# Yotsuei/ClearConverse

Measured on AMD Instinct MI355X. Metric: xRT (audio-sec/wall-sec) end-to-end, 30 s 16 kHz clips, higher is better.
Workload: dtype bf16

## Files before the change

clearconverse_amd/_lib.py:

```python
from __future__ import annotations

import ctypes as C
import os
from pathlib import Path
from typing import Optional

_PKG = Path(__file__).resolve().parent
LIB_PATH = _PKG / "libccx.so"


class CcxError(RuntimeError):
    pass


class WhisperDims(C.Structure):
    _fields_ = [(n, C.c_int) for n in (
        "n_mels", "n_audio_ctx", "n_audio_state", "n_audio_head", "n_audio_layer",
        "n_vocab", "n_text_ctx", "n_text_state", "n_text_head", "n_text_layer")]


class SepformerDims(C.Structure):
    _fields_ = [(n, C.c_int) for n in (
        "n_filters", "kernel", "stride", "d_model", "n_head", "d_ffn", "n_layers", "n_blocks", "segment", "n_spk")]


class DecodeRules(C.Structure):
    _fields_ = [(n, C.c_int) for n in (
        "eot", "sot", "sot_prev", "no_speech", "no_timestamps", "timestamp_begin", "blank",
        "max_initial_timestamp_index", "n_suppress")] + [("suppress", C.POINTER(C.c_int))]


class GemmDesc(C.Structure):
    _fields_ = [
        ("A", C.c_void_p), ("W", C.c_void_p), ("lda", C.c_int64), ("ldw", C.c_int64),
        ("M", C.c_int), ("N", C.c_int), ("K", C.c_int), ("ntaps", C.c_int), ("a_tap_stride", C.c_int64),
        ("bias", C.c_void_p), ("out", C.c_void_p), ("ldo", C.c_int64), ("resid", C.c_void_p), ("ldr", C.c_int64),
        ("resid_mod", C.c_int), ("scale", C.c_void_p), ("shift", C.c_void_p), ("slope", C.c_float),
        ("rpb_in", C.c_int), ("rpb_out", C.c_int), ("roff", C.c_int), ("rpb_valid", C.c_int),
        ("img_rows_in", C.c_int), ("img_rows_valid", C.c_int), ("img_rows_out", C.c_int),
        ("resid_bf16", C.c_void_p), ("ldrb", C.c_int64),
        ("hq", C.c_void_p), ("hk", C.c_void_p), ("hv", C.c_void_p),
        ("d_model", C.c_int), ("n_head", C.c_int), ("S", C.c_int), ("Spad", C.c_int),
        ("v_transposed", C.c_int), ("first_block", C.c_int),
        ("a_elems", C.c_int64), ("w_elems", C.c_int64), ("out_elems", C.c_int64), ("resid_elems", C.c_int64),
        ("resid_bf16_elems", C.c_int64), ("heads_elems", C.c_int64)]


class DecAttnDesc(C.Structure):
    _fields_ = [
        ("q", C.c_void_p), ("k", C.c_void_p), ("v", C.c_void_p),
        ("rows", C.c_int), ("n_seq", C.c_int), ("H", C.c_int), ("kv_T", C.c_int), ("T", C.c_int),
        ("pos", C.POINTER(C.c_int)), ("row_seq", C.POINTER(C.c_int)), ("rows_per_seq", C.c_int),
        ("nsplit", C.c_int), ("combine", C.c_int), ("lds_pad", C.c_int),
        ("x", C.c_void_p), ("pend", C.c_void_p), ("pend_n", C.c_int), ("pend_stride", C.c_int64),
        ("ln_g", C.c_void_p), ("ln_b", C.c_void_p), ("eps", C.c_float),
        ("wq_host", C.c_void_p), ("bq", C.c_void_p),
        ("out", C.c_void_p), ("part_o", C.c_void_p), ("part_ml", C.c_void_p), ("q_x_out", C.c_void_p),
        ("q_elems", C.c_int64), ("kv_elems", C.c_int64), ("out_elems", C.c_int64), ("part_o_elems", C.c_int64),
        ("part_ml_elems", C.c_int64), ("x_elems", C.c_int64), ("pend_elems", C.c_int64), ("q_x_out_elems", C.c_int64)]


DEC_ATTN_SELF, DEC_ATTN_SPLIT, DEC_ATTN_STREAM, DEC_ATTN_PREFILL, DEC_ATTN_FUSED_Q, DEC_ATTN_TWO_LAUNCH_Q = range(6)


class DecSeqState(C.Structure):
    _fields_ = [(n, C.c_int) for n in ("pos", "prompt_len", "n_gen", "done", "last_tok", "pen_tok", "last_ts_tok", "n_tokens")] + [
        ("sum_logprob", C.c_float), ("no_speech_prob", C.c_float)]


class DecSelectDesc(C.Structure):
    _fields_ = [
        ("logits", C.c_void_p), ("ld", C.c_int64), ("n_vocab", C.c_int), ("B", C.c_int),
        ("rules", C.POINTER(DecodeRules)), ("state", C.POINTER(DecSeqState)),
        ("prompt", C.POINTER(C.c_int)), ("max_prompt", C.c_int), ("sample_len", C.c_int),
        ("gen", C.POINTER(C.c_int)), ("cur_tok", C.POINTER(C.c_int)), ("pos", C.POINTER(C.c_int)), ("n_done", C.POINTER(C.c_int)),
        ("tok_emb", C.c_void_p), ("pos_emb", C.c_void_p), ("x", C.c_void_p), ("D", C.c_int),
        ("sample", C.c_int), ("temperature", C.c_float), ("seed", C.c_uint64), ("row0", C.c_int),
        ("logits_elems", C.c_int64), ("tok_emb_elems", C.c_int64), ("pos_emb_elems", C.c_int64), ("x_elems", C.c_int64)]


class SepDesc(C.Structure):
    _fields_ = (
        [(n, C.c_void_p) for n in ("h", "xin", "y", "qkv", "att", "feats", "fc")]
        + [(n, C.c_int64) for n in ("h_elems", "xin_elems", "y_elems", "qkv_elems", "att_elems", "feats_elems", "fc_elems")]
        + [("rows", C.c_int), ("seq_start", C.POINTER(C.c_int)), ("seq_len", C.POINTER(C.c_int)), ("n_seq", C.c_int),
           ("n_tok", C.c_int), ("d_ffn", C.c_int)]
        + [(n, C.c_void_p) for n in ("ln_g", "ln_b", "gln_g", "gln_b", "wqkv", "bqkv", "wo", "bo", "w1", "b1", "w2", "b2", "wdec")]
        + [(n, C.c_int64) for n in ("ln_elems", "gln_elems", "wqkv_elems", "bqkv_elems", "wo_elems", "bo_elems", "w1_elems",
                                    "b1_elems", "w2_elems", "b2_elems", "wdec_elems")]
        + [("utt_tok0", C.POINTER(C.c_int)), ("utt_L", C.POINTER(C.c_int)), ("utt_T", C.POINTER(C.c_int)), ("n_utt", C.c_int),
           ("segment", C.c_int), ("out", C.c_void_p), ("out_stride", C.c_int64), ("out_elems", C.c_int64)])


SEP_ATTN_BLOCK, SEP_ATTENTION, SEP_FFN, SEP_FINAL_NORM, SEP_DECODER = range(5)


class AlignDesc(C.Structure):
    _fields_ = [
        ("q", C.c_void_p), ("k", C.c_void_p), ("q_elems", C.c_int64), ("k_elems", C.c_int64),
        ("n_seq", C.c_int), ("H", C.c_int), ("Spad", C.c_int),
        ("heads", C.POINTER(C.c_int)), ("n_heads", C.c_int), ("head0", C.c_int), ("t", C.c_int),
        ("Hsel", C.c_int), ("T", C.c_int), ("Mmax", C.c_int),
        ("n_keys", C.POINTER(C.c_int)), ("n_rows", C.POINTER(C.c_int)), ("r0", C.c_int),
        ("P", C.c_void_p), ("A", C.c_void_p), ("P_elems", C.c_int64), ("A_elems", C.c_int64),
        ("text_idx", C.c_void_p), ("time_idx", C.c_void_p), ("path_len", C.c_void_p), ("jump_frame", C.c_void_p),
        ("text_idx_elems", C.c_int64), ("time_idx_elems", C.c_int64), ("path_len_elems", C.c_int64), ("jump_frame_elems", C.c_int64)]


ALIGN_SCORES, ALIGN_MATRIX, ALIGN_DTW = range(3)


_vp, _i, _i64, _f = C.c_void_p, C.c_int, C.c_int64, C.c_float
_ip = C.POINTER(C.c_int)
_i32p = C.POINTER(C.c_int32)
_i64p = C.POINTER(C.c_int64)
_fp = C.POINTER(C.c_float)

PROTOTYPES = {
    "ccx_version": (C.c_char_p, []),
    "ccx_ctx_create": (_i, [_i, C.POINTER(_vp)]),
    "ccx_ctx_destroy": (None, [_vp]),
    "ccx_last_error": (C.c_char_p, [_vp]),
    "ccx_prof_enable": (_i, [_vp, _i]),
    "ccx_prof_count": (_i, [_vp]),
    "ccx_prof_get": (_i, [_vp, _i, C.c_char_p, _i, C.POINTER(C.c_double), C.POINTER(C.c_double), _fp]),
    "ccx_gemm_bf16": (_i, [_vp, _i, _vp, _i64, _vp, _i64, _vp, _vp, _i64, _vp, _i64, _i, _i, _i, _vp]),
    "ccx_gemm_bf16_desc": (_i, [_vp, _i, C.POINTER(GemmDesc), _vp]),
    "ccx_layernorm": (_i, [_vp, _vp, _vp, _vp, _vp, _vp, _i, _i, _f, _vp]),
    "ccx_gather_rows": (_i, [_vp, _vp, _vp, _i, _i, _vp, _i64, _vp]),
    "ccx_peak_normalize": (_i, [_vp, _vp, _vp, _i64, _vp, _i, _f, _vp]),
    "ccx_row_variance": (_i, [_vp, _vp, _i64, _vp, _i, _vp, _vp]),
    "ccx_cross_attention_xa": (_i, [_vp, _vp, _vp, _vp, _vp, _vp, _vp, _i, _i, _i, _i, _i, _vp, _vp]),
    "ccx_cosine_rows": (_i, [_vp, _vp, _vp, _i, _i, _i, _vp, _vp]),
    "ccx_speaker_profiles": (_i, [_vp, _vp, _vp, _vp, _i, _i, _i, _i, _vp, _vp]),
    "ccx_resample_sinc": (_i, [_vp, _vp, _i64, _vp, _i, _i, _i, _i, _vp, _vp, _i64, _vp, _i, _vp]),
    "ccx_enc_attention": (_i, [_vp, _vp, _vp, _vp, _vp, _i, _i, _i, _i, _vp]),
    "ccx_whisper_create": (_i, [_vp, C.POINTER(WhisperDims), _i, C.POINTER(_vp)]),
    "ccx_whisper_destroy": (None, [_vp]),
    "ccx_whisper_set_tensor": (_i, [_vp, C.c_char_p, _vp, _i, _i, _i64p]),
    "ccx_whisper_set_max_audio": (_i, [_vp, C.c_double]),
    "ccx_whisper_share_encoder_scratch": (_i, [_vp, _vp]),
    "ccx_whisper_finalize": (_i, [_vp]),
    "ccx_whisper_set_rules": (_i, [_vp, C.POINTER(DecodeRules)]),
    "ccx_whisper_logmel": (_i, [_vp, _vp, _i64, _ip, _ip, _i, _vp, _vp]),
    "ccx_whisper_set_mel": (_i, [_vp, _vp, _i, _vp]),
    "ccx_whisper_encode": (_i, [_vp, _i, _vp, _vp]),
    "ccx_whisper_decoder_logits": (_i, [_vp, _i32p, _i, _i, _vp, _vp]),
    "ccx_whisper_decode_greedy": (_i, [_vp, _i32p, _i32p, _i, _i, _i, _i32p, _i32p, _fp, _fp, _vp]),
    "ccx_dec_attention_desc": (_i, [_vp, _i, C.POINTER(DecAttnDesc), _vp]),
    "ccx_dec_select_step": (_i, [_vp, C.POINTER(DecSelectDesc), _vp]),
    "ccx_align_op": (_i, [_vp, _i, C.POINTER(AlignDesc), _vp]),
    "ccx_whisper_align": (_i, [_vp, _i32p, _i32p, _i, _i, _i32p, _i32p, _i, _i, _vp, _vp, _i32p, _vp]),
    "ccx_whisper_last_cross_path": (_i, [_vp]),
    "ccx_whisper_prepare_lanes": (_i, [_vp, _vp]),
    "ccx_whisper_trace_lanes": (_i, [_vp, C.c_char_p, _i]),
    "ccx_whisper_decode": (_i, [_vp, _i32p, _i32p, _i, _i, _i, _f, C.c_uint64, _i32p, _i32p, _fp, _fp, _vp]),
    "ccx_sepformer_create": (_i, [_vp, C.POINTER(SepformerDims), _i, _i, C.POINTER(_vp)]),
    "ccx_sepformer_destroy": (None, [_vp]),
    "ccx_sepformer_set_tensor": (_i, [_vp, C.c_char_p, _vp, _i64]),
    "ccx_sepformer_finalize": (_i, [_vp]),
    "ccx_sepformer_separate": (_i, [_vp, _vp, _i64, _ip, _i, _vp, _vp]),
    "ccx_sep_op": (_i, [_vp, _i, C.POINTER(SepDesc), _vp]),
    "ccx_speaker_create": (_i, [_vp, _i, _i, _i, _i, _i64, C.POINTER(_vp)]),
    "ccx_speaker_destroy": (None, [_vp]),
    "ccx_speaker_set_tensor": (_i, [_vp, C.c_char_p, _vp, _i64]),
    "ccx_speaker_finalize": (_i, [_vp]),
    "ccx_speaker_embed": (_i, [_vp, _vp, _i64p, _ip, _i, _vp, _i64p, _ip, _vp, _vp]),
    "ccx_speaker_segment": (_i, [_vp, _vp, _i64p, _ip, _i, _vp, _i64, _ip, _vp]),
    "ccx_resnet_create": (_i, [_vp, _i, _i64, _i, C.POINTER(_vp)]),
    "ccx_resnet_destroy": (None, [_vp]),
    "ccx_resnet_set_tensor": (_i, [_vp, C.c_char_p, _vp, _i64]),
    "ccx_resnet_finalize": (_i, [_vp]),
    "ccx_resnet_embed": (_i, [_vp, _vp, _i64, _i, _i, _vp, _i, _ip, _i, _vp, _vp]),
    "ccx_specgate_create": (_i, [_vp, _i64, _i, _i, C.POINTER(_vp)]),
    "ccx_specgate_destroy": (None, [_vp]),
    "ccx_specgate_reduce": (_i, [_vp, _vp, _i64, _ip, _i, _f, _vp, _vp]),
    "ccx_specgate_reduce_long": (_i, [_vp, _vp, _i64, _f, _vp, _vp]),
    "ccx_specgate_set_clip_noise": (_i, [_vp, _i]),
}

_lib: Optional[C.CDLL] = None


def load() -> C.CDLL:
    global _lib
    if _lib is not None:
        return _lib
    if not LIB_PATH.exists():
        raise CcxError(f"{LIB_PATH} is missing: run `python -m clearconverse_amd.build` "
                       "(there is no CPU fallback for the HIP path)")
    import torch
    try:
        lib = C.CDLL(str(LIB_PATH))
    except OSError as e:
        raise CcxError(f"cannot load {LIB_PATH}: {e}") from e
    for name, (res, args) in PROTOTYPES.items():
        try:
            fn = getattr(lib, name)
        except AttributeError as e:
            raise CcxError(f"libccx.so does not export {name}") from e
        fn.restype = res
        fn.argtypes = args
    _lib = lib
    return lib


class Context:

    def __init__(self, device: int = 0):
        self.lib = load()
        h = _vp()
        rc = self.lib.ccx_ctx_create(device, C.byref(h))
        if rc != 0:
            raise CcxError(f"ccx_ctx_create({device}) failed: {self.lib.ccx_last_error(None).decode()}")
        self.handle = h
        self.device = device

    def check(self, rc: int, what: str = ""):
        if rc != 0:
            raise CcxError(f"{what or 'ccx call'} failed ({rc}): {self.lib.ccx_last_error(self.handle).decode()}")

    prof_on = False

    def prof_enable(self, on: bool = True):
        self.check(self.lib.ccx_prof_enable(self.handle, 1 if on else 0), "ccx_prof_enable")
        self.prof_on = bool(on)

    def prof_records(self):
        out = []
        buf = C.create_string_buffer(64)
        fl, by, ms = C.c_double(), C.c_double(), C.c_float()
        for i in range(self.lib.ccx_prof_count(self.handle)):
            self.check(self.lib.ccx_prof_get(self.handle, i, buf, 64, C.byref(fl), C.byref(by), C.byref(ms)), "ccx_prof_get")
            out.append((buf.value.decode(), fl.value, by.value, ms.value))
        return out

    def close(self):
        if getattr(self, "handle", None):
            self.lib.ccx_ctx_destroy(self.handle)
            self.handle = None

    def __del__(self):
        try:
            self.close()
        except Exception:
            pass


def current_stream_ptr() -> int:
    import torch
    return int(torch.cuda.current_stream().cuda_stream)


def ptr(t) -> int:
    if t is None:
        return 0
    if not t.is_contiguous():
        raise CcxError("tensor passed to libccx must be contiguous")
    return int(t.data_ptr())
```

clearconverse_amd/csrc/dec_ops.hip:

```cpp
#include "../../include/ccx.h"
#include "ccx_common.h"
#include "decoder.h"
#include "op_scratch.h"

static_assert(sizeof(ccx_dec_seq_state) == sizeof(DecSeqState), "ccx_dec_seq_state mirrors DecSeqState field for field");

namespace {

__global__ void dec_ops_bf16_to_f32_kernel(const bf16_t* __restrict__ in, float* __restrict__ out, long n) {
  const long i = (long)blockIdx.x * 256 + threadIdx.x;
  if (i < n) out[i] = bf16_to_f32(in[i]);
}

}

extern "C" int ccx_dec_attention_desc(ccx_ctx* ctx, int form, const ccx_dec_attn_desc* d, void* stream_) {
  if (!ctx) return CCX_ERR_ARG;
  hipStream_t stream = (hipStream_t)stream_;
  CCX_REQUIRE(ctx, d != nullptr, "ccx_dec_attention_desc: desc is NULL");
  CCX_REQUIRE(ctx, form >= CCX_DEC_ATTN_SELF && form <= CCX_DEC_ATTN_TWO_LAUNCH_Q, "ccx_dec_attention_desc: unknown form %d", form);
  const bool is_self = form == CCX_DEC_ATTN_SELF, is_split = form == CCX_DEC_ATTN_SPLIT, is_stream = form == CCX_DEC_ATTN_STREAM;
  const bool is_prefill = form == CCX_DEC_ATTN_PREFILL, with_q = form == CCX_DEC_ATTN_FUSED_Q || form == CCX_DEC_ATTN_TWO_LAUNCH_Q;
  const bool partials = is_split || with_q;
  const bool final_out = is_self || is_stream || is_prefill || (is_split && d->combine);
  const int rows = d->rows, H = d->H, n_seq = d->n_seq, kv_T = d->kv_T;
  CCX_REQUIRE(ctx, rows >= 1 && rows <= 65536 && n_seq >= 1 && n_seq <= 65536 && H >= 1 && H <= 64 && kv_T >= 1 && kv_T <= (1 << 20),
              "ccx_dec_attention_desc: rows=%d, n_seq=%d, H=%d or kv_T=%d out of range", rows, n_seq, H, kv_T);
  CCX_REQUIRE(ctx, d->k && d->v && ccx_aligned16(d->k) && ccx_aligned16(d->v), "ccx_dec_attention_desc: k / v null or not 16-byte aligned");
  const int64_t kv_need = (int64_t)n_seq * H * kv_T * 64;
  CCX_REQUIRE(ctx, kv_need <= d->kv_elems, "ccx_dec_attention_desc: k / v are read up to element %ld, kv_elems=%ld", (long)kv_need, (long)d->kv_elems);
  if (is_self || is_split || is_prefill) {
    if (d->row_seq)
      for (int i = 0; i < rows; i++)
        CCX_REQUIRE(ctx, d->row_seq[i] >= 0 && d->row_seq[i] < n_seq, "ccx_dec_attention_desc: row_seq[%d] = %d out of range [0, %d)", i, d->row_seq[i], n_seq);
    else CCX_REQUIRE(ctx, rows <= n_seq, "ccx_dec_attention_desc: row_seq is NULL with more rows (%d) than sequences (%d)", rows, n_seq);
  } else {
    CCX_REQUIRE(ctx, d->row_seq == nullptr, "ccx_dec_attention_desc: row_seq is not taken by form %d (row r reads sequence r)", form);
    CCX_REQUIRE(ctx, rows <= n_seq, "ccx_dec_attention_desc: more rows (%d) than sequences (%d)", rows, n_seq);
  }
  if (is_prefill) {
    const int P = d->rows_per_seq;
    CCX_REQUIRE(ctx, P >= 2 && P <= 4096, "ccx_dec_attention_desc: rows_per_seq = %d, the prefill form needs >= 2", P);
    CCX_REQUIRE(ctx, d->row_seq && rows % P == 0, "ccx_dec_attention_desc: rows_per_seq needs row_seq and a multiple of it in rows");
    for (int i = 0; i < rows; i++) {
      CCX_REQUIRE(ctx, d->row_seq[i] == d->row_seq[i - i % P], "ccx_dec_attention_desc: row %d is not in its group's sequence (row_seq)", i);
      CCX_REQUIRE(ctx, d->row_seq[i] == i / P, "ccx_dec_attention_desc: row_seq[%d] = %d, the prefill form needs group g on sequence g", i, d->row_seq[i]);
    }
  } else CCX_REQUIRE(ctx, d->rows_per_seq <= 1, "ccx_dec_attention_desc: rows_per_seq = %d is taken by the prefill form only", d->rows_per_seq);
  if (is_self) {
    CCX_REQUIRE(ctx, d->pos != nullptr, "ccx_dec_attention_desc: pos is NULL");
    for (int i = 0; i < rows; i++)
      CCX_REQUIRE(ctx, d->pos[i] >= 0 && d->pos[i] < kv_T, "ccx_dec_attention_desc: pos[%d] = %d out of range [0, kv_T = %d)", i, d->pos[i], kv_T);
  } else {
    CCX_REQUIRE(ctx, d->pos == nullptr, "ccx_dec_attention_desc: pos is taken by the self form only");
    CCX_REQUIRE(ctx, d->T >= 1 && d->T <= kv_T, "ccx_dec_attention_desc: T = %d out of range [1, kv_T = %d]", d->T, kv_T);
  }
  if (is_prefill) CCX_REQUIRE(ctx, d->T <= 1536, "ccx_dec_attention_desc: T = %d, the prefill form streams at most 1536 keys per block", d->T);
  const int nsplit = partials ? d->nsplit : 1;
  CCX_REQUIRE(ctx, nsplit >= 1 && nsplit <= 8, "ccx_dec_attention_desc: nsplit = %d out of range [1, 8]", d->nsplit);
  CCX_REQUIRE(ctx, d->lds_pad >= 0 && d->lds_pad <= 128 * 1024 && ((is_split || is_stream) || d->lds_pad == 0),
              "ccx_dec_attention_desc: lds_pad = %d out of range [0, 131072] or given to a form that has none", d->lds_pad);
  if (!with_q) {
    CCX_REQUIRE(ctx, d->q && ccx_aligned16(d->q), "ccx_dec_attention_desc: q null or not 16-byte aligned");
    CCX_REQUIRE(ctx, (int64_t)rows * H * 64 <= d->q_elems, "ccx_dec_attention_desc: q is read up to element %ld, q_elems=%ld", (long)rows * H * 64, (long)d->q_elems);
  }
  if (final_out) {
    CCX_REQUIRE(ctx, d->out != nullptr, "ccx_dec_attention_desc: out is NULL");
    CCX_REQUIRE(ctx, (int64_t)rows * H * 64 <= d->out_elems, "ccx_dec_attention_desc: out is written up to element %ld, out_elems=%ld", (long)rows * H * 64, (long)d->out_elems);
  }
  if (partials) {
    CCX_REQUIRE(ctx, d->part_o && d->part_ml && ccx_aligned16(d->part_o) && ccx_aligned16(d->part_ml), "ccx_dec_attention_desc: part_o / part_ml null or not 16-byte aligned");
    const int64_t po = (int64_t)rows * H * nsplit * 64, pml = (int64_t)rows * H * nsplit * 2;
    CCX_REQUIRE(ctx, po <= d->part_o_elems, "ccx_dec_attention_desc: part_o is written up to element %ld, part_o_elems=%ld", (long)po, (long)d->part_o_elems);
    CCX_REQUIRE(ctx, pml <= d->part_ml_elems, "ccx_dec_attention_desc: part_ml is written up to element %ld, part_ml_elems=%ld", (long)pml, (long)d->part_ml_elems);
  }
  if (with_q) {
    CCX_REQUIRE(ctx, rows <= 16 && H == 12, "ccx_dec_attention_desc: the fused query needs rows <= 16 (got %d) and H == 12 (got %d)", rows, H);
    CCX_REQUIRE(ctx, d->x && d->pend && d->ln_g && d->ln_b && d->bq && d->wq_host, "ccx_dec_attention_desc: x, pend, ln_g, ln_b, bq or wq_host is NULL");
    CCX_REQUIRE(ctx, ccx_aligned16(d->x) && ccx_aligned16(d->pend) && ccx_aligned16(d->ln_g) && ccx_aligned16(d->ln_b) && ccx_aligned16(d->bq),
                "ccx_dec_attention_desc: x, pend, ln_g, ln_b or bq not 16-byte aligned");
    CCX_REQUIRE(ctx, d->pend_n >= 0 && d->pend_n <= 4, "ccx_dec_attention_desc: pend_n = %d out of range [0, 4]", d->pend_n);
    CCX_REQUIRE(ctx, d->pend_stride >= (int64_t)rows * 768 && d->pend_stride % 4 == 0, "ccx_dec_attention_desc: pend_stride = %ld smaller than a slab or not a multiple of 4", (long)d->pend_stride);
    CCX_REQUIRE(ctx, (int64_t)rows * 768 <= d->x_elems, "ccx_dec_attention_desc: x is read up to element %ld, x_elems=%ld", (long)rows * 768, (long)d->x_elems);
    const int64_t pn = (int64_t)((d->pend_n > 1 ? d->pend_n : 1) - 1) * d->pend_stride + (int64_t)rows * 768;
    CCX_REQUIRE(ctx, pn <= d->pend_elems, "ccx_dec_attention_desc: pend is read up to element %ld, pend_elems=%ld", (long)pn, (long)d->pend_elems);
    if (d->q_x_out) {
      CCX_REQUIRE(ctx, ccx_aligned16(d->q_x_out) && d->q_x_out != d->x, "ccx_dec_attention_desc: q_x_out not 16-byte aligned or aliasing x");
      CCX_REQUIRE(ctx, (int64_t)rows * 768 <= d->q_x_out_elems, "ccx_dec_attention_desc: q_x_out is written up to element %ld, q_x_out_elems=%ld", (long)rows * 768, (long)d->q_x_out_elems);
    }
  }

  ccx_op_scratch sc;
#define DO_HIP(expr) do { hipError_t e_ = (expr); if (e_ != hipSuccess) return ccx_fail(ctx, CCX_ERR_HIP, "%s failed: %s", #expr, hipGetErrorString(e_)); } while (0)
  DecAttnParams ap;
  memset(&ap, 0, sizeof(ap));
  ap.q = (const float*)d->q; ap.k = (const bf16_t*)d->k; ap.v = (const bf16_t*)d->v; ap.H = H; ap.kv_T = kv_T; ap.T = is_self ? 0 : d->T;
  ap.scale_log2e = 0.125f * 1.4426950408889634f;
  ap.part_o = (float*)d->part_o; ap.part_ml = (float*)d->part_ml; ap.lds_pad = d->lds_pad;
  const long n_out = (long)rows * H * 64;
  bf16_t* d_out16 = nullptr;
  if (final_out) {
    DO_HIP(sc.alloc(&d_out16, (size_t)n_out));
    DO_HIP(hipMemsetAsync(d_out16, 0xFF, (size_t)n_out * 2, stream));
    ap.out_bf16 = d_out16;
  }
  int* d_pos = nullptr; int* d_rs = nullptr;
  if (is_self) { DO_HIP(sc.upload(&d_pos, d->pos, (size_t)rows)); ap.pos = d_pos; }
  if (d->row_seq) { DO_HIP(sc.upload(&d_rs, d->row_seq, (size_t)rows)); ap.row_seq = d_rs; }
  bf16_t* d_wq = nullptr; float* d_q = nullptr;
  if (with_q) {
    const std::vector<bf16_t> packed = pack_mfma_rows(d->wq_host, 768, 768, 16);
    DO_HIP(sc.upload(&d_wq, packed.data(), packed.size()));
  }
  int rc = CCX_OK;
  if (is_self) rc = ccx_launch_dec_attention(ctx, ap, rows, 1, true, stream);
  else if (is_split) {
    rc = ccx_launch_dec_attention(ctx, ap, rows, nsplit, false, stream);
    if (rc == CCX_OK && d->combine) rc = ccx_launch_dec_combine(ctx, ap.part_o, ap.part_ml, nsplit, d_out16, rows, H, stream);
  } else if (is_stream) {
    ap.stream_mode = 1;
    rc = ccx_launch_dec_attention(ctx, ap, rows, 1, true, stream);
  } else if (is_prefill) {
    ap.stream_mode = 1; ap.rows_per_seq = d->rows_per_seq;
    rc = ccx_launch_dec_attention(ctx, ap, rows / d->rows_per_seq, 1, true, stream);
  } else if (form == CCX_DEC_ATTN_FUSED_Q) {
    ap.qx = (const float*)d->x; ap.q_pend = (const float*)d->pend; ap.q_pend_n = d->pend_n; ap.q_pend_stride = (long)d->pend_stride;
    ap.q_x_out = (float*)d->q_x_out; ap.q_ln_g = (const float*)d->ln_g; ap.q_ln_b = (const float*)d->ln_b; ap.q_eps = d->eps;
    ap.q_W = d_wq; ap.q_bias = (const float*)d->bq; ap.q_K = 768;
    rc = ccx_launch_dec_cross_fused_q(ctx, ap, rows, nsplit, stream);
  } else {
    DO_HIP(sc.alloc(&d_q, (size_t)rows * 768));
    DecLinearParams lp;
    memset(&lp, 0, sizeof(lp));
    lp.M = rows; lp.N = 768; lp.K = 768; lp.W = d_wq; lp.ldw = 768; lp.bias = (const float*)d->bq; lp.out = d_q; lp.ldo = 768;
    lp.x = (const float*)d->x; lp.pend = (const float*)d->pend; lp.pend_n = d->pend_n; lp.pend_stride = (long)d->pend_stride;
    lp.x_out = (float*)d->q_x_out; lp.ln_g = (const float*)d->ln_g; lp.ln_b = (const float*)d->ln_b; lp.eps = d->eps;
    rc = ccx_launch_dec_linear(ctx, ACT_LN, DEPI_F32, lp, stream);
    ap.q = d_q;
    if (rc == CCX_OK) rc = ccx_launch_dec_attention(ctx, ap, rows, nsplit, false, stream);
  }
  if (rc == CCX_OK && final_out) {
    hipLaunchKernelGGL(dec_ops_bf16_to_f32_kernel, dim3((unsigned)((n_out + 255) / 256)), dim3(256), 0, stream, d_out16, (float*)d->out, n_out);
    DO_HIP(hipGetLastError());
  }
  DO_HIP(hipStreamSynchronize(stream));
  return rc;
}

extern "C" int ccx_dec_select_step(ccx_ctx* ctx, const ccx_dec_select_desc* d, void* stream_) {
  if (!ctx) return CCX_ERR_ARG;
  hipStream_t stream = (hipStream_t)stream_;
  CCX_REQUIRE(ctx, d != nullptr, "ccx_dec_select_step: desc is NULL");
  const int V = d->n_vocab, B = d->B, D = d->D;
  CCX_REQUIRE(ctx, B >= 1 && B <= 65536, "ccx_dec_select_step: B = %d out of range", B);
  CCX_REQUIRE(ctx, V >= 4 && V % 4 == 0 && V <= 13 * 4096, "ccx_dec_select_step: n_vocab = %d must be a multiple of 4 and <= 53248", V);
  CCX_REQUIRE(ctx, d->ld >= V && d->ld % 4 == 0, "ccx_dec_select_step: ld = %ld must be >= n_vocab and a multiple of 4", (long)d->ld);
  CCX_REQUIRE(ctx, d->logits && ccx_aligned16(d->logits), "ccx_dec_select_step: logits null or not 16-byte aligned");
  CCX_REQUIRE(ctx, (int64_t)(B - 1) * d->ld + V <= d->logits_elems, "ccx_dec_select_step: logits are read up to element %ld, logits_elems=%ld",
              (long)((int64_t)(B - 1) * d->ld + V), (long)d->logits_elems);
  CCX_REQUIRE(ctx, d->rules && d->state && d->gen && d->cur_tok && d->pos && d->n_done, "ccx_dec_select_step: rules, state, gen, cur_tok, pos or n_done is NULL");
  const ccx_decode_rules& r = *d->rules;
  std::vector<unsigned char> mask;
  CCX_TRY(ccx_build_suppress_mask(ctx, "ccx_dec_select_step", &r, V, mask));
  CCX_REQUIRE(ctx, r.no_speech >= 0 && r.timestamp_begin >= 0 && r.blank >= 0, "ccx_dec_select_step: rules.no_speech, timestamp_begin or blank negative");
  CCX_REQUIRE(ctx, d->sample_len >= 1 && d->sample_len <= (1 << 20), "ccx_dec_select_step: sample_len = %d out of range", d->sample_len);
  CCX_REQUIRE(ctx, d->max_prompt >= 0 && (d->max_prompt == 0 || d->prompt), "ccx_dec_select_step: prompt is NULL with max_prompt = %d", d->max_prompt);
  CCX_REQUIRE(ctx, D >= 4 && D % 4 == 0 && D <= 4096, "ccx_dec_select_step: D = %d must be a multiple of 4 in [4, 4096]", D);
  CCX_REQUIRE(ctx, d->tok_emb && d->pos_emb && d->x && ccx_aligned16(d->tok_emb) && ccx_aligned16(d->pos_emb) && ccx_aligned16(d->x),
              "ccx_dec_select_step: tok_emb, pos_emb or x null or not 16-byte aligned");
  CCX_REQUIRE(ctx, (int64_t)V * D <= d->tok_emb_elems, "ccx_dec_select_step: tok_emb is read up to element %ld, tok_emb_elems=%ld", (long)V * D, (long)d->tok_emb_elems);
  CCX_REQUIRE(ctx, (int64_t)B * D <= d->x_elems, "ccx_dec_select_step: x is written up to element %ld, x_elems=%ld", (long)B * D, (long)d->x_elems);
  const int64_t pos_rows = d->pos_emb_elems / D;
  CCX_REQUIRE(ctx, d->sample == 0 || d->sample == 1, "ccx_dec_select_step: sample = %d must be 0 or 1", d->sample);
  CCX_REQUIRE(ctx, d->sample || d->temperature == 0.f, "ccx_dec_select_step: temperature %g needs sample = 1", (double)d->temperature);
  CCX_REQUIRE(ctx, d->temperature >= 0.f && d->row0 >= 0, "ccx_dec_select_step: temperature or row0 negative");
  for (int b = 0; b < B; b++) {
    const ccx_dec_seq_state& s = d->state[b];
    CCX_REQUIRE(ctx, s.n_gen >= 0 && s.n_gen <= d->sample_len, "ccx_dec_select_step: state[%d].n_gen = %d out of range [0, sample_len = %d]", b, s.n_gen, d->sample_len);
    CCX_REQUIRE(ctx, s.pos >= 0 && s.pos + 1 < pos_rows, "ccx_dec_select_step: state[%d].pos = %d, pos + 1 must be a row of pos_emb (%ld rows)", b, s.pos, (long)pos_rows);
    CCX_REQUIRE(ctx, s.prompt_len >= 0 && s.prompt_len <= d->max_prompt, "ccx_dec_select_step: state[%d].prompt_len = %d out of range [0, max_prompt = %d]", b, s.prompt_len, d->max_prompt);
    CCX_REQUIRE(ctx, s.done == 0 || s.done == 1, "ccx_dec_select_step: state[%d].done = %d must be 0 or 1", b, s.done);
    const bool prompt_phase = s.pos < s.prompt_len - 1;
    if (prompt_phase) {
      const int tok = d->prompt[(size_t)b * d->max_prompt + s.pos + 1];
      CCX_REQUIRE(ctx, tok >= 0 && tok < V, "ccx_dec_select_step: prompt[%d][%d] = %d out of range", b, s.pos + 1, tok);
    } else if (!s.done) {
      CCX_REQUIRE(ctx, s.n_gen < d->sample_len, "ccx_dec_select_step: state[%d].n_gen = %d leaves no room in gen (sample_len = %d)", b, s.n_gen, d->sample_len);
      CCX_REQUIRE(ctx, s.last_tok < V && s.pen_tok < V && s.last_ts_tok < V, "ccx_dec_select_step: state[%d] holds a token id >= n_vocab", b);
    }
  }

  ccx_op_scratch sc;
  unsigned char* d_mask = nullptr; DecSeqState* d_state = nullptr;
  int *d_prompt = nullptr, *d_cur = nullptr, *d_pos = nullptr, *d_gen = nullptr, *d_ndone = nullptr;
  unsigned* d_cfg = nullptr;
  const size_t n_gen_tab = (size_t)B * d->sample_len;
  constexpr int kGuard = 16;
  std::vector<int> gen_h(n_gen_tab + kGuard, 0x5a5a5a5a);
  memcpy(gen_h.data(), d->gen, n_gen_tab * 4);
  DO_HIP(sc.upload(&d_mask, mask.data(), mask.size()));
  DO_HIP(sc.upload(&d_state, (const DecSeqState*)d->state, (size_t)B));
  if (d->max_prompt > 0) DO_HIP(sc.upload(&d_prompt, d->prompt, (size_t)B * d->max_prompt));
  DO_HIP(sc.upload(&d_cur, d->cur_tok, (size_t)B));
  DO_HIP(sc.upload(&d_pos, d->pos, (size_t)B));
  DO_HIP(sc.upload(&d_gen, gen_h.data(), gen_h.size()));
  DO_HIP(sc.upload(&d_ndone, d->n_done, (size_t)1));
  unsigned cfg[4] = {0u, (unsigned)(d->seed & 0xffffffffu), (unsigned)(d->seed >> 32), 0u};
  memcpy(&cfg[0], &d->temperature, 4);
  DO_HIP(sc.upload(&d_cfg, cfg, (size_t)4));

  DecSelectParams sp;
  memset(&sp, 0, sizeof(sp));
  sp.logits = (const float*)d->logits; sp.ld_logits = (long)d->ld; sp.n_vocab = V; sp.state = d_state; sp.prompt = d_prompt;
  sp.max_prompt = d->max_prompt; sp.cur_tok = d_cur; sp.pos = d_pos; sp.gen = d_gen; sp.sample_len = d->sample_len;
  sp.n_done = d_ndone; sp.suppress_mask = d_mask; sp.eot = r.eot; sp.blank = r.blank;
  sp.no_speech = r.no_speech; sp.timestamp_begin = r.timestamp_begin;
  sp.max_initial_ts = r.max_initial_timestamp_index;
  sp.tok_emb = (const float*)d->tok_emb; sp.pos_emb = (const float*)d->pos_emb; sp.x = (float*)d->x; sp.D = D;
  sp.sample_cfg = d_cfg; sp.row0 = d->row0; sp.sample = d->sample;
  CCX_TRY(ccx_launch_dec_select(ctx, sp, B, stream));
  DO_HIP(hipStreamSynchronize(stream));
  DO_HIP(hipMemcpy(gen_h.data(), d_gen, gen_h.size() * 4, hipMemcpyDeviceToHost));
  for (int i = 0; i < kGuard; i++)
    if (gen_h[n_gen_tab + i] != 0x5a5a5a5a) return ccx_fail(ctx, CCX_ERR_STATE, "ccx_dec_select_step: the kernel wrote behind the gen table (word %d)", i);
  memcpy(d->gen, gen_h.data(), n_gen_tab * 4);
  DO_HIP(hipMemcpy(d->state, d_state, (size_t)B * sizeof(DecSeqState), hipMemcpyDeviceToHost));
  DO_HIP(hipMemcpy(d->cur_tok, d_cur, (size_t)B * 4, hipMemcpyDeviceToHost));
  DO_HIP(hipMemcpy(d->pos, d_pos, (size_t)B * 4, hipMemcpyDeviceToHost));
  DO_HIP(hipMemcpy(d->n_done, d_ndone, 4, hipMemcpyDeviceToHost));
#undef DO_HIP
  return CCX_OK;
}
```

clearconverse_amd/csrc/decoder.h:

```cpp
#pragma once
#include <vector>
#include "../../include/ccx.h"
#include "ccx_common.h"

enum { ACT_LN = 0, ACT_BF16 = 1, ACT_COMBINE = 2 };
enum { DEPI_BF16_GELU = 1, DEPI_PARTIAL = 2, DEPI_F32 = 3, DEPI_SELF_QKV = 4, DEPI_RESOLVE = 5 };

struct DecLinearParams {
  int M, N, K;
  const bf16_t* W; long ldw;
  const float* bias;
  const float* x;
  const float* pend; int pend_n; long pend_stride;
  float* x_out;
  const float* ln_g; const float* ln_b; float eps;
  float* ln_mean_out;
  const bf16_t* act; long lda;
  const float* part_o; const float* part_ml; int nsplit;
  float* xres; bf16_t* xb; float2* st_out; const float* shift; float shift_c;
  void* out; long ldo;
  bf16_t* cache_k; bf16_t* cache_v; int cache_T; const int* pos; const int* row_seq;
};
int ccx_launch_dec_linear(ccx_ctx* ctx, int act, int epi, const DecLinearParams& p, hipStream_t stream);
int ccx_dec_linear_ksplit(int K, int epi);
int ccx_launch_dec_resolve_ln(ccx_ctx* ctx, const float* x, const float* pend, int pend_n, long pend_stride, const float* g,
                              const float* b, bf16_t* out, float* x_out, int M, int K, float eps, hipStream_t stream,
                              float* mean_out = nullptr);

struct DecAttnParams {
  const float* q;
  const bf16_t* k;
  const bf16_t* v;
  int H, kv_T;
  const int* pos;
  int T;
  float scale_log2e;
  bf16_t* out_bf16;
  float* part_o;
  float* part_ml;
  int lds_pad;
  int stream_mode;
  const int* row_seq; int rows_per_seq;
  const float* qx; const float* q_pend; int q_pend_n; long q_pend_stride; float* q_x_out;
  const float* q_ln_g; const float* q_ln_b; float q_eps;
  const bf16_t* q_W; const float* q_bias; int q_K;
};
int ccx_launch_dec_attention(ccx_ctx* ctx, const DecAttnParams& p, int B, int nsplit, bool final_out, hipStream_t stream);
int ccx_launch_dec_cross_fused_q(ccx_ctx* ctx, const DecAttnParams& p, int B, int nsplit, hipStream_t stream);

struct DecSeqState {
  int pos, prompt_len, n_gen, done;
  int last_tok, pen_tok, last_ts_tok, n_tokens;
  float sum_logprob, no_speech_prob;
};

struct DecSelectParams {
  const float* logits; long ld_logits; int n_vocab;
  DecSeqState* state;
  const int* prompt; int max_prompt;
  int* cur_tok; int* pos;
  int* gen; int sample_len;
  int* n_done;
  const unsigned char* suppress_mask;
  int eot, blank, no_speech, timestamp_begin, max_initial_ts;
  const float* tok_emb; const float* pos_emb; float* x; int D;
  const unsigned* sample_cfg; int row0;
  int sample;
};
int ccx_launch_dec_select(ccx_ctx* ctx, const DecSelectParams& p, int B, hipStream_t stream);
int ccx_launch_dec_embed(ccx_ctx* ctx, const float* tok_emb, const float* pos_emb, const int* cur_tok, const int* pos,
                         float* x, int B, int D, hipStream_t stream);
int ccx_launch_dec_gather_rows(ccx_ctx* ctx, const bf16_t* src, const int* idx, bf16_t* dst, int n, int D, hipStream_t stream);
int ccx_launch_dec_combine(ccx_ctx* ctx, const float* part_o, const float* part_ml, int nsplit, bf16_t* out, int M, int H,
                           hipStream_t stream);

static inline std::vector<bf16_t> pack_mfma_rows(const float* src, int N, int K, int row_pad) {
  const int Np = (N + row_pad - 1) / row_pad * row_pad;
  const int kst = K / 32;
  std::vector<bf16_t> tmp((size_t)Np * K, 0);
  for (int nt = 0; nt < Np / 16; nt++)
    for (int ks = 0; ks < kst; ks++)
      for (int l = 0; l < 64; l++) {
        const int n = nt * 16 + (l & 15), k0 = ks * 32 + 8 * (l >> 4);
        bf16_t* dst = &tmp[(((size_t)nt * kst + ks) * 64 + l) * 8];
        if (n < N)
          for (int j = 0; j < 8; j++) dst[j] = ccx_host_f32_to_bf16(src[(size_t)n * K + k0 + j]);
      }
  return tmp;
}

static inline int ccx_build_suppress_mask(ccx_ctx* ctx, const char* who, const ccx_decode_rules* r, int V, std::vector<unsigned char>& mask) {
  CCX_REQUIRE(ctx, r->eot >= 0 && r->eot < V, "%s: rules.eot = %d out of range [0, n_vocab = %d)", who, r->eot, V);
  CCX_REQUIRE(ctx, r->sot < V, "%s: rules.sot = %d out of range (n_vocab = %d)", who, r->sot, V);
  CCX_REQUIRE(ctx, r->no_speech < V, "%s: rules.no_speech = %d out of range (n_vocab = %d)", who, r->no_speech, V);
  CCX_REQUIRE(ctx, r->timestamp_begin <= V, "%s: rules.timestamp_begin = %d behind n_vocab = %d", who, r->timestamp_begin, V);
  CCX_REQUIRE(ctx, r->blank < V, "%s: rules.blank = %d out of range (n_vocab = %d)", who, r->blank, V);
  CCX_REQUIRE(ctx, r->no_timestamps < V, "%s: rules.no_timestamps = %d out of range (n_vocab = %d)", who, r->no_timestamps, V);
  mask.assign((size_t)V + 4, 0);
  for (int i = 0; i < r->n_suppress; i++) {
    CCX_REQUIRE(ctx, r->suppress[i] >= 0 && r->suppress[i] < V, "%s: rules.suppress[%d] = %d out of range [0, n_vocab = %d)", who, i, r->suppress[i], V);
    mask[r->suppress[i]] = 1;
  }
  if (r->no_timestamps >= 0) mask[r->no_timestamps] = 1;
  return CCX_OK;
}
```

clearconverse_amd/csrc/decoder.hip:

```cpp
#include <string>
#include "decoder.h"

__global__ void dec_embed_kernel(const float* __restrict__ tok_emb, const float* __restrict__ pos_emb,
                                 const int* __restrict__ cur_tok, const int* __restrict__ pos, float* __restrict__ x,
                                 int D) {
  const int b = blockIdx.x;
  const float4* te = (const float4*)(tok_emb + (long)cur_tok[b] * D);
  const float4* pe = (const float4*)(pos_emb + (long)pos[b] * D);
  float4* xo = (float4*)(x + (long)b * D);
  for (int i = threadIdx.x; i < D / 4; i += blockDim.x) {
    const float4 a = te[i], c = pe[i];
    xo[i] = make_float4(a.x + c.x, a.y + c.y, a.z + c.z, a.w + c.w);
  }
}

#include "dec_ln.h"

__device__ __forceinline__ float centre_shift(float mean, float rstd) { return fabsf(mean) * rstd > 1.f ? mean : 0.f; }

__device__ __forceinline__ uint4 combine_partials(const float* part_o, const float* part_ml, int nsplit, int mh, int c) {
  const float2* ml = (const float2*)(part_ml + ((long)mh * nsplit) * 2);
  const float* ob = part_o + ((long)mh * nsplit) * 64 + 8 * c;
  float2 mlv[8];
  float4 oa[8], oc[8];
// ... 1043 lines not shown
#pragma unroll
  for (int i = 0; i < SEL_V4; i++) {
    const int v0 = tid * 4 + i * 4096;
    if (v0 + 3 < V) {
      const float4 f = *(const float4*)(lg + v0);
      const uchar4 m = *(const uchar4*)(p.suppress_mask + v0);
      val[4 * i] = f.x; val[4 * i + 1] = f.y; val[4 * i + 2] = f.z; val[4 * i + 3] = f.w;
      sup |= ((unsigned long long)((m.x ? 1 : 0) | (m.y ? 2 : 0) | (m.z ? 4 : 0) | (m.w ? 8 : 0))) << (4 * i);
    } else {
      val[4 * i] = val[4 * i + 1] = val[4 * i + 2] = val[4 * i + 3] = -INFINITY;
      sup |= 0xFull << (4 * i);
    }
  }
  const int i_gen = s.n_gen;
  const int tsb = p.timestamp_begin;

  if (i_gen == 0) {
    float mx = -INFINITY;
#pragma unroll
    for (int i = 0; i < SEL_V4 * 4; i++) mx = fmaxf(mx, val[i]);
    mx = block_reduce_max(mx, sh);
    float sum = 0.f;
#pragma unroll
    for (int i = 0; i < SEL_V4 * 4; i++) sum += __builtin_amdgcn_exp2f((val[i] - mx) * 1.4426950408889634f);
    sum = block_reduce_sum(sum, sh);
    if (tid == 0) s.no_speech_prob = expf(lg[p.no_speech] - mx) / sum;
  }

  const bool last_ts = i_gen >= 1 && s.last_tok >= tsb;
  const bool pen_ts = i_gen < 2 || s.pen_tok >= tsb;
  int s_lo = tsb;
  if (s.last_ts_tok >= 0) s_lo = (last_ts && !pen_ts) ? s.last_ts_tok : s.last_ts_tok + 1;
  int s_hi = V;
  if (i_gen == 0 && p.max_initial_ts >= 0) s_hi = tsb + p.max_initial_ts + 1;
  if (last_ts && pen_ts) s_hi = s_lo;
  const int t_lo = (i_gen == 0) ? tsb : ((last_ts && !pen_ts) ? p.eot : 0);

  float mx_text = -INFINITY, mx_ts = -INFINITY;
  int am_text = 0x7fffffff, am_ts = 0x7fffffff;
#pragma unroll
  for (int i = 0; i < SEL_V4 * 4; i++) {
    const int v = tid * 4 + (i >> 2) * 4096 + (i & 3);
    const bool is_text = v < tsb;
    const bool allowed = !((sup >> i) & 1) && (is_text ? (v >= t_lo) : (v >= s_lo && v < s_hi));
    const float x = allowed ? val[i] : -INFINITY;
    val[i] = x;
    const bool bt_ = is_text && x > mx_text, bs_ = !is_text && x > mx_ts;
    mx_text = bt_ ? x : mx_text; am_text = bt_ ? v : am_text;
    mx_ts = bs_ ? x : mx_ts; am_ts = bs_ ? v : am_ts;
  }
  auto block_argmax = [&](float v_, int idx, float& oval, int& oidx) {
#pragma unroll
    for (int o = 32; o > 0; o >>= 1) {
      const float ov = __shfl_xor(v_, o, 64);
      const int oi = __shfl_xor(idx, o, 64);
      if (ov > v_ || (ov == v_ && oi < idx)) { v_ = ov; idx = oi; }
    }
    __syncthreads();
    if ((tid & 63) == 0) { sh_v[tid >> 6] = v_; sh_i[tid >> 6] = idx; }
    __syncthreads();
    oval = sh_v[0]; oidx = sh_i[0];
    for (int w = 1; w < (int)(blockDim.x >> 6); w++)
      if (sh_v[w] > oval || (sh_v[w] == oval && sh_i[w] < oidx)) { oval = sh_v[w]; oidx = sh_i[w]; }
  };
  float bt, bs; int it, is;
  block_argmax(mx_text, am_text, bt, it);
  block_argmax(mx_ts, am_ts, bs, is);
  const float mx_all = fmaxf(bt, bs);

  float se_text = 0.f, se_ts = 0.f;
#pragma unroll
  for (int i = 0; i < SEL_V4 * 4; i++) {
    const int v = tid * 4 + (i >> 2) * 4096 + (i & 3);
    const float e = __builtin_amdgcn_exp2f((val[i] - mx_all) * 1.4426950408889634f);
    se_text += (v < tsb) ? e : 0.f;
    se_ts += (v < tsb) ? 0.f : e;
  }
  se_text = block_reduce_sum(se_text, sh);
  se_ts = block_reduce_sum(se_ts, sh);

  const float lse_ts = (se_ts > 0.f) ? mx_all + logf(se_ts) : -INFINITY;
  const bool force_ts = lse_ts > bt;
  const float lnorm = logf(force_ts ? se_ts : se_text + se_ts);

  const float temperature = SAMPLE ? __uint_as_float(p.sample_cfg[0]) : 0.f;
  int samp = -1; float samp_logit = 0.f;
  if (SAMPLE && temperature > 0.f) {
    const uint2 key = make_uint2(p.sample_cfg[1], p.sample_cfg[2]);
    const float inv_t = 1.0f / temperature;
    float best = -INFINITY, best_logit = -INFINITY; int best_i = 0x7fffffff;
#pragma unroll
    for (int i = 0; i < SEL_V4; i++) {
      const int v0 = tid * 4 + i * 4096;
      const uint4 r = philox4x32_10(make_uint4((unsigned)(v0 >> 2), (unsigned)(p.row0 + b), (unsigned)i_gen, 0u), key);
      const unsigned rr[4] = {r.x, r.y, r.z, r.w};
#pragma unroll
      for (int j = 0; j < 4; j++) {
        const int v = v0 + j;
        const float x = (force_ts && v < tsb) ? -INFINITY : val[4 * i + j];
        const float sc = x * inv_t + gumbel_from_u32(rr[j]);
        if (sc > best) { best = sc; best_i = v; best_logit = x; }
      }
    }
    float ov; int oi;
    block_argmax(best, best_i, ov, oi);
    samp = oi;
    __syncthreads();
    if (best_i == samp && best == ov) sh[0] = best_logit;
    __syncthreads();
    samp_logit = sh[0];
  }

  if (tid == 0) {
    int next; float logprob;
    if (samp >= 0) {
      next = samp;
      logprob = (samp_logit - mx_all) - lnorm;
    } else if (force_ts) {
      next = is;
      logprob = (bs - mx_all) - lnorm;
    } else {
      if (bt > bs || (bt == bs && it < is)) next = it; else next = is;
      logprob = -lnorm;
    }
    s.sum_logprob += logprob;
    p.gen[(long)b * p.sample_len + i_gen] = next;
    s.n_gen = i_gen + 1;
    s.pen_tok = s.last_tok;
    s.last_tok = next;
    if (next >= tsb) s.last_ts_tok = next;
    int cont = 0;
    if (next == p.eot) {
      s.done = 1;
      s.n_tokens = i_gen;
      atomicAdd(p.n_done, 1);
    } else if (s.n_gen >= p.sample_len) {
      s.done = 1;
      s.n_tokens = s.n_gen;
      atomicAdd(p.n_done, 1);
    } else {
      s.pos += 1;
      p.cur_tok[b] = next;
      p.pos[b] = s.pos;
      cont = 1;
    }
    p.state[b] = s;
    sh_next[0] = cont ? next : -1;
    sh_next[1] = s.pos;
  }
  __syncthreads();
  if (sh_next[0] >= 0) embed_next(sh_next[0], sh_next[1]);
}

int ccx_launch_dec_embed(ccx_ctx* ctx, const float* tok_emb, const float* pos_emb, const int* cur_tok, const int* pos,
                         float* x, int B, int D, hipStream_t stream) {
  hipLaunchKernelGGL(dec_embed_kernel, dim3(B), dim3(192), 0, stream, tok_emb, pos_emb, cur_tok, pos, x, D);
  CCX_CHECK_LAUNCH(ctx);
  return CCX_OK;
}

int ccx_launch_dec_select(ccx_ctx* ctx, const DecSelectParams& p, int B, hipStream_t stream) {
  ccx_prof_scope ps(ctx, stream, "dec_select_kernel", 0.0, (double)B * p.n_vocab * 5.0);
  if (p.sample) hipLaunchKernelGGL(dec_select_kernel<true>, dim3(B), dim3(1024), 0, stream, p);
  else hipLaunchKernelGGL(dec_select_kernel<false>, dim3(B), dim3(1024), 0, stream, p);
  CCX_CHECK_LAUNCH(ctx);
  return CCX_OK;
}
```

clearconverse_amd/csrc/gemm_bf16.h:

```cpp
#pragma once
#include "ccx_common.h"

enum GemmEpi {
  EPI_BF16 = 0,
  EPI_BF16_GELU = 1,
  EPI_F32_RESID = 2,
  EPI_F32 = 3,
  EPI_HEADS = 4,
  EPI_BF16_RELU = 5,
  EPI_F32_GELU_POS = 6,
  EPI_BF16_LRELU_AFFINE = 7,
  EPI_BF16_ADD_RELU = 8
};

struct GemmParams {
  const bf16_t* A;
  const bf16_t* W;
  long lda, ldw;
  int M, N, K;
  int ntaps; long a_tap_stride;
  const float* bias;
  void* out;
  long ldo;
  const float* resid;
  long ldr;
  int resid_mod;
  const float* scale; const float* shift;
  float slope;
  int rpb_in, rpb_out, roff, rpb_valid;
  int img_rows_in, img_rows_valid, img_rows_out;
  const bf16_t* resid_bf16; long ldrb;
  bf16_t* hq; bf16_t* hk; bf16_t* hv;
  int d_model, n_head;
  int S, Spad;
  int v_transposed;
  int first_block;
};

__host__ __device__ inline long ccx_gemm_remap_row(const GemmParams& p, int m, bool& valid) {
  if (p.rpb_in <= 0) { valid = true; return m; }
  int g = m / p.rpb_in;
  const int i = m - g * p.rpb_in;
  valid = i < p.rpb_valid;
  if (p.img_rows_in > 0) {
    const int img = g / p.img_rows_in, r = g - img * p.img_rows_in;
    valid = valid && r < p.img_rows_valid;
    g = img * p.img_rows_out + r;
  }
  return (long)g * p.rpb_out + i + p.roff;
}

int ccx_launch_gemm(ccx_ctx* ctx, int epi, const GemmParams& p, hipStream_t stream);
```

clearconverse_amd/csrc/gemm_bf16.hip:

```cpp
#include <map>
#include <string>
#include "gemm_bf16.h"

#ifndef CCX_ABL_NO_MFMA
#define CCX_ABL_NO_MFMA 0
#endif
#ifndef CCX_ABL_NO_DMA
#define CCX_ABL_NO_DMA 0
#endif
#ifndef CCX_ABL_NO_EPI
#define CCX_ABL_NO_EPI 0
#endif
#ifndef CCX_ABL_STORE_LOCAL
#define CCX_ABL_STORE_LOCAL 0
#endif
#define BM 128
#define BN 128
#define BK 64
#define STAGE_BYTES 32768

typedef const __attribute__((address_space(1))) void* gptr_t;
typedef __attribute__((address_space(3))) void* lptr_t;

__device__ __forceinline__ int keyA(int r) { return (r >> 1) & 7; }
template <int CM> __device__ __forceinline__ int w_row(int j, int i) {
  return CM == 1 ? 16 * j + i : 32 * (j >> 1) + 8 * (i >> 2) + 4 * (j & 1) + (i & 3);
}
template <int CM> __device__ __forceinline__ int keyW(int r) {
  return CM == 1 ? (r >> 1) & 7 : ((r >> 1) & 1) | (((r >> 3) & 1) << 1) | (((r >> 4) & 1) << 2);
}
template <int CM> __device__ __forceinline__ int col4(int j, int h) {
  return CM == 1 ? 16 * j + 4 * h : 32 * (j >> 1) + 8 * h + 4 * (j & 1);
}
__device__ __forceinline__ void epi_store16(void* dst, uint4 v) { *(uint4*)dst = v; }
__device__ __forceinline__ void epi_store16f(void* dst, float4 v) { *(float4*)dst = v; }
__device__ __forceinline__ float4 epi_load16f(const float* src) { return *(const float4*)src; }

constexpr int colmap_of(int epi) { return (epi == EPI_F32 || epi == EPI_F32_RESID || epi == EPI_F32_GELU_POS) ? 1 : 2; }

template <bool SWAP, int CM, int WM, int WN, int MT>
__device__ __forceinline__ void gemm_mainloop(const GemmParams& p, char* smem, int m0, int n0, f32x4 (&acc)[MT][4]) {
  constexpr int NW = WM * WN;
  constexpr int A_ROWS = WM * MT * 16, B_ROWS = WN * 64;
  constexpr int A_BYTES = A_ROWS * 128, B_BYTES = B_ROWS * 128;
  constexpr int STAGE = A_BYTES + B_BYTES;
  constexpr int NA = A_ROWS / 8 / NW, NB = B_ROWS / 8 / NW;
  const int tid = threadIdx.x, lane = tid & 63, wave = tid >> 6;
  const int wr = wave / WN, wc = wave % WN;

  const bf16_t* srcA[NA];
  const bf16_t* srcB[NB];
#pragma unroll
  for (int i = 0; i < NA; i++) {
    const int r = (wave * NA + i) * 8 + (lane >> 3);
    int gm = m0 + r; gm = gm < p.M ? gm : p.M - 1;
    srcA[i] = p.A + (long)gm * p.lda + (((lane & 7) ^ keyA(r)) << 3);
  }
#pragma unroll
  for (int i = 0; i < NB; i++) {
    const int r = (wave * NB + i) * 8 + (lane >> 3);
    int gn = n0 + r; gn = gn < p.N ? gn : p.N - 1;
    srcB[i] = p.W + (long)gn * p.ldw + (((lane & 7) ^ keyW<CM>(r)) << 3);
  }
  const int kt_per_tap = p.K / BK;
  auto stage = [&](int t, int buf) {
    char* sA = smem + buf * STAGE;
    char* sB = sA + A_BYTES;
    const int tap = t / kt_per_tap;
    const long ka = (long)(t - tap * kt_per_tap) * BK + (long)tap * p.a_tap_stride;
    const int kw = t * BK;
#pragma unroll
    for (int i = 0; i < NA; i++)
      __builtin_amdgcn_global_load_lds((gptr_t)(srcA[i] + ka), (lptr_t)(sA + (wave * NA + i) * 1024), 16, 0, 0);
#pragma unroll
    for (int i = 0; i < NB; i++)
      __builtin_amdgcn_global_load_lds((gptr_t)(srcB[i] + kw), (lptr_t)(sB + (wave * NB + i) * 1024), 16, 0, 0);
  };

  const int l15 = lane & 15, h = lane >> 4;
  const int ka = keyA(l15);
  const int kb = keyW<CM>(w_row<CM>(0, l15));
  int offA[2], offB[2];
#pragma unroll
  for (int ks = 0; ks < 2; ks++) {
    offA[ks] = (wr * MT * 16 + l15) * 128 + (((4 * ks + h) ^ ka) << 4);
    offB[ks] = (wc * 64 + w_row<CM>(0, l15)) * 128 + (((4 * ks + h) ^ kb) << 4);
  }

  const int nt = kt_per_tap * (p.ntaps > 1 ? p.ntaps : 1);
  stage(0, 0);
  __syncthreads();
  for (int t = 0; t < nt; t++) {
    const int buf = t & 1;
    if (t + 1 < nt) stage(t + 1, buf ^ 1);
    const char* sA = smem + buf * STAGE;
    const char* sB = sA + A_BYTES;
#pragma unroll
    for (int ks = 0; ks < 2; ks++) {
      bf16x8 b[4];
#pragma unroll
      for (int j = 0; j < 4; j++) b[j] = *(const bf16x8*)(sB + offB[ks] + w_row<CM>(j, 0) * 128);
#pragma unroll
      for (int mt = 0; mt < MT; mt++) {
        const bf16x8 a = *(const bf16x8*)(sA + offA[ks] + mt * 16 * 128);
#pragma unroll
        for (int j = 0; j < 4; j++) {
          if (SWAP)
            acc[mt][j] = __builtin_amdgcn_mfma_f32_16x16x32_bf16(b[j], a, acc[mt][j], 0, 0, 0);
          else
            acc[mt][j] = __builtin_amdgcn_mfma_f32_16x16x32_bf16(a, b[j], acc[mt][j], 0, 0, 0);
        }
      }
    }
    __syncthreads();
  }
}

__device__ __forceinline__ long remap_row(const GemmParams& p, int m, bool& valid) { return ccx_gemm_remap_row(p, m, valid); }

template <int EPI, int WM, int WN, int MT, typename MainLoop>
__device__ __forceinline__ void gemm_tile(const GemmParams& p, char* smem, int m0, int n0, MainLoop mainloop) {
  constexpr int CM = colmap_of(EPI);
  const int lane = threadIdx.x & 63;
  const int wave = __builtin_amdgcn_readfirstlane(threadIdx.x >> 6);
  const int wr = wave / WN, wc = wave % WN;
  const int l15 = lane & 15, h = lane >> 4;
  const int cb = n0 + wc * 64;

  f32x4 acc[MT][4];
#pragma unroll
  for (int i = 0; i < MT; i++)
#pragma unroll
    for (int j = 0; j < 4; j++) acc[i][j] = (f32x4){0.f, 0.f, 0.f, 0.f};

  if (EPI == EPI_HEADS) {
    const int blk = n0 / p.d_model + p.first_block;
    if (blk == 2 && p.v_transposed) {
      mainloop(p, smem, m0, n0, acc, std::false_type{});
      float bvj[4];
#pragma unroll
      for (int j = 0; j < 4; j++) bvj[j] = p.bias ? p.bias[cb + w_row<CM>(j, l15)] : 0.f;
#pragma unroll
      for (int j = 0; j < 4; j++) asm volatile("" ::"v"(bvj[j]));
#pragma unroll
      for (int j = 0; j < 4; j++) {
        const int n = cb + w_row<CM>(j, l15);
        const int nn = n % p.d_model, hh = nn >> 6, d = nn & 63;
        const float bv = bvj[j];
#pragma unroll
        for (int mt = 0; mt < MT; mt++) {
          const int m = m0 + wr * MT * 16 + mt * 16 + 4 * h;
          if (m < p.M) {
            const int b = m / p.S, s = m - b * p.S;
            bf16_t* dst = p.hv + ((long)(b * p.n_head + hh) * 64 + d) * p.Spad + s;
            uint2 v;
            v.x = pack_bf16x2(acc[mt][j][0] + bv, acc[mt][j][1] + bv);
            v.y = pack_bf16x2(acc[mt][j][2] + bv, acc[mt][j][3] + bv);
            *(uint2*)dst = v;
          }
        }
      }
      return;
    }
  }

  mainloop(p, smem, m0, n0, acc, std::true_type{});

  const int Nw = (p.N + 15) & ~15;
  if (EPI != EPI_HEADS && cb >= Nw) return;
  int c4[4];
#pragma unroll
  for (int j = 0; j < 4; j++) c4[j] = cb + col4<CM>(j, h);
  float bias[16];
#pragma unroll
  for (int i = 0; i < 16; i++) bias[i] = 0.f;
  if (p.bias) {
    const bool al = ((uintptr_t)p.bias & 15) == 0;
#pragma unroll
    for (int j = 0; j < 4; j++) {
      if (al && c4[j] + 4 <= p.N) {
        const float4 b4 = *(const float4*)(p.bias + c4[j]);
        bias[4 * j] = b4.x; bias[4 * j + 1] = b4.y; bias[4 * j + 2] = b4.z; bias[4 * j + 3] = b4.w;
      } else {
#pragma unroll
        for (int r = 0; r < 4; r++) bias[4 * j + r] = (c4[j] + r < p.N) ? p.bias[c4[j] + r] : 0.f;
      }
    }
  }
#pragma unroll
  for (int i = 0; i < 16; i++) asm volatile("" ::"v"(bias[i]));

  constexpr bool RES_F32 = (EPI == EPI_F32_RESID || EPI == EPI_F32_GELU_POS || EPI == EPI_BF16_LRELU_AFFINE);
  constexpr bool RES_BF16 = (EPI == EPI_BF16_ADD_RELU);
  constexpr bool OUT_BF16 = CM == 2;
  constexpr int GM = EPI == EPI_BF16_LRELU_AFFINE ? 1 : (RES_F32 || RES_BF16) ? 2 : 4;
  constexpr int NG = MT / GM;
  struct Group {
    long orow[GM];
    bool ok[GM];
    float4 rf[RES_F32 ? GM : 1][4];
    uint4 rb[RES_BF16 ? GM : 1][2];
  };
  auto rows = [&](auto full_tag) {
    constexpr bool FULL = decltype(full_tag)::value;
    auto request = [&](int mt0, Group& G) {
      if (EPI == EPI_HEADS) return;
#pragma unroll
      for (int g = 0; g < GM; g++) {
        const int m = m0 + wr * MT * 16 + (mt0 + g) * 16 + l15;
        bool valid = FULL;
        long orow = m;
        if (!FULL) { orow = 0; if (m < p.M) orow = remap_row(p, m, valid); }
        G.ok[g] = valid; G.orow[g] = orow;
        if constexpr (RES_F32) {
          const bool have = EPI != EPI_BF16_LRELU_AFFINE || p.resid != nullptr;
          const long rrow = !valid ? 0 : (EPI != EPI_BF16_LRELU_AFFINE && p.resid_mod > 0) ? (orow % p.resid_mod) : orow;
#pragma unroll
          for (int j = 0; j < 4; j++) {
            const int cj = (FULL || c4[j] < Nw) ? c4[j] : 0;
            if (have) G.rf[g][j] = epi_load16f(p.resid + rrow * p.ldr + cj);
            else G.rf[g][j] = make_float4(0.f, 0.f, 0.f, 0.f);
          }
        }
        if constexpr (RES_BF16) {
          const long rrow = valid ? orow : 0;
#pragma unroll
          for (int i = 0; i < 2; i++) {
            const int ci = (FULL || c4[2 * i] < Nw) ? c4[2 * i] : 0;
            if (p.resid_bf16) G.rb[g][i] = *(const uint4*)(p.resid_bf16 + rrow * p.ldrb + ci);
            else G.rb[g][i] = make_uint4(0, 0, 0, 0);
          }
        }
      }
    };
    auto finish = [&](int mt0, const Group& G) {
#pragma unroll
      for (int g = 0; g < GM; g++) {
        if constexpr (RES_F32) {
#pragma unroll
          for (int j = 0; j < 4; j++) asm volatile("" ::"v"(G.rf[g][j].x), "v"(G.rf[g][j].y), "v"(G.rf[g][j].z), "v"(G.rf[g][j].w));
        }
        if constexpr (RES_BF16) {
#pragma unroll
          for (int i = 0; i < 2; i++) asm volatile("" ::"v"(G.rb[g][i].x), "v"(G.rb[g][i].y), "v"(G.rb[g][i].z), "v"(G.rb[g][i].w));
        }
      }
#pragma unroll
      for (int g = 0; g < GM; g++) {
        const int mt = mt0 + g;
        const int m = m0 + wr * MT * 16 + mt * 16 + l15;
        if (!FULL && m >= p.M) continue;
        float v[16];
#pragma unroll
        for (int j = 0; j < 4; j++)
#pragma unroll
          for (int r = 0; r < 4; r++) v[4 * j + r] = acc[mt][j][r] + bias[4 * j + r];

        if (EPI == EPI_HEADS) {
          const int blk = cb / p.d_model + p.first_block;
          const int hh = (cb % p.d_model) >> 6;
          const int b = m / p.S, s = m - b * p.S;
          bf16_t* base = blk == 0 ? p.hq : (blk == 1 ? p.hk : p.hv);
          bf16_t* dst = base + ((long)(b * p.n_head + hh) * p.Spad + s) * 64;
#pragma unroll
          for (int i = 0; i < 2; i++) {
            uint4 o;
            o.x = pack_bf16x2(v[8 * i], v[8 * i + 1]);     o.y = pack_bf16x2(v[8 * i + 2], v[8 * i + 3]);
            o.z = pack_bf16x2(v[8 * i + 4], v[8 * i + 5]); o.w = pack_bf16x2(v[8 * i + 6], v[8 * i + 7]);
            epi_store16(dst + (c4[2 * i] - cb), o);
          }
          continue;
        }

        if (!FULL && !G.ok[g]) continue;
        const long orow = CCX_ABL_STORE_LOCAL ? (G.orow[g] & 255) : G.orow[g];

        if constexpr (EPI == EPI_BF16_LRELU_AFFINE) {
#pragma unroll
          for (int j = 0; j < 4; j++) {
            v[4 * j + 0] += G.rf[g][j].x; v[4 * j + 1] += G.rf[g][j].y; v[4 * j + 2] += G.rf[g][j].z; v[4 * j + 3] += G.rf[g][j].w;
          }
#pragma unroll
          for (int j = 0; j < 4; j++)
#pragma unroll
            for (int r = 0; r < 4; r++) {
              const int c = c4[j] + r;
              float t = v[4 * j + r] >= 0.f ? v[4 * j + r] : p.slope * v[4 * j + r];
              const float sc = (p.scale && c < p.N) ? p.scale[c] : 1.f;
              const float sh = (p.shift && c < p.N) ? p.shift[c] : 0.f;
              v[4 * j + r] = t * sc + sh;
            }
        }
        if constexpr (EPI == EPI_BF16_ADD_RELU) {
          const uint32_t rw[8] = {G.rb[g][0].x, G.rb[g][0].y, G.rb[g][0].z, G.rb[g][0].w, G.rb[g][1].x, G.rb[g][1].y, G.rb[g][1].z, G.rb[g][1].w};
#pragma unroll
          for (int i = 0; i < 8; i++) {
            v[2 * i] += __uint_as_float(rw[i] << 16);
            v[2 * i + 1] += __uint_as_float(rw[i] & 0xffff0000u);
          }
#pragma unroll
          for (int i = 0; i < 16; i++) v[i] = fmaxf(v[i], 0.f);
        }
        if constexpr (OUT_BF16) {
          if (EPI == EPI_BF16_GELU) {
#pragma unroll
            for (int i = 0; i < 16; i++) v[i] = gelu_erf(v[i]);
          }
          if (EPI == EPI_BF16_RELU) {
#pragma unroll
            for (int i = 0; i < 16; i++) v[i] = fmaxf(v[i], 0.f);
          }
          bf16_t* dst = (bf16_t*)p.out + orow * p.ldo;
#pragma unroll
          for (int i = 0; i < 2; i++) {
            if (!FULL && c4[2 * i] >= Nw) continue;
            uint4 o;
            o.x = pack_bf16x2(v[8 * i], v[8 * i + 1]);     o.y = pack_bf16x2(v[8 * i + 2], v[8 * i + 3]);
            o.z = pack_bf16x2(v[8 * i + 4], v[8 * i + 5]); o.w = pack_bf16x2(v[8 * i + 6], v[8 * i + 7]);
            epi_store16(dst + c4[2 * i], o);
          }
        } else {
          if (EPI == EPI_F32_GELU_POS) {
#pragma unroll
            for (int i = 0; i < 16; i++) v[i] = gelu_erf(v[i]);
          }
          if constexpr (EPI == EPI_F32_RESID || EPI == EPI_F32_GELU_POS) {
#pragma unroll
            for (int j = 0; j < 4; j++) {
              v[4 * j + 0] += G.rf[g][j].x; v[4 * j + 1] += G.rf[g][j].y; v[4 * j + 2] += G.rf[g][j].z; v[4 * j + 3] += G.rf[g][j].w;
            }
          }
          float* dst = (float*)p.out + orow * p.ldo;
#pragma unroll
          for (int j = 0; j < 4; j++) {
            if (!FULL && c4[j] >= Nw) continue;
            epi_store16f(dst + c4[j], make_float4(v[4 * j], v[4 * j + 1], v[4 * j + 2], v[4 * j + 3]));
          }
        }
      }
    };
    Group G[2];
    request(0, G[0]);
#pragma unroll
// ... 71 lines not shown
  if (full) rows(std::true_type{});
  else rows(std::false_type{});
}

template <int EPI, int WM, int WN, int MT>
__global__ __launch_bounds__(WM * WN * 64, (WM * WN) >= 4 ? (WM * WN) / 4 * (MT == 4 ? 2 : 1) : 4) void gemm_bf16_nt_kernel(GemmParams p) {
  constexpr int TBM = WM * MT * 16, TBN = WN * 64;
  extern __shared__ __attribute__((aligned(16))) char smem[];
  const int tiles_n = (p.N + TBN - 1) / TBN;
  const int wg = xcd_remap(blockIdx.x, gridDim.x);
  const int tm = wg / tiles_n, tn = wg - tm * tiles_n;
  gemm_tile<EPI, WM, WN, MT>(p, smem, tm * TBM, tn * TBN, [](const GemmParams& pp, char* sm, int m0, int n0, f32x4 (&acc)[MT][4], auto swap) {
    gemm_mainloop<decltype(swap)::value, colmap_of(EPI), WM, WN, MT>(pp, sm, m0, n0, acc);
  });
}

template <bool SWAP, int CM>
__device__ __forceinline__ void gemm_mainloop_phased(const GemmParams& p, char* smem, int m0, int n0, f32x4 (&acc)[8][4]) {
  const int tid = threadIdx.x, lane = tid & 63;
  const int wave = __builtin_amdgcn_readfirstlane(tid >> 6);
  const int wr = wave >> 2, wc = wave & 3;

  const bf16_t* srcA[2][2];
  const bf16_t* srcB[2][2];
  int dstA[2][2], dstB[2][2];
#pragma unroll
  for (int a = 0; a < 2; a++)
#pragma unroll
    for (int i = 0; i < 2; i++) {
      const int r0 = wr * 128 + a * 64 + wc * 16 + i * 8;
      const int r = r0 + (lane >> 3);
      int gm = m0 + r; gm = gm < p.M ? gm : p.M - 1;
      srcA[a][i] = p.A + (long)gm * p.lda + (((lane & 7) ^ keyA(r)) << 3);
      dstA[a][i] = r0 * 128;
      const int x = 2 * wave + i;
      const int g8 = 8 * (x >> 2) + 4 * a + (x & 3);
      const int rb = g8 * 8 + (lane >> 3);
      int gn = n0 + rb; gn = gn < p.N ? gn : p.N - 1;
      srcB[a][i] = p.W + (long)gn * p.ldw + (((lane & 7) ^ keyW<CM>(rb)) << 3);
      dstB[a][i] = 32768 + g8 * 1024;
    }
  const int kt_per_tap = p.K / BK;
  const int nt = kt_per_tap * (p.ntaps > 1 ? p.ntaps : 1);
  auto a_koff = [&](int t) -> long {
    const int tap = t / kt_per_tap;
    return (long)(t - tap * kt_per_tap) * BK + (long)tap * p.a_tap_stride;
  };
  auto stage_a = [&](int t, long ka, int a) {
    char* buf = smem + (t & 1) * 65536;
    __builtin_amdgcn_global_load_lds((gptr_t)(srcA[a][0] + ka), (lptr_t)(buf + dstA[a][0]), 16, 0, 0);
    __builtin_amdgcn_global_load_lds((gptr_t)(srcA[a][1] + ka), (lptr_t)(buf + dstA[a][1]), 16, 0, 0);
  };
  auto stage_b = [&](int t, int b) {
    char* buf = smem + (t & 1) * 65536;
    const int kw = t * BK;
    __builtin_amdgcn_global_load_lds((gptr_t)(srcB[b][0] + kw), (lptr_t)(buf + dstB[b][0]), 16, 0, 0);
    __builtin_amdgcn_global_load_lds((gptr_t)(srcB[b][1] + kw), (lptr_t)(buf + dstB[b][1]), 16, 0, 0);
  };

  const int l15 = lane & 15, h = lane >> 4;
  const int ka_ = keyA(l15);
  const int kb_ = keyW<CM>(w_row<CM>(0, l15));
  int offA[2], offB[2];
#pragma unroll
  for (int ks = 0; ks < 2; ks++) {
    offA[ks] = (wr * 128 + l15) * 128 + (((4 * ks + h) ^ ka_) << 4);
    offB[ks] = 32768 + (wc * 64 + w_row<CM>(0, l15)) * 128 + (((4 * ks + h) ^ kb_) << 4);
  }

  long ka1 = nt > 1 ? a_koff(1) : 0;
  long ka2 = nt > 2 ? a_koff(2) : 0;
  int kk2 = nt > 2 ? 2 % kt_per_tap : 0;
  stage_a(0, 0, 0); stage_b(0, 0); stage_b(0, 1); stage_a(0, 0, 1);
  if (nt > 1) {
    stage_a(1, ka1, 0); stage_b(1, 0); stage_b(1, 1);
    asm volatile("s_waitcnt vmcnt(6)" ::: "memory");
  } else {
    asm volatile("s_waitcnt vmcnt(0)" ::: "memory");
  }
  __builtin_amdgcn_s_barrier();
  if (wr == 1) __builtin_amdgcn_s_barrier();

  bf16x8 fa[4][2], fb0[2][2], fb1[2][2];
#define CCX_PHASE_MFMA(MT0, J0, FB)                                                                         \
  __builtin_amdgcn_sched_barrier(0);                                                                        \
  __builtin_amdgcn_s_barrier();                                                                             \
  asm volatile("s_waitcnt lgkmcnt(0)" ::: "memory");                                                        \
  __builtin_amdgcn_sched_barrier(0);                                                                        \
  __builtin_amdgcn_s_setprio(1);                                                                            \
  _Pragma("unroll") for (int ks = 0; ks < 2; ks++)                                                          \
  _Pragma("unroll") for (int m = 0; m < 4; m++)                                                             \
  _Pragma("unroll") for (int jj = 0; jj < 2; jj++) {                                                        \
    if (CCX_ABL_NO_MFMA) { asm volatile("" ::"v"(FB[jj][ks]), "v"(fa[m][ks])); }                           \
    else if (SWAP) acc[MT0 + m][J0 + jj] = __builtin_amdgcn_mfma_f32_16x16x32_bf16(FB[jj][ks], fa[m][ks], acc[MT0 + m][J0 + jj], 0, 0, 0); \
    else      acc[MT0 + m][J0 + jj] = __builtin_amdgcn_mfma_f32_16x16x32_bf16(fa[m][ks], FB[jj][ks], acc[MT0 + m][J0 + jj], 0, 0, 0); \
  }                                                                                                         \
  __builtin_amdgcn_s_setprio(0);                                                                            \
  __builtin_amdgcn_sched_barrier(0);                                                                        \
  __builtin_amdgcn_s_barrier();

  for (int t = 0; t < nt; t++) {
    const char* buf = smem + (t & 1) * 65536;
#pragma unroll
    for (int ks = 0; ks < 2; ks++)
#pragma unroll
      for (int jj = 0; jj < 2; jj++) fb0[jj][ks] = *(const bf16x8*)(buf + offB[ks] + w_row<CM>(jj, 0) * 128);
    __builtin_amdgcn_sched_barrier(0);
#pragma unroll
    for (int ks = 0; ks < 2; ks++)
#pragma unroll
      for (int m = 0; m < 4; m++) fa[m][ks] = *(const bf16x8*)(buf + offA[ks] + m * 16 * 128);
    if (!CCX_ABL_NO_DMA && t + 1 < nt) stage_a(t + 1, ka1, 1);
    CCX_PHASE_MFMA(0, 0, fb0)
#pragma unroll
    for (int ks = 0; ks < 2; ks++)
#pragma unroll
      for (int jj = 0; jj < 2; jj++) fb1[jj][ks] = *(const bf16x8*)(buf + offB[ks] + w_row<CM>(2 + jj, 0) * 128);
    if (!CCX_ABL_NO_DMA && t + 2 < nt) stage_a(t + 2, ka2, 0);
    CCX_PHASE_MFMA(0, 2, fb1)
#pragma unroll
    for (int ks = 0; ks < 2; ks++)
#pragma unroll
      for (int m = 0; m < 4; m++) fa[m][ks] = *(const bf16x8*)(buf + offA[ks] + (4 + m) * 16 * 128);
    if (!CCX_ABL_NO_DMA && t + 2 < nt) stage_b(t + 2, 0);
    CCX_PHASE_MFMA(4, 2, fb1)
    if (!CCX_ABL_NO_DMA && t + 2 < nt) {
      stage_b(t + 2, 1);
      asm volatile("s_waitcnt vmcnt(6)" ::: "memory");
    } else {
      asm volatile("s_waitcnt vmcnt(0)" ::: "memory");
    }
    CCX_PHASE_MFMA(4, 0, fb0)
    ka1 = ka2;
    kk2++;
    if (kk2 == kt_per_tap) { kk2 = 0; ka2 += BK + p.a_tap_stride - (long)kt_per_tap * BK; }
    else ka2 += BK;
  }
#undef CCX_PHASE_MFMA
  if (wr == 0) __builtin_amdgcn_s_barrier();
}

template <int EPI>
__global__ __launch_bounds__(512, 1) void gemm_bf16_phased_kernel(GemmParams p) {
  extern __shared__ __attribute__((aligned(16))) char smem[];
  const int tiles_n = (p.N + 255) / 256;
  const int wg = xcd_remap(blockIdx.x, gridDim.x);
  const int tm = wg / tiles_n, tn = wg - tm * tiles_n;
  gemm_tile<EPI, 2, 4, 8>(p, smem, tm * 256, tn * 256, [](const GemmParams& pp, char* sm, int m0, int n0, f32x4 (&acc)[8][4], auto swap) {
    gemm_mainloop_phased<decltype(swap)::value, colmap_of(EPI)>(pp, sm, m0, n0, acc);
  });
}

template <int EPI, int WM, int WN, int MT>
static int launch_epi_geo(ccx_ctx* ctx, const GemmParams& p, hipStream_t stream) {
  constexpr int TBM = WM * MT * 16, TBN = WN * 64;
  constexpr int LDS = 2 * (TBM + TBN) * 128;
  const int tiles = ccx_cdiv(p.M, TBM) * ccx_cdiv(p.N, TBN);
  static ccx_lds_optin optin;
  CCX_HIP(ctx, optin.ensure(ctx->device, (const void*)gemm_bf16_nt_kernel<EPI, WM, WN, MT>, LDS));
  {
    const double obytes = (EPI == EPI_F32 || EPI == EPI_F32_RESID || EPI == EPI_F32_GELU_POS) ? 4.0 : 2.0;
    const double kt = (double)p.K * (p.ntaps > 1 ? p.ntaps : 1);
    const bool by_shape = ctx->prof_on && getenv("CCX_PROF_SHAPES") != nullptr;
    const char* label = "gemm_bf16_nt_kernel";
    if (by_shape) {
      static std::mutex mu;
      static std::map<std::string, std::string> names;
      char buf[160];
      snprintf(buf, sizeof(buf), "gemm<epi%d,%dx%d> M=%d N=%d K=%d taps=%d", EPI, TBM, TBN, p.M, p.N, p.K, p.ntaps > 1 ? p.ntaps : 1);
      std::lock_guard<std::mutex> lk(mu);
      label = names.emplace(buf, buf).first->second.c_str();
    }
    ccx_prof_scope ps(ctx, stream, label, 2.0 * p.M * (double)p.N * kt,
                      2.0 * ((double)p.M * p.K + (double)p.N * kt) + obytes * p.M * (double)p.N);
    hipLaunchKernelGGL((gemm_bf16_nt_kernel<EPI, WM, WN, MT>), dim3(tiles), dim3(WM * WN * 64), LDS, stream, p);
  }
  CCX_CHECK_LAUNCH(ctx);
  return CCX_OK;
}

template <int EPI>
static int launch_phased(ccx_ctx* ctx, const GemmParams& p, hipStream_t stream) {
  constexpr int LDS = 131072;
  const int tiles = ccx_cdiv(p.M, 256) * ccx_cdiv(p.N, 256);
  static ccx_lds_optin optin;
  CCX_HIP(ctx, optin.ensure(ctx->device, (const void*)gemm_bf16_phased_kernel<EPI>, LDS));
  {
    const double obytes = (EPI == EPI_F32 || EPI == EPI_F32_RESID || EPI == EPI_F32_GELU_POS) ? 4.0 : 2.0;
    const double kt = (double)p.K * (p.ntaps > 1 ? p.ntaps : 1);
    const bool by_shape = ctx->prof_on && getenv("CCX_PROF_SHAPES") != nullptr;
    const char* label = "gemm_bf16_nt_kernel";
    if (by_shape) {
      static std::mutex mu;
      static std::map<std::string, std::string> names;
      char buf[160];
      snprintf(buf, sizeof(buf), "gemm<epi%d,256x256> M=%d N=%d K=%d taps=%d", EPI, p.M, p.N, p.K, p.ntaps > 1 ? p.ntaps : 1);
      std::lock_guard<std::mutex> lk(mu);
      label = names.emplace(buf, buf).first->second.c_str();
    }
    ccx_prof_scope ps(ctx, stream, label, 2.0 * p.M * (double)p.N * kt,
                      2.0 * ((double)p.M * p.K + (double)p.N * kt) + obytes * p.M * (double)p.N);
    hipLaunchKernelGGL((gemm_bf16_phased_kernel<EPI>), dim3(tiles), dim3(512), LDS, stream, p);
  }
  CCX_CHECK_LAUNCH(ctx);
  return CCX_OK;
}

template <int EPI>
static int launch_epi(ccx_ctx* ctx, const GemmParams& p, hipStream_t stream) {
  const long big_tiles = (long)ccx_cdiv(p.M, 256) * ccx_cdiv(p.N, 256);
  bool fits = p.N >= 256 && (p.N % 256 == 0 || p.N >= 1024);
  if (EPI == EPI_HEADS) fits = fits && p.N % 256 == 0 && p.d_model % 256 == 0;
  if (fits && big_tiles >= 224) return launch_phased<EPI>(ctx, p, stream);
  if (EPI != EPI_HEADS && p.N <= 64) return launch_epi_geo<EPI, 4, 1, 4>(ctx, p, stream);
  return launch_epi_geo<EPI, 2, 2, 4>(ctx, p, stream);
}

int ccx_launch_gemm(ccx_ctx* ctx, int epi, const GemmParams& p, hipStream_t stream) {
  CCX_REQUIRE(ctx, p.M > 0 && p.N > 0 && p.K > 0, "gemm: empty problem M=%d N=%d K=%d", p.M, p.N, p.K);
  CCX_REQUIRE(ctx, p.K % BK == 0, "gemm: K=%d must be a multiple of %d", p.K, BK);
  CCX_REQUIRE(ctx, p.lda % 8 == 0 && p.ldw % 8 == 0, "gemm: lda/ldw must be multiples of 8 elements");
  CCX_REQUIRE(ctx, p.ntaps <= 1 || (p.a_tap_stride % 8 == 0 && p.ldw >= (long)p.ntaps * p.K), "gemm: bad tap layout");
  CCX_REQUIRE(ctx, ((uintptr_t)p.A & 15) == 0 && ((uintptr_t)p.W & 15) == 0, "gemm: A/W must be 16-byte aligned");
  if (epi == EPI_HEADS) {
    CCX_REQUIRE(ctx, p.d_model % 128 == 0 && p.S > 0 && p.S % 4 == 0 && p.Spad >= p.S && p.Spad % 8 == 0,
                "gemm heads: bad d_model/S/Spad");
    CCX_REQUIRE(ctx, p.N % 128 == 0, "gemm heads: N must be a multiple of 128");
    CCX_REQUIRE(ctx, p.n_head > 0 && p.d_model == 64 * p.n_head && p.M % p.S == 0, "gemm heads: d_model must be 64 * n_head and M a multiple of S");
    const int nblk = p.N / p.d_model;
    CCX_REQUIRE(ctx, p.N % p.d_model == 0 && p.first_block >= 0 && p.first_block + nblk <= 3,
                "gemm heads: N=%d from block %d does not fit q/k/v of d_model=%d", p.N, p.first_block, p.d_model);
    for (int b = p.first_block; b < p.first_block + nblk; b++) {
      const bf16_t* dst = b == 0 ? p.hq : (b == 1 ? p.hk : p.hv);
      CCX_REQUIRE(ctx, dst != nullptr && ((uintptr_t)dst & 15) == 0, "gemm heads: hq/hk/hv null or not 16-byte aligned (block %d)", b);
    }
  } else {
    CCX_REQUIRE(ctx, p.out != nullptr && p.ldo % 8 == 0, "gemm: out null or ldo not a multiple of 8");
    CCX_REQUIRE(ctx, p.ldo >= (long)ccx_cdiv(p.N, 16) * 16, "gemm: ldo=%ld must cover N rounded up to 16", p.ldo);
    CCX_REQUIRE(ctx, ((uintptr_t)p.out & 15) == 0, "gemm: out must be 16-byte aligned");
  }
  const long Nw = (long)ccx_cdiv(p.N, 16) * 16;
  const bool res_f32 = epi == EPI_F32_RESID || epi == EPI_F32_GELU_POS || epi == EPI_BF16_LRELU_AFFINE;
  CCX_REQUIRE(ctx, (epi != EPI_F32_RESID && epi != EPI_F32_GELU_POS) || p.resid != nullptr, "gemm: epilogue %d needs resid", epi);
  if (res_f32 && p.resid) {
    CCX_REQUIRE(ctx, ((uintptr_t)p.resid & 15) == 0, "gemm: resid must be 16-byte aligned");
    CCX_REQUIRE(ctx, p.ldr % 4 == 0 && p.ldr >= Nw, "gemm: ldr=%ld must be a multiple of 4 and cover N rounded up to 16", p.ldr);
  }
  if (epi == EPI_BF16_ADD_RELU && p.resid_bf16) {
    CCX_REQUIRE(ctx, ((uintptr_t)p.resid_bf16 & 15) == 0, "gemm: resid_bf16 must be 16-byte aligned");
    CCX_REQUIRE(ctx, p.ldrb % 8 == 0 && p.ldrb >= Nw, "gemm: ldrb=%ld must be a multiple of 8 and cover N rounded up to 16", p.ldrb);
  }
  CCX_REQUIRE(ctx, p.resid_mod >= 0, "gemm: resid_mod=%d must not be negative", p.resid_mod);
  CCX_REQUIRE(ctx, p.resid_mod == 0 || epi == EPI_F32_RESID || epi == EPI_F32_GELU_POS,
              "gemm: resid_mod is honoured by epilogues 2 and 6 only (epilogue %d)", epi);
  CCX_REQUIRE(ctx, p.rpb_in <= 0 || (p.rpb_valid > 0 && p.rpb_valid <= p.rpb_in),
              "gemm: row remap needs 0 < rpb_valid <= rpb_in (rpb_valid=%d rpb_in=%d)", p.rpb_valid, p.rpb_in);
  CCX_REQUIRE(ctx, p.img_rows_in <= 0 || (p.img_rows_valid > 0 && p.img_rows_valid <= p.img_rows_in),
              "gemm: row remap needs 0 < img_rows_valid <= img_rows_in (img_rows_valid=%d img_rows_in=%d)", p.img_rows_valid, p.img_rows_in);
  switch (epi) {
    case EPI_BF16: return launch_epi<EPI_BF16>(ctx, p, stream);
    case EPI_BF16_GELU: return launch_epi<EPI_BF16_GELU>(ctx, p, stream);
    case EPI_BF16_RELU: return launch_epi<EPI_BF16_RELU>(ctx, p, stream);
    case EPI_F32_RESID: return launch_epi<EPI_F32_RESID>(ctx, p, stream);
    case EPI_F32: return launch_epi<EPI_F32>(ctx, p, stream);
    case EPI_HEADS: return launch_epi<EPI_HEADS>(ctx, p, stream);
    case EPI_F32_GELU_POS: return launch_epi<EPI_F32_GELU_POS>(ctx, p, stream);
    case EPI_BF16_LRELU_AFFINE: return launch_epi<EPI_BF16_LRELU_AFFINE>(ctx, p, stream);
    case EPI_BF16_ADD_RELU: return launch_epi<EPI_BF16_ADD_RELU>(ctx, p, stream);
  }
  return ccx_fail(ctx, CCX_ERR_ARG, "gemm: unknown epilogue %d", epi);
}
```

clearconverse_amd/csrc/whisper.hip:

```cpp
#include <array>
#include <atomic>
#include <map>
#include <chrono>
#include <math.h>
#include "../../include/ccx.h"
#include "align.h"
#include "attention.h"
#include "ccx_common.h"
#include "cross_x.h"
#include "decoder.h"
#include "elementwise.h"
#include "gemm_bf16.h"
#include "logmel.h"
#include "model_store.h"

namespace {

struct EncLayer {
  float *ln1_g, *ln1_b, *ln2_g, *ln2_b;
  bf16_t *Wqkv, *Wo, *W1, *W2;
  float *bqkv, *bo, *b1, *b2;
};
struct DecLayer {
  float *ln1_g, *ln1_b, *lnc_g, *lnc_b, *ln2_g, *ln2_b;
  bf16_t *Wqkv, *Wo, *Wcq, *Wckv, *Wco, *W1, *W2;
  bf16_t* WckT = nullptr;
  bf16_t* Wcq_plain = nullptr;
  bf16_t* Wcq_g = nullptr;
  float *scq = nullptr, *ccq = nullptr;
  float bo_mean = 0.f;
  float *bqkv, *bo, *bcq, *bckv, *bco, *b1, *b2;
  bf16_t *crossK, *crossV, *selfK, *selfV;
};

}

struct ccx_whisper {
  ccx_ctx* ctx = nullptr;
  ccx_whisper_dims d{};
  int max_batch = 0;
  bool finalized = false;
  ccx_whisper* scratch_donor = nullptr;
  int scratch_takers = 0;
  bool destroy_pending = false;
  std::atomic<ccx_whisper*> scratch_owner{nullptr};
  hipEvent_t scratch_free = nullptr;
  ccx_dev_store store{"whisper"};

  int Spad = 0;
  int Vpad = 0;
  int Fraw = 3008;
  static constexpr int kCrossSplitMax = 8;

  LogmelTables lm{};
  bf16_t *Wc1 = nullptr, *Wc2 = nullptr;
  float *bc1 = nullptr, *bc2 = nullptr, *enc_pos = nullptr, *lnp_g = nullptr, *lnp_b = nullptr;
  std::vector<EncLayer> enc;
  float *tok_emb_f32 = nullptr, *dec_pos = nullptr, *lnd_g = nullptr, *lnd_b = nullptr;
  bf16_t* tok_emb_rm = nullptr;
  std::vector<DecLayer> dec;
  ccx_decode_rules rules{};
  unsigned char* suppress_mask = nullptr;
  bool rules_set = false;

  float* lm_raw = nullptr; unsigned int* lm_max = nullptr; int *lm_n = nullptr, *lm_seek = nullptr, *lm_seg = nullptr;
  bf16_t *im2col = nullptr, *h1 = nullptr, *xn = nullptr, *qb = nullptr, *kb = nullptr, *vtb = nullptr, *attn = nullptr,
         *ffn = nullptr, *xa = nullptr;
  float* x = nullptr;
  float *dx = nullptr, *dx2 = nullptr, *pend = nullptr, *dq = nullptr, *dlogits = nullptr, *part_o = nullptr, *part_ml = nullptr;
  bf16_t *dattn = nullptr, *dffn = nullptr, *dxn = nullptr;
  int *cur_tok = nullptr, *pos = nullptr, *prompt = nullptr, *gen = nullptr, *n_done = nullptr;
  bool sampling = false;
  unsigned* sample_cfg = nullptr;
  DecSeqState* state = nullptr;
  int max_prompt_cap = 0, sample_cap = 0;
  static constexpr int kPrefillMax = 16;
  float *pf_x = nullptr, *pf_x2 = nullptr, *pf_pend = nullptr, *pf_q = nullptr;
  bf16_t *pf_xn = nullptr, *pf_attn = nullptr, *pf_ffn = nullptr;
  int *pf_tok = nullptr, *pf_pos = nullptr, *pf_seq = nullptr, *pf_last = nullptr;
  std::map<std::array<int, 9>, hipGraphExec_t> graphs;
  hipStream_t own_stream = nullptr;
  hipEvent_t own_event = nullptr;
  static constexpr int kMaxLanes = 4;
  int cross_lds_pad = 0;
  int cross_stream = 0;
  int fuse_cross_q = 1;
  static constexpr int kKvSeqs = 80;
  bool xs_on = false, xs_active = false, xs_fuse_q = true;
  int last_cross_path = -1;
  int kv_cap = 0, kv_ready = 0;
  bf16_t *xq = nullptr, *pf_xq = nullptr;
  bf16_t *dxb = nullptr, *pf_xb = nullptr;
  float2 *dst2 = nullptr, *pf_st2 = nullptr;
  float *dshift = nullptr, *pf_shift = nullptr;
  bool lnfree = true;
  float *xs_po = nullptr, *xs_pml = nullptr, *pf_xs_po = nullptr, *pf_xs_pml = nullptr;
  static constexpr int kLanePool = 8;
  hipStream_t lane_pool[kLanePool] = {};
  std::map<hipStream_t, std::vector<hipStream_t>> lane_sets;
  int* probe_sink = nullptr;
  unsigned long long* stamps = nullptr;
  int* stamp_count = nullptr;
  bool stamps_on = false;
  int stamp_level = 1;
  std::string stamp_path;
  static constexpr int kStampCap = 1 << 16;
  hipEvent_t lane_start[kMaxLanes] = {}, lane_poll[2][kMaxLanes] = {};
  int* poll_host = nullptr;
  float *al_P = nullptr, *al_A = nullptr;
  unsigned char* al_trace = nullptr;
  int* al_ints = nullptr;
  size_t al_P_elems = 0, al_A_elems = 0, al_trace_bytes = 0, al_ints_elems = 0;
  const struct AlignPass* align_pass = nullptr;
};

struct AlignPass {
  std::vector<int> first, count;
  const int *heads = nullptr, *hsel = nullptr, *n_keys = nullptr;
  int Hsel = 0, T = 0, Mmax = 0, t = 0;
};

namespace {

int up_bf16_packed(ccx_whisper* w, bf16_t** out, const float* src, int N, int K, int row_pad) {
  return w->store.upload(out, pack_mfma_rows(src, N, K, row_pad));
}

std::vector<float> conv_to_gemm(const ccx_host_tensor& t, int Kpad) {
  const int64_t O = t.shape[0], I = t.shape[1], T = t.shape[2];
  std::vector<float> r((size_t)O * Kpad, 0.f);
  for (int64_t o = 0; o < O; o++)
    for (int64_t c = 0; c < I; c++)
      for (int64_t k = 0; k < T; k++) r[(size_t)o * Kpad + k * I + c] = t.data[(o * I + c) * T + k];
  return r;
}

int build_logmel_tables(ccx_whisper* w) {
  CCX_NEED(w->store, mf, "mel_filters", w->d.n_mels, 201);
  CCX_REQUIRE(w->ctx, w->d.n_mels == 80, "whisper: only n_mels == 80 is supported (got %d)", w->d.n_mels);
  std::vector<float> c(400 * 208, 0.f), s(400 * 208, 0.f), fb(80 * 208, 0.f);
  std::vector<int> rg(160);
  const double two_pi = 6.283185307179586476925286766559;
  for (int n = 0; n < 400; n++) {
    const double win = 0.5 - 0.5 * cos(two_pi * n / 400.0);
    for (int k = 0; k < 201; k++) {
      const int ph = (int)(((long)n * k) % 400);
      const double a = two_pi * ph / 400.0;
      c[n * 208 + k] = (float)(cos(a) * win);
      s[n * 208 + k] = (float)(sin(a) * win);
    }
  }
  for (int m = 0; m < 80; m++) {
    int k0 = 201, k1 = 0;
    for (int k = 0; k < 201; k++) {
      const float v = mf->data[m * 201 + k];
      fb[m * 208 + k] = v;
      if (v != 0.f) { if (k < k0) k0 = k; k1 = k + 1; }
    }
    if (k1 == 0) { k0 = 0; k1 = 0; }
    rg[2 * m] = k0; rg[2 * m + 1] = k1;
  }
  float *dc, *ds, *dfb; int* drg;
  CCX_TRY(w->store.upload(&dc, c));
  CCX_TRY(w->store.upload(&ds, s));
  CCX_TRY(w->store.upload(&dfb, fb));
  CCX_TRY(w->store.upload(&drg, rg));
  w->lm.dft_cos = dc; w->lm.dft_sin = ds; w->lm.mel_fb = dfb; w->lm.mel_range = drg;
  return CCX_OK;
}

std::vector<float> cat_rows(std::initializer_list<const std::vector<float>*> parts) {
  std::vector<float> r;
  for (auto p : parts) r.insert(r.end(), p->begin(), p->end());
  return r;
}

}

extern "C" {

int ccx_whisper_create(ccx_ctx* ctx, const ccx_whisper_dims* dims, int max_batch, ccx_whisper** out) {
  if (!ctx) return CCX_ERR_ARG;
  CCX_REQUIRE(ctx, dims && out, "ccx_whisper_create: null argument");
  CCX_REQUIRE(ctx, max_batch >= 1 && max_batch <= 1536, "ccx_whisper_create: max_batch %d out of range", max_batch);
  const ccx_whisper_dims& d = *dims;
  CCX_REQUIRE(ctx, d.n_audio_state % 128 == 0 && d.n_text_state == d.n_audio_state, "whisper: n_state must be a multiple of 128 and equal for encoder/decoder");
  CCX_REQUIRE(ctx, d.n_audio_state / d.n_audio_head == 64 && d.n_text_state / d.n_text_head == 64, "whisper: head_dim must be 64");
  CCX_REQUIRE(ctx, d.n_audio_state <= 1024, "whisper: n_state > 1024 not supported yet");
  CCX_REQUIRE(ctx, d.n_audio_ctx == 1500 && d.n_mels == 80, "whisper: n_audio_ctx must be 1500 and n_mels 80");
  CCX_REQUIRE(ctx, d.n_audio_ctx % 4 == 0, "whisper: n_audio_ctx must be a multiple of 4");
  CCX_REQUIRE(ctx, d.n_vocab % 4 == 0 && d.n_vocab <= 13 * 4096, "whisper: n_vocab must be a multiple of 4 and <= 53248");
  ccx_whisper* w = new ccx_whisper();
  w->ctx = ctx;
  w->store.ctx = ctx;
  w->store.zero_uploads = false;
  w->d = d;
  w->max_batch = max_batch;
  w->Spad = ccx_cdiv(d.n_audio_ctx, 128) * 128;
  w->Vpad = ccx_cdiv(d.n_vocab, 128) * 128;
  *out = w;
  return CCX_OK;
}

void ccx_whisper_destroy(ccx_whisper* w) {
  if (!w) return;
  if (w->scratch_takers > 0) {
    w->destroy_pending = true;
    return;
  }
  if (ccx_whisper* dn = w->scratch_donor) {
    w->scratch_donor = nullptr;
    ccx_whisper* me = w;
    dn->scratch_owner.compare_exchange_strong(me, nullptr);
    if (--dn->scratch_takers == 0 && dn->destroy_pending) ccx_whisper_destroy(dn);
  }
  if (w->scratch_free) hipEventDestroy(w->scratch_free);
  for (auto& g : w->graphs) hipGraphExecDestroy(g.second);
  if (w->own_stream) hipStreamDestroy(w->own_stream);
  if (w->own_event) hipEventDestroy(w->own_event);
  for (int i = 0; i < ccx_whisper::kMaxLanes; i++) {
    if (w->lane_start[i]) hipEventDestroy(w->lane_start[i]);
    if (w->lane_poll[0][i]) hipEventDestroy(w->lane_poll[0][i]);
    if (w->lane_poll[1][i]) hipEventDestroy(w->lane_poll[1][i]);
  }
  for (int i = 0; i < ccx_whisper::kLanePool; i++)
    if (w->lane_pool[i]) hipStreamDestroy(w->lane_pool[i]);
  if (w->poll_host) hipHostFree(w->poll_host);
  for (void* p : {(void*)w->al_P, (void*)w->al_A, (void*)w->al_trace, (void*)w->al_ints})
    if (p) hipFree(p);
  w->store.free_all();
  delete w;
}

int ccx_whisper_set_tensor(ccx_whisper* w, const char* name, const void* data, int dtype, int ndim, const int64_t* shape) {
  if (!w) return CCX_ERR_ARG;
  CCX_REQUIRE(w->ctx, !w->finalized, "whisper: set_tensor after finalize");
  CCX_REQUIRE(w->ctx, name && data && ndim >= 1 && ndim <= 4 && shape, "whisper: set_tensor bad arguments");
  const std::string nm(name);
  const bool known = nm == "mel_filters" || nm.rfind("encoder.", 0) == 0 || nm.rfind("decoder.", 0) == 0;
  CCX_REQUIRE(w->ctx, known, "whisper: unknown tensor name '%s'", name);
  return w->store.stage(name, data, dtype, ndim, shape);
}

int ccx_whisper_set_max_audio(ccx_whisper* w, double seconds) {
  if (!w) return CCX_ERR_ARG;
  CCX_REQUIRE(w->ctx, !w->finalized, "whisper: set_max_audio after finalize");
  CCX_REQUIRE(w->ctx, seconds >= 1.0 && seconds <= 7200.0, "whisper: max audio %.1f s out of range [1, 7200]", seconds);
  const long frames = (long)(seconds * 100.0) + 8;
  w->Fraw = (int)((frames + 31) / 32 * 32);
// ... 61 lines not shown
    CCX_TRY(w->store.upload_bf16(&w->Wc2, g2));
    CCX_TRY(w->store.upload(&w->bc1, c1b->data.data(), D));
    CCX_TRY(w->store.upload(&w->bc2, c2b->data.data(), D));
    CCX_TRY(w->store.upload(&w->enc_pos, pe->data.data(), (size_t)S * D));
    CCX_TRY(w->store.upload(&w->lnp_g, lg->data.data(), D));
    CCX_TRY(w->store.upload(&w->lnp_b, lb->data.data(), D));
  }
  w->enc.resize(d.n_audio_layer);
  const std::vector<float> zerosD(D, 0.f);
  for (int l = 0; l < d.n_audio_layer; l++) {
    const std::string p = "encoder.blocks." + std::to_string(l) + ".";
    EncLayer& L = w->enc[l];
    CCX_NEED(w->store, qw, p + "attn.query.weight", D, D); CCX_NEED(w->store, qbias, p + "attn.query.bias", D);
    CCX_NEED(w->store, kw, p + "attn.key.weight", D, D);
    CCX_NEED(w->store, vw, p + "attn.value.weight", D, D); CCX_NEED(w->store, vbias, p + "attn.value.bias", D);
    CCX_NEED(w->store, ow, p + "attn.out.weight", D, D); CCX_NEED(w->store, obias, p + "attn.out.bias", D);
    CCX_NEED(w->store, l1g, p + "attn_ln.weight", D); CCX_NEED(w->store, l1b, p + "attn_ln.bias", D);
    CCX_NEED(w->store, m0w, p + "mlp.0.weight", F, D); CCX_NEED(w->store, m0b, p + "mlp.0.bias", F);
    CCX_NEED(w->store, m2w, p + "mlp.2.weight", D, F); CCX_NEED(w->store, m2b, p + "mlp.2.bias", D);
    CCX_NEED(w->store, l2g, p + "mlp_ln.weight", D); CCX_NEED(w->store, l2b, p + "mlp_ln.bias", D);
    std::vector<float> wqkv = cat_rows({&qw->data, &kw->data, &vw->data});
    std::vector<float> bqkv = cat_rows({&qbias->data, &zerosD, &vbias->data});
    CCX_TRY(w->store.upload_bf16(&L.Wqkv, wqkv)); CCX_TRY(w->store.upload(&L.bqkv, bqkv));
    CCX_TRY(w->store.upload_bf16(&L.Wo, ow->data)); CCX_TRY(w->store.upload(&L.bo, obias->data.data(), D));
    CCX_TRY(w->store.upload_bf16(&L.W1, m0w->data)); CCX_TRY(w->store.upload(&L.b1, m0b->data.data(), F));
    CCX_TRY(w->store.upload_bf16(&L.W2, m2w->data)); CCX_TRY(w->store.upload(&L.b2, m2b->data.data(), D));
    CCX_TRY(w->store.upload(&L.ln1_g, l1g->data.data(), D)); CCX_TRY(w->store.upload(&L.ln1_b, l1b->data.data(), D));
    CCX_TRY(w->store.upload(&L.ln2_g, l2g->data.data(), D)); CCX_TRY(w->store.upload(&L.ln2_b, l2b->data.data(), D));
  }

  {
    CCX_NEED(w->store, te, "decoder.token_embedding.weight", d.n_vocab, D);
    CCX_NEED(w->store, pe, "decoder.positional_embedding", d.n_text_ctx, D);
    CCX_NEED(w->store, lg, "decoder.ln.weight", D);
    CCX_NEED(w->store, lb, "decoder.ln.bias", D);
    CCX_TRY(w->store.upload(&w->tok_emb_f32, te->data));
    CCX_TRY(w->store.upload_bf16(&w->tok_emb_rm, te->data.data(), (size_t)d.n_vocab * D));
    CCX_TRY(w->store.upload(&w->dec_pos, pe->data));
    CCX_TRY(w->store.upload(&w->lnd_g, lg->data.data(), D));
    CCX_TRY(w->store.upload(&w->lnd_b, lb->data.data(), D));
  }
  w->dec.resize(d.n_text_layer);
  const int Tc = d.n_text_ctx;
  {
    const char* e = getenv("CCX_CROSS_X");
    w->xs_on = (!e || atoi(e) != 0) && d.n_text_state == D && d.n_text_head == H && ccx_xs_supported(D, H);
    w->kv_cap = w->xs_on ? (B < ccx_whisper::kKvSeqs ? B : ccx_whisper::kKvSeqs) : B;
  }
  for (int l = 0; l < d.n_text_layer; l++) {
    const std::string p = "decoder.blocks." + std::to_string(l) + ".";
    DecLayer& L = w->dec[l];
    CCX_NEED(w->store, qw, p + "attn.query.weight", D, D); CCX_NEED(w->store, qbias, p + "attn.query.bias", D);
    CCX_NEED(w->store, kw, p + "attn.key.weight", D, D);
    CCX_NEED(w->store, vw, p + "attn.value.weight", D, D); CCX_NEED(w->store, vbias, p + "attn.value.bias", D);
    CCX_NEED(w->store, ow, p + "attn.out.weight", D, D); CCX_NEED(w->store, obias, p + "attn.out.bias", D);
    CCX_NEED(w->store, l1g, p + "attn_ln.weight", D); CCX_NEED(w->store, l1b, p + "attn_ln.bias", D);
    CCX_NEED(w->store, cqw, p + "cross_attn.query.weight", D, D); CCX_NEED(w->store, cqb, p + "cross_attn.query.bias", D);
    CCX_NEED(w->store, ckw, p + "cross_attn.key.weight", D, D);
    CCX_NEED(w->store, cvw, p + "cross_attn.value.weight", D, D); CCX_NEED(w->store, cvb, p + "cross_attn.value.bias", D);
    CCX_NEED(w->store, cow, p + "cross_attn.out.weight", D, D); CCX_NEED(w->store, cob, p + "cross_attn.out.bias", D);
    CCX_NEED(w->store, lcg, p + "cross_attn_ln.weight", D); CCX_NEED(w->store, lcb, p + "cross_attn_ln.bias", D);
    CCX_NEED(w->store, m0w, p + "mlp.0.weight", F, D); CCX_NEED(w->store, m0b, p + "mlp.0.bias", F);
    CCX_NEED(w->store, m2w, p + "mlp.2.weight", D, F); CCX_NEED(w->store, m2b, p + "mlp.2.bias", D);
    CCX_NEED(w->store, l2g, p + "mlp_ln.weight", D); CCX_NEED(w->store, l2b, p + "mlp_ln.bias", D);
    std::vector<float> wqkv = cat_rows({&qw->data, &kw->data, &vw->data});
    std::vector<float> bqkv = cat_rows({&qbias->data, &zerosD, &vbias->data});
    std::vector<float> wckv = cat_rows({&ckw->data, &cvw->data});
    std::vector<float> bckv = cat_rows({&zerosD, &cvb->data});
    CCX_TRY(up_bf16_packed(w, &L.Wqkv, wqkv.data(), 3 * D, D, 16)); CCX_TRY(w->store.upload(&L.bqkv, bqkv));
    CCX_TRY(up_bf16_packed(w, &L.Wo, ow->data.data(), D, D, 16)); CCX_TRY(w->store.upload(&L.bo, obias->data.data(), D));
    { double sb = 0.0; for (int k = 0; k < D; k++) sb += obias->data[k]; L.bo_mean = (float)(sb / D); }
    CCX_TRY(up_bf16_packed(w, &L.Wcq, cqw->data.data(), D, D, 16)); CCX_TRY(w->store.upload(&L.bcq, cqb->data.data(), D));
    CCX_TRY(w->store.upload_bf16(&L.Wckv, wckv)); CCX_TRY(w->store.upload(&L.bckv, bckv));
    CCX_TRY(up_bf16_packed(w, &L.Wco, cow->data.data(), D, D, 16)); CCX_TRY(w->store.upload(&L.bco, cob->data.data(), D));
    CCX_TRY(up_bf16_packed(w, &L.W1, m0w->data.data(), F, D, 16)); CCX_TRY(w->store.upload(&L.b1, m0b->data.data(), F));
    CCX_TRY(up_bf16_packed(w, &L.W2, m2w->data.data(), D, F, 16)); CCX_TRY(w->store.upload(&L.b2, m2b->data.data(), D));
    CCX_TRY(w->store.upload(&L.ln1_g, l1g->data.data(), D)); CCX_TRY(w->store.upload(&L.ln1_b, l1b->data.data(), D));
    CCX_TRY(w->store.upload(&L.lnc_g, lcg->data.data(), D)); CCX_TRY(w->store.upload(&L.lnc_b, lcb->data.data(), D));
    CCX_TRY(w->store.upload(&L.ln2_g, l2g->data.data(), D)); CCX_TRY(w->store.upload(&L.ln2_b, l2b->data.data(), D));
    if (w->xs_on) {
      std::vector<float> wkt((size_t)D * D);
      for (int hh = 0; hh < H; hh++)
        for (int f = 0; f < D; f++)
          for (int dd = 0; dd < 64; dd++) wkt[((size_t)hh * D + f) * 64 + dd] = ckw->data[(size_t)(hh * 64 + dd) * D + f];
      CCX_TRY(w->store.upload_bf16(&L.WckT, wkt));
      CCX_TRY(w->store.upload_bf16(&L.Wcq_plain, cqw->data));
      std::vector<float> Wg((size_t)D * D), sv(D), cv(D);
      for (int n = 0; n < D; n++) {
        double ss = 0.0, cc = 0.0;
        for (int k = 0; k < D; k++) {
          const float v = lcg->data[k] * cqw->data[(size_t)n * D + k];
          Wg[(size_t)n * D + k] = v;
          const uint32_t bits = (uint32_t)ccx_host_f32_to_bf16(v) << 16;
          float r;
          memcpy(&r, &bits, 4);
          ss += (double)r;
          cc += (double)lcb->data[k] * (double)cqw->data[(size_t)n * D + k];
        }
        sv[n] = (float)ss;
        cv[n] = (float)(cc + (double)cqb->data[n]);
      }
      CCX_TRY(w->store.upload_bf16(&L.Wcq_g, Wg)); CCX_TRY(w->store.upload(&L.scq, sv)); CCX_TRY(w->store.upload(&L.ccq, cv));
    }
    const size_t ck = (size_t)w->kv_cap * H * w->Spad * 64, sk = (size_t)B * H * Tc * 64;
    CCX_TRY(w->store.alloc(&L.crossK, ck, true)); CCX_TRY(w->store.alloc(&L.crossV, ck, true));
    CCX_TRY(w->store.alloc(&L.selfK, sk, true)); CCX_TRY(w->store.alloc(&L.selfV, sk, true));
  }
  w->store.staged.clear();

  if (ccx_whisper* dn = w->scratch_donor) {
    w->lm_raw = dn->lm_raw; w->lm_max = dn->lm_max; w->lm_n = dn->lm_n; w->lm_seek = dn->lm_seek; w->lm_seg = dn->lm_seg;
    w->im2col = dn->im2col; w->h1 = dn->h1; w->x = dn->x; w->xn = dn->xn;
    w->qb = dn->qb; w->kb = dn->kb; w->vtb = dn->vtb; w->attn = dn->attn; w->ffn = dn->ffn;
  } else {
    CCX_TRY(w->store.alloc(&w->lm_raw, (size_t)B * 80 * w->Fraw, true));
    CCX_TRY(w->store.alloc(&w->lm_max, (size_t)B, true));
    CCX_TRY(w->store.alloc(&w->lm_n, (size_t)B, true));
    CCX_TRY(w->store.alloc(&w->lm_seek, (size_t)B, true));
    CCX_TRY(w->store.alloc(&w->lm_seg, (size_t)B, true));
    CCX_TRY(w->store.alloc(&w->im2col, (size_t)B * 3000 * 256, true));
    CCX_TRY(w->store.alloc(&w->h1, ((size_t)B * 3002 + 2) * D, true));
    CCX_TRY(w->store.alloc(&w->x, (size_t)B * S * D, true));
    CCX_TRY(w->store.alloc(&w->xn, (size_t)B * S * D, true));
    CCX_TRY(w->store.alloc(&w->qb, (size_t)B * H * w->Spad * 64, true));
    CCX_TRY(w->store.alloc(&w->kb, (size_t)B * H * w->Spad * 64, true));
    CCX_TRY(w->store.alloc(&w->vtb, (size_t)B * H * 64 * w->Spad, true));
    CCX_TRY(w->store.alloc(&w->attn, (size_t)B * S * D, true));
    CCX_TRY(w->store.alloc(&w->ffn, (size_t)B * S * F, true));
  }

  CCX_TRY(w->store.alloc(&w->xa, ((size_t)B * S + 16) * D, true));
  if (w->xs_on) {
    CCX_TRY(w->store.alloc(&w->xq, (size_t)B * H * D, true));
    CCX_TRY(w->store.alloc(&w->pf_xq, (size_t)B * ccx_whisper::kPrefillMax * H * D, true));
    CCX_TRY(w->store.alloc(&w->xs_po, ccx_xs_part_o_elems(B, H, D), true));
    CCX_TRY(w->store.alloc(&w->xs_pml, ccx_xs_part_ml_elems(B), true));
    CCX_TRY(w->store.alloc(&w->pf_xs_po, ccx_xs_part_o_elems((size_t)B * ccx_whisper::kPrefillMax, H, D), true));
    CCX_TRY(w->store.alloc(&w->pf_xs_pml, ccx_xs_part_ml_elems((size_t)B * ccx_whisper::kPrefillMax), true));
    CCX_TRY(w->store.alloc(&w->dxb, (size_t)B * D, true));
    CCX_TRY(w->store.alloc(&w->pf_xb, (size_t)B * ccx_whisper::kPrefillMax * D, true));
    CCX_TRY(w->store.alloc(&w->dst2, (size_t)B * (D / 16), true));
    CCX_TRY(w->store.alloc(&w->pf_st2, (size_t)B * ccx_whisper::kPrefillMax * (D / 16), true));
    CCX_TRY(w->store.alloc(&w->dshift, (size_t)B, true));
    CCX_TRY(w->store.alloc(&w->pf_shift, (size_t)B * ccx_whisper::kPrefillMax, true));
  }
  CCX_TRY(w->store.alloc(&w->dx, (size_t)B * D, true));
  CCX_TRY(w->store.alloc(&w->dx2, (size_t)B * D, true));
  CCX_TRY(w->store.alloc(&w->pend, (size_t)4 * B * D, true));
  CCX_TRY(w->store.alloc(&w->dxn, (size_t)B * D, true));
  CCX_TRY(w->store.alloc(&w->dq, (size_t)B * D, true));
  CCX_TRY(w->store.alloc(&w->dattn, (size_t)B * D, true));
  CCX_TRY(w->store.alloc(&w->dffn, (size_t)B * F, true));
  CCX_TRY(w->store.alloc(&w->dlogits, (size_t)B * w->Vpad, true));
  CCX_TRY(w->store.alloc(&w->part_o, (size_t)B * H * ccx_whisper::kCrossSplitMax * 64, true));
  CCX_TRY(w->store.alloc(&w->part_ml, (size_t)B * H * ccx_whisper::kCrossSplitMax * 2, true));
  CCX_TRY(w->store.alloc(&w->cur_tok, (size_t)B, true));
  CCX_TRY(w->store.alloc(&w->pos, (size_t)B, true));
  CCX_TRY(w->store.alloc(&w->n_done, (size_t)ccx_whisper::kMaxLanes, true));
  CCX_TRY(w->store.alloc(&w->sample_cfg, (size_t)4, true));
  CCX_TRY(w->store.alloc(&w->state, (size_t)B, true));
  {
    const size_t R = (size_t)B * ccx_whisper::kPrefillMax;
    CCX_TRY(w->store.alloc(&w->pf_x, R * D, true)); CCX_TRY(w->store.alloc(&w->pf_x2, R * D, true)); CCX_TRY(w->store.alloc(&w->pf_pend, 4 * R * D, true));
    CCX_TRY(w->store.alloc(&w->pf_q, R * D, true)); CCX_TRY(w->store.alloc(&w->pf_xn, R * D, true)); CCX_TRY(w->store.alloc(&w->pf_attn, R * D, true));
    CCX_TRY(w->store.alloc(&w->pf_ffn, R * F, true));
    CCX_TRY(w->store.alloc(&w->pf_tok, R, true)); CCX_TRY(w->store.alloc(&w->pf_pos, R, true)); CCX_TRY(w->store.alloc(&w->pf_seq, R, true));
    CCX_TRY(w->store.alloc(&w->pf_last, (size_t)B, true));
  }
  w->max_prompt_cap = d.n_text_ctx;
  w->sample_cap = d.n_text_ctx;
  CCX_TRY(w->store.alloc(&w->prompt, (size_t)B * w->max_prompt_cap, true));
  CCX_TRY(w->store.alloc(&w->gen, (size_t)B * w->sample_cap, true));
  int prio_least = 0, prio_greatest = 0;
  CCX_HIP(w->ctx, hipDeviceGetStreamPriorityRange(&prio_least, &prio_greatest));
  CCX_HIP(w->ctx, hipStreamCreateWithPriority(&w->own_stream, hipStreamNonBlocking, prio_greatest));
  CCX_HIP(w->ctx, hipEventCreateWithFlags(&w->own_event, hipEventDisableTiming));
  for (int i = 0; i < ccx_whisper::kMaxLanes; i++) {
    CCX_HIP(w->ctx, hipEventCreateWithFlags(&w->lane_start[i], hipEventDisableTiming));
    CCX_HIP(w->ctx, hipEventCreateWithFlags(&w->lane_poll[0][i], hipEventDisableTiming));
    CCX_HIP(w->ctx, hipEventCreateWithFlags(&w->lane_poll[1][i], hipEventDisableTiming));
  }
  for (int i = 0; i < ccx_whisper::kLanePool; i++) CCX_HIP(w->ctx, hipStreamCreateWithPriority(&w->lane_pool[i], hipStreamNonBlocking, prio_greatest));
  CCX_TRY(w->store.alloc(&w->probe_sink, (size_t)64, true));
  CCX_TRY(w->store.alloc(&w->stamps, (size_t)ccx_whisper::kMaxLanes * ccx_whisper::kStampCap, true));
  CCX_TRY(w->store.alloc(&w->stamp_count, (size_t)ccx_whisper::kMaxLanes, true));
  if (const char* e = getenv("CCX_DEC_STAMPS")) {
    w->stamps_on = true;
    w->stamp_path = e;
    if (const char* l = getenv("CCX_DEC_STAMP_LEVEL")) w->stamp_level = atoi(l);
  }
  CCX_HIP(w->ctx, hipHostMalloc((void**)&w->poll_host, 2 * ccx_whisper::kMaxLanes * sizeof(int), 0));
  w->finalized = true;
  return CCX_OK;
}

static int scratch_acquire(ccx_whisper* w, hipStream_t stream) {
  ccx_whisper* root = w->scratch_donor ? w->scratch_donor : w;
  if (root->scratch_free) {
    ccx_whisper* owner = root->scratch_owner.load(std::memory_order_acquire);
    CCX_REQUIRE(w->ctx, owner == nullptr || owner == w,
                "whisper: the shared encoder workspaces hold another instance's staged windows -- issue its ccx_whisper_encode before this logmel / set_mel");
    root->scratch_owner.store(w, std::memory_order_release);
    CCX_HIP(w->ctx, hipStreamWaitEvent(stream, root->scratch_free, 0));
  }
  return CCX_OK;
}
static int scratch_release(ccx_whisper* w, hipStream_t stream) {
  ccx_whisper* root = w->scratch_donor ? w->scratch_donor : w;
  if (root->scratch_free) {
    CCX_HIP(w->ctx, hipEventRecord(root->scratch_free, stream));
    ccx_whisper* me = w;
    root->scratch_owner.compare_exchange_strong(me, nullptr, std::memory_order_acq_rel);
  }
  return CCX_OK;
}

int ccx_whisper_logmel(ccx_whisper* w, const float* audio, int64_t stride, const int* n_samples, const int* seek, int B,
                       float* mel_out, void* stream_) {
  if (!w) return CCX_ERR_ARG;
  hipStream_t stream = (hipStream_t)stream_;
  CCX_REQUIRE(w->ctx, w->finalized, "whisper: not finalized");
  CCX_REQUIRE(w->ctx, audio && n_samples && B >= 1 && B <= w->max_batch, "whisper_logmel: bad arguments (B=%d, max %d)", B, w->max_batch);
  CCX_TRY(scratch_acquire(w, stream));
  long fcomp = 32;
  for (int b = 0; b < B; b++) {
    CCX_REQUIRE(w->ctx, n_samples[b] >= 0 && n_samples[b] <= stride, "whisper_logmel: n_samples[%d]=%d exceeds stride", b, n_samples[b]);
    const int s = seek ? seek[b] : 0;
    const long need_frames = ((long)n_samples[b] + 200 + 159) / 160 + 1;
    CCX_REQUIRE(w->ctx, need_frames <= w->Fraw, "whisper_logmel: clip %d (%d samples) exceeds the configured maximum of %d frames (ccx_whisper_set_max_audio)", b, n_samples[b], w->Fraw);
    if (need_frames > fcomp) fcomp = need_frames;
    CCX_REQUIRE(w->ctx, s >= 0, "whisper_logmel: negative seek");
  }
  std::vector<int> seg(B), sk(B);
  for (int b = 0; b < B; b++) {
    sk[b] = seek ? seek[b] : 0;
    int sl = n_samples[b] / 160 - sk[b];
    seg[b] = sl < 0 ? 0 : (sl > 3000 ? 3000 : sl);
  }
  CCX_HIP(w->ctx, hipMemcpyAsync(w->lm_n, n_samples, B * 4, hipMemcpyHostToDevice, stream));
  CCX_HIP(w->ctx, hipMemcpyAsync(w->lm_seek, sk.data(), B * 4, hipMemcpyHostToDevice, stream));
  CCX_HIP(w->ctx, hipMemcpyAsync(w->lm_seg, seg.data(), B * 4, hipMemcpyHostToDevice, stream));
  CCX_HIP(w->ctx, hipStreamSynchronize(stream));
  fcomp = (fcomp + 31) / 32 * 32;
  return ccx_launch_logmel(w->ctx, w->lm, audio, stride, w->lm_n, w->lm_seek, w->lm_seg, B, w->Fraw, (int)fcomp, w->lm_raw,
                           w->lm_max, mel_out, w->im2col, stream);
}

__global__ void mel_to_im2col_kernel(const float* __restrict__ mel, bf16_t* __restrict__ im2col) {
  const int b = blockIdx.y, t = blockIdx.x * 4 + (threadIdx.x >> 8), k = threadIdx.x & 255;
  if (t >= 3000) return;
  float v = 0.f;
  if (k < 240) {
    const int tap = k / 80, c = k - tap * 80, fr = t - 1 + tap;
    if (fr >= 0 && fr < 3000) v = mel[((long)b * 80 + c) * 3000 + fr];
  }
  im2col[((long)b * 3000 + t) * 256 + k] = f32_to_bf16(v);
}

int ccx_whisper_set_mel(ccx_whisper* w, const float* mel, int B, void* stream_) {
  if (!w) return CCX_ERR_ARG;
  CCX_REQUIRE(w->ctx, w->finalized && mel && B >= 1 && B <= w->max_batch, "whisper_set_mel: bad arguments");
  CCX_TRY(scratch_acquire(w, (hipStream_t)stream_));
  hipLaunchKernelGGL(mel_to_im2col_kernel, dim3(750, B), dim3(1024), 0, (hipStream_t)stream_, mel, w->im2col);
  CCX_CHECK_LAUNCH(w->ctx);
  return CCX_OK;
}

static int project_cross_kv(ccx_whisper* w, int n, hipStream_t stream) {
  const ccx_whisper_dims& d = w->d;
  const int D = d.n_audio_state, S = d.n_audio_ctx, H = d.n_audio_head;
  CCX_REQUIRE(w->ctx, n <= w->kv_cap, "whisper: cross K/V caches hold %d sequences, %d asked for", w->kv_cap, n);
  GemmParams p;
  for (int l = 0; l < d.n_text_layer; l++) {
    const DecLayer& L = w->dec[l];
    memset(&p, 0, sizeof(p));
    p.A = w->xa; p.lda = D; p.W = L.Wckv; p.ldw = D; p.M = n * S; p.N = 2 * D; p.K = D; p.bias = L.bckv;
    p.hk = L.crossK; p.hv = L.crossV; p.d_model = D; p.n_head = H; p.S = S; p.Spad = w->Spad; p.v_transposed = 0;
    p.first_block = 1;
    CCX_TRY(ccx_launch_gemm(w->ctx, EPI_HEADS, p, stream));
  }
  w->kv_ready = n;
  return CCX_OK;
}
static void read_chain_switches(ccx_whisper* w) {
  { const char* e = getenv("CCX_FUSE_CROSS_Q"); w->fuse_cross_q = e ? (atoi(e) != 0) : 1; }
  { const char* e = getenv("CCX_DEC_LNFREE"); w->lnfree = !(e && strcmp(e, "0") == 0); }
  { const char* e = getenv("CCX_XS_FUSE_Q"); w->xs_fuse_q = !e || atoi(e) != 0; }
}
static int select_cross_path(ccx_whisper* w, int B, hipStream_t stream) {
  const char* e = getenv("CCX_CROSS_X_MIN_ROWS");
  const int min_rows = e ? atoi(e) : ccx_whisper::kKvSeqs + 1;
  w->xs_active = w->xs_on && (B >= min_rows || B > w->kv_cap);
  if (w->xs_on && !w->xs_active && w->kv_ready < B) CCX_TRY(project_cross_kv(w, B, stream));
  return CCX_OK;
}

int ccx_whisper_encode(ccx_whisper* w, int B, float* xa_out, void* stream_) {
  if (!w) return CCX_ERR_ARG;
  hipStream_t stream = (hipStream_t)stream_;
  ccx_ctx* ctx = w->ctx;
  CCX_REQUIRE(ctx, w->finalized, "whisper: not finalized");
  CCX_REQUIRE(ctx, B >= 1 && B <= w->max_batch, "whisper_encode: B=%d out of range (max %d)", B, w->max_batch);
  const ccx_whisper_dims& d = w->d;
  const int D = d.n_audio_state, F = 4 * D, S = d.n_audio_ctx, H = d.n_audio_head;
  GemmParams p;
  memset(&p, 0, sizeof(p));
  p.A = w->im2col; p.lda = 256; p.W = w->Wc1; p.ldw = 256; p.M = B * 3000; p.N = D; p.K = 256;
  p.bias = w->bc1; p.out = w->h1; p.ldo = D; p.rpb_in = 3000; p.rpb_out = 3002; p.roff = 1; p.rpb_valid = 3000;
  CCX_TRY(ccx_launch_gemm(ctx, EPI_BF16_GELU, p, stream));
  memset(&p, 0, sizeof(p));
  p.A = w->h1; p.lda = 2 * D; p.W = w->Wc2; p.ldw = 3 * D; p.M = B * 1501; p.N = D; p.K = 3 * D;
  p.bias = w->bc2; p.out = w->x; p.ldo = D; p.resid = w->enc_pos; p.ldr = D; p.resid_mod = S;
  p.rpb_in = 1501; p.rpb_out = S; p.roff = 0; p.rpb_valid = S;
  CCX_TRY(ccx_launch_gemm(ctx, EPI_F32_GELU_POS, p, stream));

  const int M = B * S;
  for (int l = 0; l < d.n_audio_layer; l++) {
    const EncLayer& L = w->enc[l];
    CCX_TRY(ccx_launch_layernorm(ctx, w->x, D, L.ln1_g, L.ln1_b, w->xn, nullptr, D, M, D, 1e-5f, stream));
    memset(&p, 0, sizeof(p));
    p.A = w->xn; p.lda = D; p.W = L.Wqkv; p.ldw = D; p.M = M; p.N = 3 * D; p.K = D; p.bias = L.bqkv;
    p.hq = w->qb; p.hk = w->kb; p.hv = w->vtb; p.d_model = D; p.n_head = H; p.S = S; p.Spad = w->Spad; p.v_transposed = 1;
    CCX_TRY(ccx_launch_gemm(ctx, EPI_HEADS, p, stream));
    CCX_TRY(ccx_launch_enc_attention(ctx, w->qb, w->kb, w->vtb, w->attn, B, H, S, w->Spad, stream));
    memset(&p, 0, sizeof(p));
    p.A = w->attn; p.lda = D; p.W = L.Wo; p.ldw = D; p.M = M; p.N = D; p.K = D; p.bias = L.bo;
    p.out = w->x; p.ldo = D; p.resid = w->x; p.ldr = D;
    CCX_TRY(ccx_launch_gemm(ctx, EPI_F32_RESID, p, stream));
    CCX_TRY(ccx_launch_layernorm(ctx, w->x, D, L.ln2_g, L.ln2_b, w->xn, nullptr, D, M, D, 1e-5f, stream));
    memset(&p, 0, sizeof(p));
    p.A = w->xn; p.lda = D; p.W = L.W1; p.ldw = D; p.M = M; p.N = F; p.K = D; p.bias = L.b1; p.out = w->ffn; p.ldo = F;
    CCX_TRY(ccx_launch_gemm(ctx, EPI_BF16_GELU, p, stream));
    memset(&p, 0, sizeof(p));
    p.A = w->ffn; p.lda = F; p.W = L.W2; p.ldw = F; p.M = M; p.N = D; p.K = F; p.bias = L.b2;
    p.out = w->x; p.ldo = D; p.resid = w->x; p.ldr = D;
    CCX_TRY(ccx_launch_gemm(ctx, EPI_F32_RESID, p, stream));
  }
  CCX_TRY(ccx_launch_layernorm(ctx, w->x, D, w->lnp_g, w->lnp_b, w->xa, xa_out, D, M, D, 1e-5f, stream));
  CCX_TRY(scratch_release(w, stream));
  w->kv_ready = 0;
  if (!w->xs_on) CCX_TRY(project_cross_kv(w, B, stream));
  return CCX_OK;
}

}

namespace {

__global__ void dec_stamp_kernel(unsigned long long* trace, int* count, int cap, int tag) {
  const int i = atomicAdd(count, 1);
  if (i < cap) trace[i] = (__builtin_amdgcn_s_memrealtime() << 8) | (unsigned long long)(tag & 255);
}

__global__ void lane_probe_spin(int* sink, long cycles) {
  const long t0 = __builtin_amdgcn_s_memtime();
  while (__builtin_amdgcn_s_memtime() - t0 < cycles) {}
  if (sink && threadIdx.x == 0) atomicAdd(sink, 1);
}

double lane_probe_time(ccx_whisper* w, hipStream_t a, hipStream_t b) {
  hipStreamSynchronize(a);
  if (b) hipStreamSynchronize(b);
  const auto t0 = std::chrono::steady_clock::now();
  for (int k = 0; k < 4; k++) {
    hipLaunchKernelGGL(lane_probe_spin, dim3(1), dim3(64), 0, a, w->probe_sink, 120000L);
    if (b) hipLaunchKernelGGL(lane_probe_spin, dim3(1), dim3(64), 0, b, w->probe_sink + 1, 120000L);
  }
  hipStreamSynchronize(a);
  if (b) hipStreamSynchronize(b);
  return std::chrono::duration<double, std::micro>(std::chrono::steady_clock::now() - t0).count();
}

const std::vector<hipStream_t>& lane_streams_for(ccx_whisper* w, hipStream_t s0, int want) {
  auto it = w->lane_sets.find(s0);
  if (it != w->lane_sets.end()) return it->second;
  (void)want;
  std::vector<hipStream_t>& set = w->lane_sets[s0];
  set.clear();
  lane_probe_time(w, s0, nullptr);
  double single = lane_probe_time(w, s0, nullptr);
  const double s2 = lane_probe_time(w, s0, nullptr);
  if (s2 < single) single = s2;
  for (int c = 0; c < ccx_whisper::kLanePool && (int)set.size() < ccx_whisper::kMaxLanes - 1; c++) {
    hipStream_t cand = w->lane_pool[c];
    bool ok = lane_probe_time(w, s0, cand) < 1.5 * single;
    for (size_t j = 0; ok && j < set.size(); j++) ok = lane_probe_time(w, set[j], cand) < 1.5 * single;
    if (ok) set.push_back(cand);
  }
  if (getenv("CCX_DEBUG_LANES")) fprintf(stderr, "[lanes] probe: single %.0f us, %zu concurrent streams found\n", single, set.size());
  return set;
}

int cross_split(int B, int H, bool lean) {
  if (lean && B > 16) return 1;
  int ns = ccx_cdiv(512, B * H);
  if (ns < 6) ns = 6;
  if (ns > ccx_whisper::kCrossSplitMax) ns = ccx_whisper::kCrossSplitMax;
  return ns;
}

int align_scores_hook(ccx_whisper* w, int l, const float* dq, int B, hipStream_t stream) {
  const AlignPass& a = *w->align_pass;
  if (a.count[l] == 0) return CCX_OK;
  AlignScoresParams p{dq, w->dec[l].crossK, w->d.n_text_head, w->Spad, a.heads + a.first[l], a.hsel + a.first[l], a.count[l], a.n_keys,
                      w->al_P, a.Hsel, a.T, a.Mmax, a.t};
  return ccx_launch_align_scores(w->ctx, p, B, stream);
}

int dec_head(ccx_whisper* w, int b0, int B, float* logits, long ld, bool select, int sample_len, int max_prompt, int* n_done,
             hipStream_t stream) {
  ccx_ctx* ctx = w->ctx;
  const ccx_whisper_dims& d = w->d;
  const int D = d.n_text_state;
  const long ro = b0;
  bf16_t* dxn = w->dxn + ro * D;
  int* pos = w->pos + b0;
  {
    GemmParams gp;
    memset(&gp, 0, sizeof(gp));
    gp.A = dxn; gp.lda = D; gp.W = w->tok_emb_rm; gp.ldw = D; gp.M = B; gp.N = d.n_vocab; gp.K = D; gp.out = logits; gp.ldo = ld;
    CCX_TRY(ccx_launch_gemm(ctx, EPI_F32, gp, stream));
  }
  if (select) {
    DecSelectParams sp;
    memset(&sp, 0, sizeof(sp));
    sp.logits = logits; sp.ld_logits = ld; sp.n_vocab = d.n_vocab; sp.state = w->state + b0; sp.prompt = w->prompt + ro * max_prompt;
    sp.max_prompt = max_prompt; sp.cur_tok = w->cur_tok + b0; sp.pos = pos; sp.gen = w->gen + ro * sample_len; sp.sample_len = sample_len;
    sp.n_done = n_done; sp.suppress_mask = w->suppress_mask; sp.eot = w->rules.eot; sp.blank = w->rules.blank;
    sp.no_speech = w->rules.no_speech; sp.timestamp_begin = w->rules.timestamp_begin;
    sp.max_initial_ts = w->rules.max_initial_timestamp_index;
    sp.tok_emb = w->tok_emb_f32; sp.pos_emb = w->dec_pos; sp.x = w->dx + ro * D; sp.D = D;
    sp.sample_cfg = w->sample_cfg; sp.row0 = b0; sp.sample = w->sampling ? 1 : 0;
    CCX_TRY(ccx_launch_dec_select(ctx, sp, B, stream));
  }
  return CCX_OK;
}

int dec_step(ccx_whisper* w, int b0, int B, float* logits, long ld, bool select, int sample_len, int max_prompt, int* n_done,
             hipStream_t stream, hipEvent_t stagger = nullptr, int lane_idx = 0, int prefill_rows = 0) {
  ccx_ctx* ctx = w->ctx;
  const ccx_whisper_dims& d = w->d;
  const int D = d.n_text_state, F = 4 * D, H = d.n_text_head, Tc = d.n_text_ctx;
  const float scale_log2e = 0.125f * 1.4426950408889634f;
  const int ns = cross_split(B, H, w->cross_stream != 0);
  long pstride = (long)B * D;
  const long ro = b0;
  const bool pre = prefill_rows > 0;
  const int nseq = B;
  if (pre) B = nseq * prefill_rows;
  pstride = (long)B * D;
  float* cur = pre ? w->pf_x : w->dx + ro * D;
  float* other = pre ? w->pf_x2 : w->dx2 + ro * D;
  float* pend = pre ? w->pf_pend : w->pend + 4 * ro * D;
  float* dq = pre ? w->pf_q : w->dq + ro * D;
  bf16_t* dxn = pre ? w->pf_xn : w->dxn + ro * D;
  bf16_t* dattn = pre ? w->pf_attn : w->dattn + ro * D;
  bf16_t* dffn = pre ? w->pf_ffn : w->dffn + ro * F;
  float* part_o = w->part_o + ro * H * ccx_whisper::kCrossSplitMax * 64;
  float* part_ml = w->part_ml + ro * H * ccx_whisper::kCrossSplitMax * 2;
  int* pos = pre ? w->pf_pos : w->pos + b0;
  const int* row_seq = pre ? w->pf_seq : nullptr;
  const long cross_off = ro * H * w->Spad * 64, self_off = ro * H * Tc * 64;
  const int stamp_level = w->stamp_level;
  auto stamp = [&](int tag, int level) {
    if (w->stamps_on && level <= stamp_level)
      hipLaunchKernelGGL(dec_stamp_kernel, dim3(1), dim3(1), 0, stream, w->stamps + (size_t)lane_idx * ccx_whisper::kStampCap,
                         w->stamp_count + lane_idx, ccx_whisper::kStampCap, tag);
  };
  int pend_n = 0;
  auto ln_linear = [&](int epi, const bf16_t* W, const float* bias, int N, const float* g, const float* bta, void* out, long ldo,
                       DecLinearParams* extra) -> int {
    DecLinearParams lp;
    if (extra) lp = *extra; else memset(&lp, 0, sizeof(lp));
    lp.M = B; lp.N = N; lp.K = D; lp.W = W; lp.ldw = D; lp.bias = bias; lp.out = out; lp.ldo = ldo;
    int rc;
    if (B > 16) {
      rc = ccx_launch_dec_resolve_ln(ctx, cur, pend, pend_n, pstride, g, bta, dxn, pend_n > 0 ? other : nullptr, B, D, 1e-5f, stream,
                                     lp.ln_mean_out);
      if (rc) return rc;
      lp.ln_mean_out = nullptr;
      lp.act = dxn; lp.lda = D;
      rc = ccx_launch_dec_linear(ctx, ACT_BF16, epi, lp, stream);
    } else {
      lp.x = cur; lp.pend = pend; lp.pend_n = pend_n; lp.pend_stride = pstride; lp.x_out = pend_n > 0 ? other : nullptr;
      lp.ln_g = g; lp.ln_b = bta; lp.eps = 1e-5f;
      rc = ccx_launch_dec_linear(ctx, ACT_LN, epi, lp, stream);
    }
    if (rc) return rc;
    if (pend_n > 0) { float* t = cur; cur = other; other = t; pend_n = 0; }
    return CCX_OK;
  };
  auto partial_linear = [&](int act, const bf16_t* W, const float* bias, int K, const bf16_t* a) -> int {
    DecLinearParams lp;
    memset(&lp, 0, sizeof(lp));
    lp.M = B; lp.N = D; lp.K = K; lp.W = W; lp.ldw = K; lp.bias = bias; lp.act = a; lp.lda = K;
    lp.part_o = part_o; lp.part_ml = part_ml; lp.nsplit = ns;
    lp.out = pend; lp.ldo = D; lp.pend_stride = pstride;
    int rc = ccx_launch_dec_linear(ctx, act, DEPI_PARTIAL, lp, stream);
    if (rc) return rc;
    pend_n = ccx_dec_linear_ksplit(K, DEPI_PARTIAL);
    return CCX_OK;
  };
  const bool lnfree = w->xs_active && w->lnfree;
  const bool xs_fused = w->xs_active && !lnfree && w->xs_fuse_q;
  const bool fuse_q = !w->xs_active && w->fuse_cross_q && !pre && B <= 16 && D == 768;
  const bool q_launch = !fuse_q && !lnfree && !xs_fused;
  bf16_t* xb = !lnfree ? nullptr : (pre ? w->pf_xb : w->dxb + ro * D);
  float2* st2 = !lnfree ? nullptr : (pre ? w->pf_st2 : w->dst2 + ro * (D / 16));
  float* shift = !lnfree ? nullptr : (pre ? w->pf_shift : w->dshift + ro);
  for (int l = 0; l < d.n_text_layer; l++) {
    const DecLayer& L = w->dec[l];
    {
      DecLinearParams ex;
      memset(&ex, 0, sizeof(ex));
      ex.cache_k = L.selfK + self_off; ex.cache_v = L.selfV + self_off; ex.cache_T = Tc; ex.pos = pos; ex.row_seq = row_seq;
      ex.ln_mean_out = shift;
      CCX_TRY(ln_linear(DEPI_SELF_QKV, L.Wqkv, L.bqkv, 3 * D, L.ln1_g, L.ln1_b, dq, D, &ex));
      stamp(16, 2);
    }
    DecAttnParams ap;
    memset(&ap, 0, sizeof(ap));
    ap.q = dq; ap.k = L.selfK + self_off; ap.v = L.selfV + self_off; ap.H = H; ap.kv_T = Tc; ap.pos = pos; ap.scale_log2e = scale_log2e;
    ap.out_bf16 = dattn; ap.row_seq = row_seq;
    CCX_TRY(ccx_launch_dec_attention(ctx, ap, B, 1, true, stream));
    stamp(17, 2);
    if (lnfree) {
      DecLinearParams lp;
      memset(&lp, 0, sizeof(lp));
      lp.M = B; lp.N = D; lp.K = D; lp.W = L.Wo; lp.ldw = D; lp.bias = L.bo; lp.act = dattn; lp.lda = D;
      lp.xres = cur; lp.xb = xb; lp.st_out = st2; lp.shift = shift; lp.shift_c = L.bo_mean;
      CCX_TRY(ccx_launch_dec_linear(ctx, ACT_BF16, DEPI_RESOLVE, lp, stream));
    } else {
      CCX_TRY(partial_linear(ACT_BF16, L.Wo, L.bo, D, dattn));
    }
    stamp(18, 2);
    if (q_launch) CCX_TRY(ln_linear(DEPI_F32, L.Wcq, L.bcq, D, L.lnc_g, L.lnc_b, dq, D, nullptr));
    if (w->align_pass) CCX_TRY(align_scores_hook(w, l, dq, B, stream));
    stamp(1, 1);
    if (l == 0 && stagger) CCX_HIP(ctx, hipEventRecord(stagger, stream));
    if (w->xs_active) {
      XsParams xp;
      memset(&xp, 0, sizeof(xp));
      if (lnfree) {
        xp.xb = xb; xp.ln_stats = st2; xp.ln_s = L.scq; xp.Wq = L.Wcq_g; xp.bq = L.ccq; xp.eps = 1e-5f;
      } else if (xs_fused) {
        xp.x = cur; xp.pend = pend; xp.pend_n = pend_n; xp.pend_stride = pstride; xp.x_out = pend_n > 0 ? other : nullptr;
        xp.ln_g = L.lnc_g; xp.ln_b = L.lnc_b; xp.eps = 1e-5f; xp.Wq = L.Wcq_plain; xp.bq = L.bcq;
      }
      xp.q = dq; xp.WkT = L.WckT; xp.xq = pre ? w->pf_xq : w->xq + ro * H * D;
      xp.part_o = pre ? w->pf_xs_po : w->xs_po + ccx_xs_part_o_elems(ro, H, D);
      xp.part_ml = pre ? w->pf_xs_pml : w->xs_pml + ccx_xs_part_ml_elems(ro);
      xp.X = pre ? w->xa : w->xa + ro * (long)d.n_audio_ctx * D; xp.x_seq_stride = (long)d.n_audio_ctx * D; xp.row_seq = row_seq;
      xp.Wv = L.Wckv + (long)D * D; xp.bv = L.bckv + D; xp.out = dattn;
      xp.rows = B; xp.H = H; xp.S = d.n_audio_ctx; xp.D = D; xp.scale_log2e = scale_log2e;
      xp.lds_pad = (w->cross_lds_pad > 0 && !pre) ? 65536 : 0;
      xp.rows_per_seq = pre ? prefill_rows : 0;
      CCX_TRY(ccx_launch_xs_cross_attention(ctx, xp, stream));
      if (xs_fused && pend_n > 0) { float* t = cur; cur = other; other = t; pend_n = 0; }
      stamp(2, 1);
      CCX_TRY(partial_linear(ACT_BF16, L.Wco, L.bco, D, dattn));
      stamp(19, 2);
    } else {
      memset(&ap, 0, sizeof(ap));
      ap.q = dq; ap.k = L.crossK + cross_off; ap.v = L.crossV + cross_off; ap.H = H; ap.kv_T = w->Spad; ap.pos = nullptr; ap.T = d.n_audio_ctx;
      ap.scale_log2e = scale_log2e; ap.part_o = part_o; ap.part_ml = part_ml; ap.out_bf16 = dattn;
      ap.lds_pad = w->cross_lds_pad;
      ap.stream_mode = (w->cross_stream && B > 16) ? 1 : 0;
      if (fuse_q) {
        ap.qx = cur; ap.q_pend = pend; ap.q_pend_n = pend_n; ap.q_pend_stride = pstride; ap.q_x_out = pend_n > 0 ? other : nullptr;
        ap.q_ln_g = L.lnc_g; ap.q_ln_b = L.lnc_b; ap.q_eps = 1e-5f; ap.q_W = L.Wcq; ap.q_bias = L.bcq; ap.q_K = D;
        CCX_TRY(ccx_launch_dec_cross_fused_q(ctx, ap, B, ns, stream));
        if (pend_n > 0) { float* t = cur; cur = other; other = t; pend_n = 0; }
        CCX_TRY(partial_linear(ACT_COMBINE, L.Wco, L.bco, D, nullptr));
      } else if (pre) {
        ap.row_seq = prefill_rows > 1 ? row_seq : nullptr; ap.rows_per_seq = prefill_rows > 1 ? prefill_rows : 0;
        ap.lds_pad = 0; ap.stream_mode = 1;
        CCX_TRY(ccx_launch_dec_attention(ctx, ap, nseq, 1, true, stream));
        CCX_TRY(partial_linear(ACT_BF16, L.Wco, L.bco, D, dattn));
      } else if (B > 16) {
        CCX_TRY(ccx_launch_dec_attention(ctx, ap, B, ns, ns == 1, stream));
        stamp(2, 1);
        if (ns > 1) CCX_TRY(ccx_launch_dec_combine(ctx, part_o, part_ml, ns, dattn, B, H, stream));
        CCX_TRY(partial_linear(ACT_BF16, L.Wco, L.bco, D, dattn));
        stamp(19, 2);
      } else {
// ... 123 lines not shown
    keys[b] = n_frames[b] / 2; nrows[b] = lens[b]; r1[b] = lens[b] - 1;
    for (int t = 0; t < lens[b]; t++) {
      const int32_t tok = tokens[(size_t)b * max_len + t];
      CCX_REQUIRE(ctx, tok >= 0 && tok < d.n_vocab, "ccx_whisper_align: tokens[%d][%d] = %d out of range [0, n_vocab = %d)", b, t, tok, d.n_vocab);
      padded[(size_t)b * T + t] = tok;
    }
  }
  AlignPass pass;
  pass.first.assign(L, 0); pass.count.assign(L, 0);
  std::vector<int> h_heads, h_hsel;
  for (int i = 0; i < n_heads; i++) {
    const int l = heads[2 * i], h = heads[2 * i + 1];
    CCX_REQUIRE(ctx, l >= 0 && l < L && h >= 0 && h < d.n_text_head, "ccx_whisper_align: heads[%d] = (layer %d, head %d) outside %d layers x %d heads", i, l, h, L,
                d.n_text_head);
    for (int j = 0; j < i; j++)
      CCX_REQUIRE(ctx, heads[2 * j] != l || heads[2 * j + 1] != h, "ccx_whisper_align: heads[%d] repeats heads[%d] = (layer %d, head %d)", i, j, l, h);
  }
  for (int l = 0; l < L; l++) {
    pass.first[l] = (int)h_heads.size();
    for (int i = 0; i < n_heads; i++)
      if (heads[2 * i] == l) { h_heads.push_back(heads[2 * i + 1]); h_hsel.push_back(i); }
    pass.count[l] = (int)h_heads.size() - pass.first[l];
  }
  const size_t seqs = (size_t)(w->max_batch < w->kv_cap ? w->max_batch : w->kv_cap);
  const size_t Tcap = (size_t)(d.n_text_ctx / 2 + 4 > T ? d.n_text_ctx / 2 + 4 : T);
  const size_t P_need = seqs * n_heads * Tcap * Mmax, A_need = seqs * Tcap * Mmax, tr_need = seqs * (Tcap + 1) * (Mmax + 1);
  const size_t path_cap = (size_t)T + Mmax;
  const size_t ints_need = 2 * (size_t)CCX_ALIGN_MAX_HEADS + seqs * (4 + 2 * (Tcap + Mmax) + Tcap);
  auto grow = [&](void** buf, size_t* have, size_t need_bytes) -> int {
    if (*have >= need_bytes) return CCX_OK;
    if (*buf) { CCX_HIP(ctx, hipStreamSynchronize(stream)); CCX_HIP(ctx, hipFree(*buf)); *buf = nullptr; *have = 0; }
    CCX_HIP(ctx, hipMalloc(buf, need_bytes));
    *have = need_bytes;
    return CCX_OK;
  };
  CCX_TRY(grow((void**)&w->al_P, &w->al_P_elems, P_need * sizeof(float)));
  CCX_TRY(grow((void**)&w->al_A, &w->al_A_elems, A_need * sizeof(float)));
  CCX_TRY(grow((void**)&w->al_trace, &w->al_trace_bytes, tr_need));
  CCX_TRY(grow((void**)&w->al_ints, &w->al_ints_elems, ints_need * sizeof(int)));
  int* i_heads = w->al_ints;
  int* i_hsel = i_heads + CCX_ALIGN_MAX_HEADS;
  int* i_keys = i_hsel + CCX_ALIGN_MAX_HEADS;
  int* i_rows = i_keys + seqs;
  int* i_r1 = i_rows + seqs;
  int* i_len = i_r1 + seqs;
  int* i_text = i_len + seqs;
  int* i_time = i_text + seqs * (Tcap + Mmax);
  int* i_jump = i_time + seqs * (Tcap + Mmax);
  CCX_HIP(ctx, hipMemcpyAsync(i_heads, h_heads.data(), (size_t)n_heads * 4, hipMemcpyHostToDevice, stream));
  CCX_HIP(ctx, hipMemcpyAsync(i_hsel, h_hsel.data(), (size_t)n_heads * 4, hipMemcpyHostToDevice, stream));
  CCX_HIP(ctx, hipMemcpyAsync(i_keys, keys.data(), (size_t)B * 4, hipMemcpyHostToDevice, stream));
  CCX_HIP(ctx, hipMemcpyAsync(i_rows, nrows.data(), (size_t)B * 4, hipMemcpyHostToDevice, stream));
  CCX_HIP(ctx, hipMemcpyAsync(i_r1, r1.data(), (size_t)B * 4, hipMemcpyHostToDevice, stream));
  CCX_HIP(ctx, hipMemsetAsync(w->al_A, 0, (size_t)B * T * Mmax * 4, stream));
  pass.heads = i_heads; pass.hsel = i_hsel; pass.n_keys = i_keys; pass.Hsel = n_heads; pass.T = T; pass.Mmax = Mmax;

  read_chain_switches(w);
  w->fuse_cross_q = 0;
  w->xs_active = false;
  if (w->kv_ready < B) CCX_TRY(project_cross_kv(w, B, stream));
  std::vector<int32_t> plens(B, T + 1);
  CCX_TRY(upload_decode_state(w, padded.data(), plens.data(), T, B, 0.f, 0, stream));
  w->cross_lds_pad = 0;
  w->cross_stream = 0;
  struct Guard { ccx_whisper* w; ~Guard() { w->align_pass = nullptr; } } guard{w};
  w->align_pass = &pass;
  for (int t = 0; t < T; t++) {
    pass.t = t;
    CCX_TRY(dec_step(w, 0, B, w->dlogits, w->Vpad, t + 1 < T, 1, T, w->n_done, stream));
  }
  w->align_pass = nullptr;
  AlignMatrixParams mp{w->al_P, w->al_A, n_heads, T, Mmax, i_rows, i_keys};
  CCX_TRY(ccx_launch_align_matrix(ctx, mp, B, stream));
  AlignDtwParams dp{w->al_A, T, Mmax, row0, i_r1, i_keys, w->al_trace, (long)((size_t)(T + 1) * (Mmax + 1)), i_text, i_time, (int)path_cap, i_len, i_jump};
  CCX_TRY(ccx_launch_align_dtw(ctx, dp, B, stream));
  if (probs_out_dev) CCX_HIP(ctx, hipMemcpyAsync(probs_out_dev, w->al_P, (size_t)B * n_heads * T * Mmax * 4, hipMemcpyDeviceToDevice, stream));
  if (matrix_out_dev) CCX_HIP(ctx, hipMemcpyAsync(matrix_out_dev, w->al_A, (size_t)B * T * Mmax * 4, hipMemcpyDeviceToDevice, stream));
  CCX_HIP(ctx, hipMemcpyAsync(jump_frame_out, i_jump, (size_t)B * T * 4, hipMemcpyDeviceToHost, stream));
  CCX_HIP(ctx, hipStreamSynchronize(stream));
  return CCX_OK;
}

int ccx_whisper_last_cross_path(ccx_whisper* w) { return w ? w->last_cross_path : -1; }

int ccx_whisper_prepare_lanes(ccx_whisper* w, void* stream_) {
  if (!w) return CCX_ERR_ARG;
  CCX_REQUIRE(w->ctx, w->finalized, "whisper: not finalized");
  hipStream_t stream = stream_ ? (hipStream_t)stream_ : w->own_stream;
  CCX_HIP(w->ctx, hipDeviceSynchronize());
  (void)lane_streams_for(w, stream, ccx_whisper::kMaxLanes - 1);
  return CCX_OK;
}

int ccx_whisper_decode_greedy(ccx_whisper* w, const int32_t* prompt_ids, const int32_t* prompt_lens, int max_prompt, int B,
                              int sample_len, int32_t* tokens_out, int32_t* n_tokens_out, float* sum_logprob_out,
                              float* no_speech_prob_out, void* stream_) {
  return ccx_whisper_decode(w, prompt_ids, prompt_lens, max_prompt, B, sample_len, 0.f, 0, tokens_out, n_tokens_out, sum_logprob_out,
                            no_speech_prob_out, stream_);
}

int ccx_whisper_decode(ccx_whisper* w, const int32_t* prompt_ids, const int32_t* prompt_lens, int max_prompt, int B, int sample_len,
                       float temperature, uint64_t seed, int32_t* tokens_out, int32_t* n_tokens_out, float* sum_logprob_out,
                       float* no_speech_prob_out, void* stream_) {
  if (!w) return CCX_ERR_ARG;
  CCX_REQUIRE(w->ctx, temperature >= 0.f && temperature == temperature, "decode: temperature must be >= 0");
  hipStream_t stream = (hipStream_t)stream_;
  ccx_ctx* ctx = w->ctx;
  CCX_REQUIRE(ctx, w->finalized && w->rules_set, "whisper: not finalized or rules not set");
  CCX_REQUIRE(ctx, prompt_ids && prompt_lens && tokens_out && B >= 1 && B <= w->max_batch, "decode_greedy: bad arguments");
  if (stream == nullptr) {
    CCX_HIP(ctx, hipEventRecord(w->own_event, nullptr));
    CCX_HIP(ctx, hipStreamWaitEvent(w->own_stream, w->own_event, 0));
    stream = w->own_stream;
  }
  CCX_REQUIRE(ctx, sample_len >= 1 && sample_len <= w->sample_cap && max_prompt >= 1 && max_prompt <= w->max_prompt_cap, "decode_greedy: sample_len/max_prompt out of range");
  int max_pl = 0;
  for (int b = 0; b < B; b++) {
    CCX_REQUIRE(ctx, prompt_lens[b] >= 1 && prompt_lens[b] <= max_prompt, "decode_greedy: prompt_lens[%d]=%d out of range", b, prompt_lens[b]);
    CCX_REQUIRE(ctx, prompt_lens[b] + sample_len - 1 <= w->d.n_text_ctx, "decode_greedy: prompt %d + sample_len %d exceeds n_text_ctx", prompt_lens[b], sample_len);
    for (int i = 0; i < prompt_lens[b]; i++) {
      const int t = prompt_ids[(size_t)b * max_prompt + i];
      CCX_REQUIRE(ctx, t >= 0 && t < w->d.n_vocab, "decode_greedy: prompt token %d out of range", t);
    }
    if (prompt_lens[b] > max_pl) max_pl = prompt_lens[b];
  }
  const int prefill_on = [] { const char* e = getenv("CCX_PREFILL"); return e ? atoi(e) : 1; }();
  const bool prefill = prefill_on && max_pl >= 2;
  read_chain_switches(w);
  CCX_TRY(select_cross_path(w, B, stream));
  CCX_TRY(upload_decode_state(w, prompt_ids, prompt_lens, max_prompt, B, temperature, seed, stream, prefill));
  const int total_steps = prefill ? sample_len : max_pl - 1 + sample_len;
  const bool use_graph = getenv("CCX_NO_GRAPH") == nullptr;
  const long ld = w->Vpad;

  int nl = 1;
  {
    const char* e = getenv("CCX_DEC_LANES");
    const int forced = e ? atoi(e) : 0;
    if (forced >= 1) nl = forced;
    else if (w->xs_on) nl = B >= 320 ? 3 : 1;
    else nl = B >= 640 ? 2 : (B >= 144 ? 3 : (B >= 96 ? 2 : 1));
    if (nl > ccx_whisper::kMaxLanes) nl = ccx_whisper::kMaxLanes;
    while (nl > 1 && B / nl < 16) nl--;
  }
  const std::vector<hipStream_t>* extra = nullptr;
  if (nl > 1) {
    extra = &lane_streams_for(w, stream, nl - 1);
    if ((int)extra->size() + 1 < nl) nl = (int)extra->size() + 1;
  }
  {
    w->cross_stream = 1;
    w->cross_lds_pad = nl > 1 ? 98304 : 0;
  }
  struct Lane { int b0, B; hipStream_t s; hipGraphExec_t exec; };
  Lane lanes[ccx_whisper::kMaxLanes];
  {
    const int per = ccx_cdiv(ccx_cdiv(B, nl), 16) * 16;
    int b0 = 0, n = 0;
    for (; n < nl && b0 < B; n++) {
      lanes[n].b0 = b0; lanes[n].B = (b0 + per <= B) ? per : B - b0;
      lanes[n].s = n == 0 ? stream : (*extra)[n - 1];
      lanes[n].exec = nullptr;
      b0 += lanes[n].B;
    }
    nl = n;
  }
  w->last_cross_path = w->xs_active ? 2 : ((w->cross_stream && lanes[0].B > 16) ? 1 : 0);
  if (prefill) {
    CCX_TRY(run_prefill(w, prompt_ids, prompt_lens, max_prompt, B, max_pl, sample_len, stream));
    for (int i = 0; i < nl; i++)
      CCX_TRY(dec_head(w, lanes[i].b0, lanes[i].B, w->dlogits + (long)lanes[i].b0 * ld, ld, true, sample_len, max_prompt, w->n_done + i, stream));
  }
  CCX_HIP(ctx, hipEventRecord(w->own_event, stream));
  for (int i = 1; i < nl; i++) CCX_HIP(ctx, hipStreamWaitEvent(lanes[i].s, w->own_event, 0));
  auto step_lane = [&](int i, hipEvent_t stagger) -> int {
    const Lane& L = lanes[i];
    return dec_step(w, L.b0, L.B, w->dlogits + (long)L.b0 * ld, ld, true, sample_len, max_prompt, w->n_done + i, L.s, stagger, i);
  };
  int step = prefill ? 1 : 0;
  if (step < total_steps) {
    for (int i = 0; i < nl; i++) {
      if (i > 0) CCX_HIP(ctx, hipStreamWaitEvent(lanes[i].s, w->lane_start[i - 1], 0));
      CCX_TRY(step_lane(i, (i + 1 < nl) ? w->lane_start[i] : nullptr));
      if (ctx->prof_on && !use_graph && nl > 1) CCX_HIP(ctx, hipStreamSynchronize(lanes[i].s));
    }
    step += 1;
  }
  if (use_graph && step < total_steps) {
    for (int i = 0; i < nl; i++) {
      const int ns_key = cross_split(lanes[i].B, w->d.n_text_head, w->cross_stream != 0);
      const int form = (w->fuse_cross_q ? 1 : 0) | ((w->xs_active ? 1 : 0) << 1) | ((w->xs_fuse_q ? 1 : 0) << 2) | ((w->lnfree ? 1 : 0) << 3);
      const std::array<int, 9> key = {lanes[i].b0, lanes[i].B, sample_len, max_prompt, w->sampling ? 1 : 0, ns_key, w->cross_lds_pad, form, i};
      auto it = w->graphs.find(key);
      if (it != w->graphs.end()) { lanes[i].exec = it->second; continue; }
      hipGraph_t graph = nullptr;
      hipGraphExec_t exec = nullptr;
      CCX_HIP(ctx, hipStreamBeginCapture(lanes[i].s, hipStreamCaptureModeThreadLocal));
      int rc = step_lane(i, nullptr);
      hipError_t e = hipStreamEndCapture(lanes[i].s, &graph);
      if (rc) { if (graph) hipGraphDestroy(graph); return rc; }
      if (e != hipSuccess) return ccx_fail(ctx, CCX_ERR_HIP, "hipStreamEndCapture: %s", hipGetErrorString(e));
      e = hipGraphInstantiate(&exec, graph, nullptr, nullptr, 0);
      hipGraphDestroy(graph);
      if (e != hipSuccess) return ccx_fail(ctx, CCX_ERR_HIP, "hipGraphInstantiate: %s", hipGetErrorString(e));
      w->graphs[key] = exec;
      lanes[i].exec = exec;
    }
  }
  const int kChunk = 8;
  auto queue_chunk = [&](int c, int n) -> int {
    for (int k = 0; k < n; k++)
      for (int i = 0; i < nl; i++) {
        if (lanes[i].exec) CCX_HIP(ctx, hipGraphLaunch(lanes[i].exec, lanes[i].s));
        else {
          CCX_TRY(step_lane(i, nullptr));
          if (ctx->prof_on && !use_graph && nl > 1) CCX_HIP(ctx, hipStreamSynchronize(lanes[i].s));
        }
      }
    for (int i = 0; i < nl; i++) {
      CCX_HIP(ctx, hipMemcpyAsync(&w->poll_host[(c & 1) * ccx_whisper::kMaxLanes + i], w->n_done + i, 4, hipMemcpyDeviceToHost, lanes[i].s));
      CCX_HIP(ctx, hipEventRecord(w->lane_poll[c & 1][i], lanes[i].s));
    }
    return CCX_OK;
  };
  auto chunk_done = [&](int c, bool* all) -> int {
    *all = true;
    for (int i = 0; i < nl; i++) {
      CCX_HIP(ctx, hipEventSynchronize(w->lane_poll[c & 1][i]));
      if (w->poll_host[(c & 1) * ccx_whisper::kMaxLanes + i] < lanes[i].B) *all = false;
    }
    return CCX_OK;
  };
  int c = 0;
  bool pending = false;
  while (step < total_steps) {
    const int n = (total_steps - step < kChunk) ? total_steps - step : kChunk;
    CCX_TRY(queue_chunk(c, n));
    step += n;
    if (pending) {
      bool all;
      CCX_TRY(chunk_done(c - 1, &all));
      if (all) break;
    }
    pending = true;
    c++;
  }
  for (int i = 1; i < nl; i++) {
    CCX_HIP(ctx, hipEventRecord(w->lane_start[i], lanes[i].s));
    CCX_HIP(ctx, hipStreamWaitEvent(stream, w->lane_start[i], 0));
  }
  if (w->stamps_on) {
    CCX_HIP(ctx, hipStreamSynchronize(stream));
    std::vector<int> cnt(ccx_whisper::kMaxLanes);
    CCX_HIP(ctx, hipMemcpy(cnt.data(), w->stamp_count, cnt.size() * 4, hipMemcpyDeviceToHost));
    if (FILE* f = fopen(w->stamp_path.c_str(), "a")) {
      fprintf(f, "decode B %d lanes %d\n", B, nl);
      for (int i = 0; i < nl; i++) {
        const int n = cnt[i] < ccx_whisper::kStampCap ? cnt[i] : ccx_whisper::kStampCap;
        std::vector<unsigned long long> buf(n);
        CCX_HIP(ctx, hipMemcpy(buf.data(), w->stamps + (size_t)i * ccx_whisper::kStampCap, (size_t)n * 8, hipMemcpyDeviceToHost));
        fprintf(f, "lane %d %d", i, n);
        for (int k = 0; k < n; k++) fprintf(f, " %llu", buf[k]);
        fprintf(f, "\n");
      }
      fclose(f);
    }
    CCX_HIP(ctx, hipMemset(w->stamp_count, 0, ccx_whisper::kMaxLanes * 4));
  }
  std::vector<DecSeqState> st(B);
  std::vector<int> gen((size_t)B * sample_len);
  CCX_HIP(ctx, hipMemcpyAsync(st.data(), w->state, B * sizeof(DecSeqState), hipMemcpyDeviceToHost, stream));
  CCX_HIP(ctx, hipMemcpyAsync(gen.data(), w->gen, gen.size() * 4, hipMemcpyDeviceToHost, stream));
  CCX_HIP(ctx, hipStreamSynchronize(stream));
  for (int b = 0; b < B; b++) {
    const int ng = st[b].n_gen < sample_len ? st[b].n_gen : sample_len;
    const int ntok = st[b].done ? st[b].n_tokens : ng;
    for (int i = 0; i < sample_len; i++) tokens_out[(size_t)b * sample_len + i] = (i < ntok) ? gen[(size_t)b * sample_len + i] : w->rules.eot;
    if (n_tokens_out) n_tokens_out[b] = ntok;
    if (sum_logprob_out) sum_logprob_out[b] = st[b].sum_logprob;
    if (no_speech_prob_out) no_speech_prob_out[b] = st[b].no_speech_prob;
  }
  return CCX_OK;
}

}
```

include/ccx.h:

```cpp
#ifndef CCX_H
#define CCX_H
#include <stdint.h>
#ifdef __cplusplus
extern "C" {
#endif

#define CCX_DTYPE_F32 0
#define CCX_DTYPE_BF16 1
#define CCX_DTYPE_F16 2

typedef struct ccx_ctx ccx_ctx;
typedef struct ccx_whisper ccx_whisper;

const char* ccx_version(void);
int ccx_ctx_create(int device, ccx_ctx** out);
void ccx_ctx_destroy(ccx_ctx* ctx);
const char* ccx_last_error(const ccx_ctx* ctx);

int ccx_prof_enable(ccx_ctx* ctx, int on);
int ccx_prof_count(ccx_ctx* ctx);
int ccx_prof_get(ccx_ctx* ctx, int i, char* name_out, int name_cap, double* flops, double* bytes, float* ms);


int ccx_gemm_bf16(ccx_ctx* ctx, int epi, const void* A_dev, int64_t lda, const void* W_dev, int64_t ldw,
                  const float* bias_dev, void* out_dev, int64_t ldo, const float* resid_dev, int64_t ldr,
                  int M, int N, int K, void* stream);

typedef struct ccx_gemm_desc {
  const void* A; const void* W;
  int64_t lda, ldw;
  int M, N, K;
  int ntaps; int64_t a_tap_stride;
  const void* bias;
  const void* out;
  int64_t ldo;
  const void* resid;
  int64_t ldr;
  int resid_mod;
  const void* scale; const void* shift;
  float slope;
  int rpb_in, rpb_out, roff, rpb_valid;
  int img_rows_in, img_rows_valid, img_rows_out;
  const void* resid_bf16; int64_t ldrb;
  const void* hq; const void* hk; const void* hv;
  int d_model, n_head;
  int S, Spad;
  int v_transposed;
  int first_block;
  int64_t a_elems, w_elems, out_elems, resid_elems, resid_bf16_elems, heads_elems;
} ccx_gemm_desc;

int ccx_gemm_bf16_desc(ccx_ctx* ctx, int epi, const ccx_gemm_desc* desc, void* stream);

int ccx_layernorm(ccx_ctx* ctx, const float* x_dev, const float* gamma_dev, const float* beta_dev,
                  void* out_bf16_dev, float* out_f32_dev, int M, int D, float eps, void* stream);

int ccx_gather_rows(ccx_ctx* ctx, const int64_t* src_ptrs_dev, const int* lens_dev, int n_rows, int max_len, float* dst_dev,
                    int64_t stride, void* stream);
int ccx_peak_normalize(ccx_ctx* ctx, const float* x_dev, float* y_dev, int64_t stride, const int* n_samples_dev, int B,
                       float eps, void* stream);
int ccx_cross_attention_xa(ccx_ctx* ctx, const float* q_dev, const float* wk_host, const float* wv_host, const float* bv_host,
                           const uint16_t* xa_dev, const int* row_seq_host, int rows_per_seq, int rows, int n_seq, int n_head, int n_ctx,
                           float* out_dev, void* stream);
int ccx_row_variance(ccx_ctx* ctx, const float* x_dev, int64_t stride, const int* n_samples_dev, int B, float* out_dev, void* stream);
int ccx_cosine_rows(ccx_ctx* ctx, const float* a_dev, const float* b_dev, int R, int D, int b_rows, float* out_dev, void* stream);
int ccx_speaker_profiles(ccx_ctx* ctx, const float* emb_dev, const float* w_dev, const int* spk_dev, int C, int T, int D, int S,
                         float* out_dev, void* stream);

int ccx_resample_sinc(ccx_ctx* ctx, const float* x_dev, int64_t stride_in, const int* n_in_dev, int B, int orig, int new_,
                      int width, const float* kernT_dev, float* y_dev, int64_t stride_out, const int* n_out_dev, int max_out,
                      void* stream);

int ccx_enc_attention(ccx_ctx* ctx, const void* q_dev, const void* k_dev, const void* vt_dev, void* o_dev,
                      int B, int H, int S, int Spad, void* stream);


typedef struct {
  int n_mels, n_audio_ctx, n_audio_state, n_audio_head, n_audio_layer;
  int n_vocab, n_text_ctx, n_text_state, n_text_head, n_text_layer;
} ccx_whisper_dims;

typedef struct {
  int eot, sot, sot_prev, no_speech, no_timestamps, timestamp_begin, blank;
  int max_initial_timestamp_index;
  int n_suppress;
  const int* suppress;
} ccx_decode_rules;

int ccx_whisper_create(ccx_ctx* ctx, const ccx_whisper_dims* dims, int max_batch, ccx_whisper** out);
void ccx_whisper_destroy(ccx_whisper* w);
int ccx_whisper_set_tensor(ccx_whisper* w, const char* name, const void* data, int dtype, int ndim,
                           const int64_t* shape);
int ccx_whisper_set_max_audio(ccx_whisper* w, double seconds);
int ccx_whisper_share_encoder_scratch(ccx_whisper* w, ccx_whisper* donor);
int ccx_whisper_finalize(ccx_whisper* w);
int ccx_whisper_set_rules(ccx_whisper* w, const ccx_decode_rules* rules);

int ccx_whisper_logmel(ccx_whisper* w, const float* audio_dev, int64_t stride, const int* n_samples,
                       const int* seek_frames, int B, float* mel_out_dev, void* stream);
int ccx_whisper_set_mel(ccx_whisper* w, const float* mel_dev, int B, void* stream);
int ccx_whisper_encode(ccx_whisper* w, int B, float* xa_out_dev, void* stream);

int ccx_whisper_decoder_logits(ccx_whisper* w, const int32_t* tokens, int B, int T, float* logits_dev,
                               void* stream);

int ccx_whisper_decode_greedy(ccx_whisper* w, const int32_t* prompt_ids, const int32_t* prompt_lens,
                              int max_prompt, int B, int sample_len, int32_t* tokens_out,
                              int32_t* n_tokens_out, float* sum_logprob_out, float* no_speech_prob_out,
                              void* stream);

int ccx_whisper_decode(ccx_whisper* w, const int32_t* prompt_ids, const int32_t* prompt_lens, int max_prompt, int B,
                       int sample_len, float temperature, uint64_t seed, int32_t* tokens_out, int32_t* n_tokens_out,
                       float* sum_logprob_out, float* no_speech_prob_out, void* stream);

#define CCX_DEC_ATTN_SELF 0
#define CCX_DEC_ATTN_SPLIT 1
#define CCX_DEC_ATTN_STREAM 2
#define CCX_DEC_ATTN_PREFILL 3
#define CCX_DEC_ATTN_FUSED_Q 4
#define CCX_DEC_ATTN_TWO_LAUNCH_Q 5

typedef struct ccx_dec_attn_desc {
  const void* q; const void* k; const void* v;
  int rows, n_seq, H, kv_T;
  int T;
  const int* pos;
  const int* row_seq;
  int rows_per_seq;
  int nsplit, combine;
  int lds_pad;
  const void* x; const void* pend; int pend_n; int64_t pend_stride;
  const void* ln_g; const void* ln_b; float eps;
  const float* wq_host; const void* bq;
  void* out; void* part_o; void* part_ml; void* q_x_out;
  int64_t q_elems, kv_elems, out_elems, part_o_elems, part_ml_elems, x_elems, pend_elems, q_x_out_elems;
} ccx_dec_attn_desc;

int ccx_dec_attention_desc(ccx_ctx* ctx, int form, const ccx_dec_attn_desc* desc, void* stream);

typedef struct ccx_dec_seq_state {
  int pos, prompt_len, n_gen, done;
  int last_tok, pen_tok, last_ts_tok, n_tokens;
  float sum_logprob, no_speech_prob;
} ccx_dec_seq_state;

typedef struct ccx_dec_select_desc {
  const void* logits; int64_t ld; int n_vocab; int B;
  const ccx_decode_rules* rules;
  ccx_dec_seq_state* state;
  const int* prompt; int max_prompt;
  int sample_len;
  int* gen;
  int* cur_tok; int* pos;
  int* n_done;
  const void* tok_emb; const void* pos_emb; void* x; int D;
  int sample; float temperature; uint64_t seed; int row0;
  int64_t logits_elems, tok_emb_elems, pos_emb_elems, x_elems;
} ccx_dec_select_desc;

int ccx_dec_select_step(ccx_ctx* ctx, const ccx_dec_select_desc* desc, void* stream);

#define CCX_ALIGN_SCORES 0
#define CCX_ALIGN_MATRIX 1
#define CCX_ALIGN_DTW 2

typedef struct ccx_align_desc {
  const void* q; const void* k;
  int64_t q_elems, k_elems;
  int n_seq, H, Spad;
  const int* heads; int n_heads; int head0;
  int t;
  int Hsel, T, Mmax;
  const int* n_keys;
  const int* n_rows;
  int r0;
  void* P; void* A;
  int64_t P_elems, A_elems;
  void* text_idx; void* time_idx; void* path_len; void* jump_frame;
  int64_t text_idx_elems, time_idx_elems, path_len_elems, jump_frame_elems;
} ccx_align_desc;

int ccx_align_op(ccx_ctx* ctx, int op, const ccx_align_desc* desc, void* stream);

int ccx_whisper_align(ccx_whisper* w, const int32_t* tokens, const int32_t* lens, int max_len, int B, const int32_t* n_frames,
                      const int32_t* heads, int n_heads, int row0, float* probs_out_dev, float* matrix_out_dev,
                      int32_t* jump_frame_out, void* stream);

int ccx_whisper_last_cross_path(ccx_whisper* w);

int ccx_whisper_prepare_lanes(ccx_whisper* w, void* stream);
int ccx_whisper_trace_lanes(ccx_whisper* w, const char* path, int level);


typedef struct ccx_sepformer ccx_sepformer;
typedef struct {
  int n_filters, kernel, stride, d_model, n_head, d_ffn, n_layers, n_blocks, segment, n_spk;
} ccx_sepformer_dims;

int ccx_sepformer_create(ccx_ctx* ctx, const ccx_sepformer_dims* dims, int max_tokens, int max_utts,
                         ccx_sepformer** out);
void ccx_sepformer_destroy(ccx_sepformer* s);
int ccx_sepformer_set_tensor(ccx_sepformer* s, const char* name, const float* data, int64_t numel);
int ccx_sepformer_finalize(ccx_sepformer* s);
int ccx_sepformer_separate(ccx_sepformer* s, const float* mix_dev, int64_t stride, const int* n_samples, int B,
                           float* out_dev, void* stream);

#define CCX_SEP_ATTN_BLOCK 0
#define CCX_SEP_ATTENTION 1
#define CCX_SEP_FFN 2
#define CCX_SEP_FINAL_NORM 3
#define CCX_SEP_DECODER 4

typedef struct ccx_sep_desc {
  void* h; const void* xin; void* y; const void* qkv; void* att; const void* feats; const void* fc;
  int64_t h_elems, xin_elems, y_elems, qkv_elems, att_elems, feats_elems, fc_elems;
  int rows;
  const int* seq_start; const int* seq_len; int n_seq;
  int n_tok, d_ffn;
  const void* ln_g; const void* ln_b; const void* gln_g; const void* gln_b;
  const void* wqkv; const void* bqkv; const void* wo; const void* bo;
  const void* w1; const void* b1; const void* w2; const void* b2; const void* wdec;
  int64_t ln_elems, gln_elems, wqkv_elems, bqkv_elems, wo_elems, bo_elems, w1_elems, b1_elems, w2_elems, b2_elems, wdec_elems;
  const int* utt_tok0; const int* utt_L; const int* utt_T; int n_utt; int segment;
  void* out; int64_t out_stride; int64_t out_elems;
} ccx_sep_desc;

int ccx_sep_op(ccx_ctx* ctx, int op, const ccx_sep_desc* desc, void* stream);


typedef struct ccx_speaker ccx_speaker;
int ccx_speaker_create(ccx_ctx* ctx, int kind, int n_classes, int powerset, int max_crops, int64_t max_samples,
                       ccx_speaker** out);
void ccx_speaker_destroy(ccx_speaker* s);
int ccx_speaker_set_tensor(ccx_speaker* s, const char* name, const float* data, int64_t numel);
int ccx_speaker_finalize(ccx_speaker* s);
int ccx_speaker_embed(ccx_speaker* s, const float* wav_dev, const int64_t* offsets, const int* n_samples, int n,
                      const float* weights_dev, const int64_t* w_offsets, const int* w_lens, float* out_dev, void* stream);
int ccx_speaker_segment(ccx_speaker* s, const float* wav_dev, const int64_t* offsets, const int* n_samples, int n,
                        float* out_dev, int64_t out_capacity_rows, int* frames_out, void* stream);

typedef struct ccx_resnet ccx_resnet;
int ccx_resnet_create(ccx_ctx* ctx, int max_chunks, int64_t max_samples, int max_masks, ccx_resnet** out);
void ccx_resnet_destroy(ccx_resnet* r);
int ccx_resnet_set_tensor(ccx_resnet* r, const char* name, const float* data, int64_t numel);
int ccx_resnet_finalize(ccx_resnet* r);
int ccx_resnet_embed(ccx_resnet* r, const float* wav_dev, int64_t stride, int n_samples, int n_chunks, const float* weights_dev,
                     int n_w, const int* mask_chunk, int n_masks, float* out_dev, void* stream);

typedef struct ccx_specgate ccx_specgate;
int ccx_specgate_create(ccx_ctx* ctx, int64_t max_samples, int max_clips, int sample_rate, ccx_specgate** out);
void ccx_specgate_destroy(ccx_specgate* g);
int ccx_specgate_reduce(ccx_specgate* g, const float* y_dev, int64_t stride, const int* n_samples, int B,
                        float prop_decrease, float* out_dev, void* stream);
int ccx_specgate_set_clip_noise(ccx_specgate* g, int on);
int ccx_specgate_reduce_long(ccx_specgate* g, const float* y_dev, int64_t n, float prop_decrease, float* out_dev, void* stream);

#ifdef __cplusplus
}
#endif
#endif
```

Baseline: 1647.

## Fuse logits GEMM epilogue with per-group max/sum records for greedy select

Adds an EPI_F32_LOGITS GEMM epilogue that, for text columns below eot's 128-column group, writes per-group masked max, argmax and exp-sum records. A new select kernel then reads only those records plus the tail of at most 2048 logits, instead of scanning the full vocabulary with a 1024-thread block. Decode graphs are captured in two variants (with and without records) and picked per step. The aim is to remove most of the full-vocab rescan in the per-token select; the cost is extra epilogue work in the GEMM and a second graph per lane.

```diff
diff --git a/clearconverse_amd/_lib.py b/clearconverse_amd/_lib.py
--- a/clearconverse_amd/_lib.py
+++ b/clearconverse_amd/_lib.py
@@ -77,6 +77,14 @@
         ("tok_emb", C.c_void_p), ("pos_emb", C.c_void_p), ("x", C.c_void_p), ("D", C.c_int),
         ("sample", C.c_int), ("temperature", C.c_float), ("seed", C.c_uint64), ("row0", C.c_int),
         ("logits_elems", C.c_int64), ("tok_emb_elems", C.c_int64), ("pos_emb_elems", C.c_int64), ("x_elems", C.c_int64)]
+
+
+class DecHeadDesc(C.Structure):
+    _fields_ = [
+        ("a", C.c_void_p), ("w", C.c_void_p), ("bias", C.c_void_p), ("K", C.c_int),
+        ("fused", C.c_int), ("run_select", C.c_int), ("rec", C.c_void_p), ("ld_rec", C.c_int64),
+        ("a_elems", C.c_int64), ("w_elems", C.c_int64), ("bias_elems", C.c_int64), ("rec_elems", C.c_int64),
+        ("sel", DecSelectDesc)]
 
 
 class SepDesc(C.Structure):
@@ -149,6 +157,7 @@
     "ccx_whisper_decode_greedy": (_i, [_vp, _i32p, _i32p, _i, _i, _i, _i32p, _i32p, _fp, _fp, _vp]),
     "ccx_dec_attention_desc": (_i, [_vp, _i, C.POINTER(DecAttnDesc), _vp]),
     "ccx_dec_select_step": (_i, [_vp, C.POINTER(DecSelectDesc), _vp]),
+    "ccx_dec_head_step": (_i, [_vp, C.POINTER(DecHeadDesc), _vp]),
     "ccx_align_op": (_i, [_vp, _i, C.POINTER(AlignDesc), _vp]),
     "ccx_whisper_align": (_i, [_vp, _i32p, _i32p, _i, _i, _i32p, _i32p, _i, _i, _vp, _vp, _i32p, _vp]),
     "ccx_whisper_last_cross_path": (_i, [_vp]),
diff --git a/clearconverse_amd/csrc/dec_ops.hip b/clearconverse_amd/csrc/dec_ops.hip
--- a/clearconverse_amd/csrc/dec_ops.hip
+++ b/clearconverse_amd/csrc/dec_ops.hip
@@ -1,6 +1,7 @@
 #include "../../include/ccx.h"
 #include "ccx_common.h"
 #include "decoder.h"
+#include "gemm_bf16.h"
 #include "op_scratch.h"
 
 static_assert(sizeof(ccx_dec_seq_state) == sizeof(DecSeqState), "ccx_dec_seq_state mirrors DecSeqState field for field");
@@ -147,10 +148,7 @@
   return rc;
 }
 
-extern "C" int ccx_dec_select_step(ccx_ctx* ctx, const ccx_dec_select_desc* d, void* stream_) {
-  if (!ctx) return CCX_ERR_ARG;
-  hipStream_t stream = (hipStream_t)stream_;
-  CCX_REQUIRE(ctx, d != nullptr, "ccx_dec_select_step: desc is NULL");
+static int select_step(ccx_ctx* ctx, const ccx_dec_select_desc* d, const float4* rec, long ld_rec, int rec_c0, hipStream_t stream) {
   const int V = d->n_vocab, B = d->B, D = d->D;
   CCX_REQUIRE(ctx, B >= 1 && B <= 65536, "ccx_dec_select_step: B = %d out of range", B);
   CCX_REQUIRE(ctx, V >= 4 && V % 4 == 0 && V <= 13 * 4096, "ccx_dec_select_step: n_vocab = %d must be a multiple of 4 and <= 53248", V);
@@ -218,6 +216,7 @@
   sp.max_initial_ts = r.max_initial_timestamp_index;
   sp.tok_emb = (const float*)d->tok_emb; sp.pos_emb = (const float*)d->pos_emb; sp.x = (float*)d->x; sp.D = D;
   sp.sample_cfg = d_cfg; sp.row0 = d->row0; sp.sample = d->sample;
+  sp.rec = rec; sp.ld_rec = ld_rec; sp.rec_c0 = rec_c0;
   CCX_TRY(ccx_launch_dec_select(ctx, sp, B, stream));
   DO_HIP(hipStreamSynchronize(stream));
   DO_HIP(hipMemcpy(gen_h.data(), d_gen, gen_h.size() * 4, hipMemcpyDeviceToHost));
@@ -228,6 +227,59 @@
   DO_HIP(hipMemcpy(d->cur_tok, d_cur, (size_t)B * 4, hipMemcpyDeviceToHost));
   DO_HIP(hipMemcpy(d->pos, d_pos, (size_t)B * 4, hipMemcpyDeviceToHost));
   DO_HIP(hipMemcpy(d->n_done, d_ndone, 4, hipMemcpyDeviceToHost));
+  return CCX_OK;
+}
+
+extern "C" int ccx_dec_select_step(ccx_ctx* ctx, const ccx_dec_select_desc* d, void* stream_) {
+  if (!ctx) return CCX_ERR_ARG;
+  CCX_REQUIRE(ctx, d != nullptr, "ccx_dec_select_step: desc is NULL");
+  return select_step(ctx, d, nullptr, 0, 0, (hipStream_t)stream_);
+}
+
+extern "C" int ccx_dec_head_step(ccx_ctx* ctx, const ccx_dec_head_desc* d, void* stream_) {
+  if (!ctx) return CCX_ERR_ARG;
+  hipStream_t stream = (hipStream_t)stream_;
+  CCX_REQUIRE(ctx, d != nullptr, "ccx_dec_head_step: desc is NULL");
+  const ccx_dec_select_desc& sd = d->sel;
+  const int V = sd.n_vocab, B = sd.B, K = d->K;
+  CCX_REQUIRE(ctx, d->fused == 0 || d->fused == 1, "ccx_dec_head_step: fused = %d must be 0 or 1", d->fused);
+  CCX_REQUIRE(ctx, d->run_select == 0 || d->run_select == 1, "ccx_dec_head_step: run_select = %d must be 0 or 1", d->run_select);
+  CCX_REQUIRE(ctx, B >= 1 && B <= 65536, "ccx_dec_head_step: sel.B = %d out of range", B);
+  CCX_REQUIRE(ctx, V >= 4 && V % 4 == 0 && V <= 13 * 4096, "ccx_dec_head_step: sel.n_vocab = %d must be a multiple of 4 and <= 53248", V);
+  CCX_REQUIRE(ctx, K >= 64 && K % 64 == 0 && K <= 8192, "ccx_dec_head_step: K = %d must be a multiple of 64 in [64, 8192]", K);
+  CCX_REQUIRE(ctx, d->a && d->w && ccx_aligned16(d->a) && ccx_aligned16(d->w), "ccx_dec_head_step: a / w null or not 16-byte aligned");
+  CCX_REQUIRE(ctx, (int64_t)B * K <= d->a_elems, "ccx_dec_head_step: a is read up to element %ld, a_elems=%ld", (long)B * K, (long)d->a_elems);
+  CCX_REQUIRE(ctx, (int64_t)V * K <= d->w_elems, "ccx_dec_head_step: w is read up to element %ld, w_elems=%ld", (long)V * K, (long)d->w_elems);
+  CCX_REQUIRE(ctx, !d->bias || V <= d->bias_elems, "ccx_dec_head_step: bias is read up to element %d, bias_elems=%ld", V, (long)d->bias_elems);
+  const int64_t Vw = ((int64_t)V + 15) / 16 * 16;
+  CCX_REQUIRE(ctx, sd.logits && ccx_aligned16(sd.logits), "ccx_dec_head_step: sel.logits null or not 16-byte aligned");
+  CCX_REQUIRE(ctx, sd.ld >= Vw && sd.ld % 8 == 0, "ccx_dec_head_step: sel.ld = %ld must be a multiple of 8 and cover n_vocab rounded up to 16", (long)sd.ld);
+  CCX_REQUIRE(ctx, (int64_t)(B - 1) * sd.ld + Vw <= sd.logits_elems, "ccx_dec_head_step: sel.logits are written up to element %ld, logits_elems=%ld",
+              (long)((int64_t)(B - 1) * sd.ld + Vw), (long)sd.logits_elems);
+  CCX_REQUIRE(ctx, sd.rules != nullptr, "ccx_dec_head_step: sel.rules is NULL");
+  std::vector<unsigned char> mask;
+  CCX_TRY(ccx_build_suppress_mask(ctx, "ccx_dec_head_step", sd.rules, V, mask));
+  const int c0 = sd.rules->eot / 128 * 128;
+  const long ng = c0 / 128;
+  if (d->fused) {
+    CCX_REQUIRE(ctx, sd.sample == 0, "ccx_dec_head_step: the fused head is greedy (sel.sample = %d)", sd.sample);
+    CCX_REQUIRE(ctx, d->rec && ccx_aligned16(d->rec), "ccx_dec_head_step: rec null or not 16-byte aligned");
+    CCX_REQUIRE(ctx, d->ld_rec >= ng, "ccx_dec_head_step: ld_rec = %ld below the %ld records of a row", (long)d->ld_rec, ng);
+    CCX_REQUIRE(ctx, ((int64_t)(B - 1) * d->ld_rec + ng) * 4 <= d->rec_elems, "ccx_dec_head_step: rec is written up to element %ld, rec_elems=%ld",
+                (long)(((int64_t)(B - 1) * d->ld_rec + ng) * 4), (long)d->rec_elems);
+    CCX_REQUIRE(ctx, !d->run_select || V - c0 <= kSelTailMax, "ccx_dec_head_step: %d logits from eot's group on, the select takes %d", V - c0, (int)kSelTailMax);
+  }
+  ccx_op_scratch sc;
+  unsigned char* d_mask = nullptr;
+  DO_HIP(sc.upload(&d_mask, mask.data(), mask.size()));
+  GemmParams gp;
+  memset(&gp, 0, sizeof(gp));
+  gp.A = (const bf16_t*)d->a; gp.lda = K; gp.W = (const bf16_t*)d->w; gp.ldw = K; gp.M = B; gp.N = V; gp.K = K;
+  gp.bias = (const float*)d->bias; gp.out = (void*)sd.logits; gp.ldo = (long)sd.ld;
+  if (d->fused) { gp.rec = (float4*)d->rec; gp.ld_rec = (long)d->ld_rec; gp.col_mask = d_mask; gp.rec_c0 = c0; }
+  CCX_TRY(ccx_launch_gemm(ctx, d->fused ? EPI_F32_LOGITS : EPI_F32, gp, stream));
+  DO_HIP(hipStreamSynchronize(stream));
+  if (!d->run_select) return CCX_OK;
+  return select_step(ctx, &sd, d->fused ? (const float4*)d->rec : nullptr, (long)d->ld_rec, c0, stream);
 #undef DO_HIP
-  return CCX_OK;
-}
+}
diff --git a/clearconverse_amd/csrc/decoder.h b/clearconverse_amd/csrc/decoder.h
--- a/clearconverse_amd/csrc/decoder.h
+++ b/clearconverse_amd/csrc/decoder.h
@@ -66,7 +66,9 @@
   const float* tok_emb; const float* pos_emb; float* x; int D;
   const unsigned* sample_cfg; int row0;
   int sample;
+  const float4* rec; long ld_rec; int rec_c0;
 };
+enum { kSelTailMax = 2048 };
 int ccx_launch_dec_select(ccx_ctx* ctx, const DecSelectParams& p, int B, hipStream_t stream);
 int ccx_launch_dec_embed(ccx_ctx* ctx, const float* tok_emb, const float* pos_emb, const int* cur_tok, const int* pos,
                          float* x, int B, int D, hipStream_t stream);
diff --git a/clearconverse_amd/csrc/decoder.hip b/clearconverse_amd/csrc/decoder.hip
--- a/clearconverse_amd/csrc/decoder.hip
+++ b/clearconverse_amd/csrc/decoder.hip
@@ -1219,6 +1219,173 @@
   if (sh_next[0] >= 0) embed_next(sh_next[0], sh_next[1]);
 }
 
+__global__ __launch_bounds__(256) void dec_select_records_kernel(DecSelectParams p) {
+  __shared__ float sh[16];
+  __shared__ float sh_v[16];
+  __shared__ int sh_i[16];
+  __shared__ int sh_next[2];
+  const int b = blockIdx.x, tid = threadIdx.x;
+  const int V = p.n_vocab, c0 = p.rec_c0;
+  const float* lg = p.logits + (long)b * p.ld_logits;
+  DecSeqState s = p.state[b];
+  __syncthreads();
+
+  auto embed_next = [&](int tok, int pos) {
+    const float4* te = (const float4*)(p.tok_emb + (long)tok * p.D);
+    const float4* pe = (const float4*)(p.pos_emb + (long)pos * p.D);
+    float4* xo = (float4*)(p.x + (long)b * p.D);
+    for (int i = tid; i < p.D / 4; i += blockDim.x) {
+      const float4 a = te[i], c = pe[i];
+      xo[i] = make_float4(a.x + c.x, a.y + c.y, a.z + c.z, a.w + c.w);
+    }
+  };
+  if (s.pos < s.prompt_len - 1) {
+    const int np = s.pos + 1;
+    const int tok = p.prompt[(long)b * p.max_prompt + np];
+    embed_next(tok, np);
+    if (tid == 0) {
+      s.pos = np;
+      p.cur_tok[b] = tok;
+      p.pos[b] = np;
+      p.state[b] = s;
+    }
+    return;
+  }
+  if (s.done) {
+    if (tid == 0 && s.n_gen < p.sample_len) {
+      p.gen[(long)b * p.sample_len + s.n_gen] = p.eot;
+      s.n_gen += 1;
+      p.state[b] = s;
+    }
+    return;
+  }
+
+  constexpr int TV4 = kSelTailMax / 1024, RPT = 2;
+  float val[TV4 * 4];
+  unsigned sup = 0;
+#pragma unroll
+  for (int i = 0; i < TV4; i++) {
+    const int v0 = c0 + tid * 4 + i * 1024;
+    if (v0 + 3 < V) {
+      const float4 f = *(const float4*)(lg + v0);
+      const uchar4 m = *(const uchar4*)(p.suppress_mask + v0);
+      val[4 * i] = f.x; val[4 * i + 1] = f.y; val[4 * i + 2] = f.z; val[4 * i + 3] = f.w;
+      sup |= (unsigned)((m.x ? 1 : 0) | (m.y ? 2 : 0) | (m.z ? 4 : 0) | (m.w ? 8 : 0)) << (4 * i);
+    } else {
+      val[4 * i] = val[4 * i + 1] = val[4 * i + 2] = val[4 * i + 3] = -INFINITY;
+      sup |= 0xFu << (4 * i);
+    }
+  }
+  const int i_gen = s.n_gen;
+  const int tsb = p.timestamp_begin;
+  const bool last_ts = i_gen >= 1 && s.last_tok >= tsb;
+  const bool pen_ts = i_gen < 2 || s.pen_tok >= tsb;
+  int s_lo = tsb;
+  if (s.last_ts_tok >= 0) s_lo = (last_ts && !pen_ts) ? s.last_ts_tok : s.last_ts_tok + 1;
+  int s_hi = V;
+  if (i_gen == 0 && p.max_initial_ts >= 0) s_hi = tsb + p.max_initial_ts + 1;
+  if (last_ts && pen_ts) s_hi = s_lo;
+  const int t_lo = (i_gen == 0) ? tsb : ((last_ts && !pen_ts) ? p.eot : 0);
+  const int ng = (t_lo == 0) ? c0 / 128 : 0;
+  float4 rc[RPT];
+#pragma unroll
+  for (int k = 0; k < RPT; k++) {
+    const int g = tid + k * 256;
+    rc[k] = g < ng ? p.rec[(long)b * p.ld_rec + g] : make_float4(-INFINITY, __int_as_float(-1), 0.f, 0.f);
+  }
+
+  float mx_text = -INFINITY, mx_ts = -INFINITY;
+  int am_text = 0x7fffffff, am_ts = 0x7fffffff;
+#pragma unroll
+  for (int k = 0; k < RPT; k++) {
+    const int ri = __float_as_int(rc[k].y);
+    if (ri >= 0 && rc[k].x > mx_text) { mx_text = rc[k].x; am_text = ri; }
+  }
+#pragma unroll
+  for (int i = 0; i < TV4 * 4; i++) {
+    const int v = c0 + tid * 4 + (i >> 2) * 1024 + (i & 3);
+    const bool is_text = v < tsb;
+    const bool allowed = !((sup >> i) & 1) && (is_text ? (v >= t_lo) : (v >= s_lo && v < s_hi));
+    const float x = allowed ? val[i] : -INFINITY;
+    val[i] = x;
+    const bool bt_ = is_text && x > mx_text, bs_ = !is_text && x > mx_ts;
+    mx_text = bt_ ? x : mx_text; am_text = bt_ ? v : am_text;
+    mx_ts = bs_ ? x : mx_ts; am_ts = bs_ ? v : am_ts;
+  }
+  auto block_argmax = [&](float v_, int idx, float& oval, int& oidx) {
+#pragma unroll
+    for (int o = 32; o > 0; o >>= 1) {
+      const float ov = __shfl_xor(v_, o, 64);
+      const int oi = __shfl_xor(idx, o, 64);
+      if (ov > v_ || (ov == v_ && oi < idx)) { v_ = ov; idx = oi; }
+    }
+    __syncthreads();
+    if ((tid & 63) == 0) { sh_v[tid >> 6] = v_; sh_i[tid >> 6] = idx; }
+    __syncthreads();
+    oval = sh_v[0]; oidx = sh_i[0];
+    for (int w = 1; w < (int)(blockDim.x >> 6); w++)
+      if (sh_v[w] > oval || (sh_v[w] == oval && sh_i[w] < oidx)) { oval = sh_v[w]; oidx = sh_i[w]; }
+  };
+  float bt, bs; int it, is;
+  block_argmax(mx_text, am_text, bt, it);
+  block_argmax(mx_ts, am_ts, bs, is);
+  const float mx_all = fmaxf(bt, bs);
+
+  float se_text = 0.f, se_ts = 0.f;
+#pragma unroll
+  for (int k = 0; k < RPT; k++)
+    se_text += rc[k].z > 0.f ? rc[k].z * __builtin_amdgcn_exp2f((rc[k].x - mx_all) * 1.4426950408889634f) : 0.f;
+#pragma unroll
+  for (int i = 0; i < TV4 * 4; i++) {
+    const int v = c0 + tid * 4 + (i >> 2) * 1024 + (i & 3);
+    const float e = __builtin_amdgcn_exp2f((val[i] - mx_all) * 1.4426950408889634f);
+    se_text += (v < tsb) ? e : 0.f;
+    se_ts += (v < tsb) ? 0.f : e;
+  }
+  se_text = block_reduce_sum(se_text, sh);
+  se_ts = block_reduce_sum(se_ts, sh);
+  const float lse_ts = (se_ts > 0.f) ? mx_all + logf(se_ts) : -INFINITY;
+  const bool force_ts = lse_ts > bt;
+  const float lnorm = logf(force_ts ? se_ts : se_text + se_ts);
+
+  if (tid == 0) {
+    int next; float logprob;
+    if (force_ts) {
+      next = is;
+      logprob = (bs - mx_all) - lnorm;
+    } else {
+      if (bt > bs || (bt == bs && it < is)) next = it; else next = is;
+      logprob = -lnorm;
+    }
+    s.sum_logprob += logprob;
+    p.gen[(long)b * p.sample_len + i_gen] = next;
+    s.n_gen = i_gen + 1;
+    s.pen_tok = s.last_tok;
+    s.last_tok = next;
+    if (next >= tsb) s.last_ts_tok = next;
+    int cont = 0;
+    if (next == p.eot) {
+      s.done = 1;
+      s.n_tokens = i_gen;
+      atomicAdd(p.n_done, 1);
+    } else if (s.n_gen >= p.sample_len) {
+      s.done = 1;
+      s.n_tokens = s.n_gen;
+      atomicAdd(p.n_done, 1);
+    } else {
+      s.pos += 1;
+      p.cur_tok[b] = next;
+      p.pos[b] = s.pos;
+      cont = 1;
+    }
+    p.state[b] = s;
+    sh_next[0] = cont ? next : -1;
+    sh_next[1] = s.pos;
+  }
+  __syncthreads();
+  if (sh_next[0] >= 0) embed_next(sh_next[0], sh_next[1]);
+}
+
 int ccx_launch_dec_embed(ccx_ctx* ctx, const float* tok_emb, const float* pos_emb, const int* cur_tok, const int* pos,
                          float* x, int B, int D, hipStream_t stream) {
   hipLaunchKernelGGL(dec_embed_kernel, dim3(B), dim3(192), 0, stream, tok_emb, pos_emb, cur_tok, pos, x, D);
@@ -1227,6 +1394,16 @@
 }
 
 int ccx_launch_dec_select(ccx_ctx* ctx, const DecSelectParams& p, int B, hipStream_t stream) {
+  if (p.rec) {
+    CCX_REQUIRE(ctx, !p.sample, "dec_select: the selection from records is greedy only");
+    CCX_REQUIRE(ctx, p.rec_c0 >= 0 && p.rec_c0 % 128 == 0 && p.rec_c0 <= p.eot && p.rec_c0 / 128 <= 512 && p.ld_rec >= p.rec_c0 / 128,
+                "dec_select: rec_c0=%d must be a multiple of 128 in [0, eot=%d] (<= 512 records), ld_rec=%ld", p.rec_c0, p.eot, p.ld_rec);
+    CCX_REQUIRE(ctx, p.n_vocab - p.rec_c0 <= kSelTailMax, "dec_select: %d logits behind rec_c0, at most %d", p.n_vocab - p.rec_c0, (int)kSelTailMax);
+    ccx_prof_scope ps(ctx, stream, "dec_select_records_kernel", 0.0, (double)B * ((p.n_vocab - p.rec_c0) * 5.0 + p.rec_c0 / 128 * 16.0));
+    hipLaunchKernelGGL(dec_select_records_kernel, dim3(B), dim3(256), 0, stream, p);
+    CCX_CHECK_LAUNCH(ctx);
+    return CCX_OK;
+  }
   ccx_prof_scope ps(ctx, stream, "dec_select_kernel", 0.0, (double)B * p.n_vocab * 5.0);
   if (p.sample) hipLaunchKernelGGL(dec_select_kernel<true>, dim3(B), dim3(1024), 0, stream, p);
   else hipLaunchKernelGGL(dec_select_kernel<false>, dim3(B), dim3(1024), 0, stream, p);
diff --git a/clearconverse_amd/csrc/gemm_bf16.h b/clearconverse_amd/csrc/gemm_bf16.h
--- a/clearconverse_amd/csrc/gemm_bf16.h
+++ b/clearconverse_amd/csrc/gemm_bf16.h
@@ -10,7 +10,8 @@
   EPI_BF16_RELU = 5,
   EPI_F32_GELU_POS = 6,
   EPI_BF16_LRELU_AFFINE = 7,
-  EPI_BF16_ADD_RELU = 8
+  EPI_BF16_ADD_RELU = 8,
+  EPI_F32_LOGITS = 9
 };
 
 struct GemmParams {
@@ -35,6 +36,9 @@
   int S, Spad;
   int v_transposed;
   int first_block;
+  float4* rec; long ld_rec;
+  const unsigned char* col_mask;
+  int rec_c0;
 };
 
 __host__ __device__ inline long ccx_gemm_remap_row(const GemmParams& p, int m, bool& valid) {
@@ -51,3 +55,4 @@
 }
 
 int ccx_launch_gemm(ccx_ctx* ctx, int epi, const GemmParams& p, hipStream_t stream);
+int ccx_gemm_prepare_logits(ccx_ctx* ctx);
diff --git a/clearconverse_amd/csrc/gemm_bf16.hip b/clearconverse_amd/csrc/gemm_bf16.hip
--- a/clearconverse_amd/csrc/gemm_bf16.hip
+++ b/clearconverse_amd/csrc/gemm_bf16.hip
@@ -36,7 +36,7 @@
 __device__ __forceinline__ void epi_store16f(void* dst, float4 v) { *(float4*)dst = v; }
 __device__ __forceinline__ float4 epi_load16f(const float* src) { return *(const float4*)src; }
 
-constexpr int colmap_of(int epi) { return (epi == EPI_F32 || epi == EPI_F32_RESID || epi == EPI_F32_GELU_POS) ? 1 : 2; }
+constexpr int colmap_of(int epi) { return (epi == EPI_F32 || epi == EPI_F32_RESID || epi == EPI_F32_GELU_POS || epi == EPI_F32_LOGITS) ? 1 : 2; }
 
 template <bool SWAP, int CM, int WM, int WN, int MT>
 __device__ __forceinline__ void gemm_mainloop(const GemmParams& p, char* smem, int m0, int n0, f32x4 (&acc)[MT][4]) {
@@ -189,6 +189,61 @@
   }
 #pragma unroll
   for (int i = 0; i < 16; i++) asm volatile("" ::"v"(bias[i]));
+
+  if constexpr (EPI == EPI_F32_LOGITS) {
+    static_assert(WN * 64 == 128 && WM * WN * 64 >= WM * MT * 16, "a record is one 128-column tile row, merged by one thread per row");
+    if (n0 < p.rec_c0) {
+      constexpr float kLog2e = 1.4426950408889634f;
+      unsigned mk[4];
+#pragma unroll
+      for (int j = 0; j < 4; j++) mk[j] = *(const unsigned*)(p.col_mask + c4[j]);
+      float4* sm = (float4*)smem;
+#pragma unroll
+      for (int mt = 0; mt < MT; mt++) {
+        float x[16];
+        float m = -INFINITY; int idx = 0x7fffffff;
+#pragma unroll
+        for (int j = 0; j < 4; j++)
+#pragma unroll
+          for (int r = 0; r < 4; r++) {
+            const bool ok = ((mk[j] >> (8 * r)) & 0xffu) == 0;
+            const float v = ok ? acc[mt][j][r] + bias[4 * j + r] : -INFINITY;
+            x[4 * j + r] = v;
+            if (ok && (v > m || idx == 0x7fffffff)) { m = v; idx = c4[j] + r; }
+          }
+#pragma unroll
+        for (int o = 16; o <= 32; o <<= 1) {
+          const float om = __shfl_xor(m, o, 64);
+          const int oi = __shfl_xor(idx, o, 64);
+          if (om > m || (om == m && oi < idx)) { m = om; idx = oi; }
+        }
+        float s = 0.f;
+#pragma unroll
+        for (int i = 0; i < 16; i++) s += (x[i] == -INFINITY) ? 0.f : __builtin_amdgcn_exp2f((x[i] - m) * kLog2e);
+        s += __shfl_xor(s, 16, 64);
+        s += __shfl_xor(s, 32, 64);
+        if (h == 0) sm[wc * (WM * MT * 16) + wr * MT * 16 + mt * 16 + l15] = make_float4(m, __int_as_float(idx), s, 0.f);
+      }
+      __syncthreads();
+      const int row = threadIdx.x;
+      if (row < WM * MT * 16 && m0 + row < p.M) {
+        float4 a = sm[row];
+#pragma unroll
+        for (int c = 1; c < WN; c++) {
+          const float4 b = sm[c * (WM * MT * 16) + row];
+          const int ai = __float_as_int(a.y), bi = __float_as_int(b.y);
+          const float m = fmaxf(a.x, b.x);
+          const float sa = a.z > 0.f ? a.z * __builtin_amdgcn_exp2f((a.x - m) * kLog2e) : 0.f;
+          const float sb = b.z > 0.f ? b.z * __builtin_amdgcn_exp2f((b.x - m) * kLog2e) : 0.f;
+          const bool take_b = b.x > a.x || (b.x == a.x && bi < ai);
+          a = make_float4(m, take_b ? b.y : a.y, sa + sb, 0.f);
+        }
+        if (__float_as_int(a.y) == 0x7fffffff) a.y = __int_as_float(-1);
+        p.rec[(long)(m0 + row) * p.ld_rec + n0 / (WN * 64)] = a;
+      }
+      return;
+    }
+  }
 
   constexpr bool RES_F32 = (EPI == EPI_F32_RESID || EPI == EPI_F32_GELU_POS || EPI == EPI_BF16_LRELU_AFFINE);
   constexpr bool RES_BF16 = (EPI == EPI_BF16_ADD_RELU);
@@ -566,15 +621,21 @@
 }
 
 template <int EPI, int WM, int WN, int MT>
+static hipError_t optin_epi_geo(ccx_ctx* ctx) {
+  static ccx_lds_optin optin;
+  return optin.ensure(ctx->device, (const void*)gemm_bf16_nt_kernel<EPI, WM, WN, MT>, 2 * (WM * MT * 16 + WN * 64) * 128);
+}
+
+template <int EPI, int WM, int WN, int MT>
 static int launch_epi_geo(ccx_ctx* ctx, const GemmParams& p, hipStream_t stream) {
   constexpr int TBM = WM * MT * 16, TBN = WN * 64;
   constexpr int LDS = 2 * (TBM + TBN) * 128;
   const int tiles = ccx_cdiv(p.M, TBM) * ccx_cdiv(p.N, TBN);
-  static ccx_lds_optin optin;
-  CCX_HIP(ctx, optin.ensure(ctx->device, (const void*)gemm_bf16_nt_kernel<EPI, WM, WN, MT>, LDS));
+  CCX_HIP(ctx, (optin_epi_geo<EPI, WM, WN, MT>(ctx)));
   {
-    const double obytes = (EPI == EPI_F32 || EPI == EPI_F32_RESID || EPI == EPI_F32_GELU_POS) ? 4.0 : 2.0;
+    const double obytes = (EPI == EPI_F32 || EPI == EPI_F32_RESID || EPI == EPI_F32_GELU_POS || EPI == EPI_F32_LOGITS) ? 4.0 : 2.0;
     const double kt = (double)p.K * (p.ntaps > 1 ? p.ntaps : 1);
+    const double ocols = EPI == EPI_F32_LOGITS ? (double)(p.N - p.rec_c0) + p.rec_c0 / 128 * 4.0 : (double)p.N;
     const bool by_shape = ctx->prof_on && getenv("CCX_PROF_SHAPES") != nullptr;
     const char* label = "gemm_bf16_nt_kernel";
     if (by_shape) {
@@ -586,7 +647,7 @@
       label = names.emplace(buf, buf).first->second.c_str();
     }
     ccx_prof_scope ps(ctx, stream, label, 2.0 * p.M * (double)p.N * kt,
-                      2.0 * ((double)p.M * p.K + (double)p.N * kt) + obytes * p.M * (double)p.N);
+                      2.0 * ((double)p.M * p.K + (double)p.N * kt) + obytes * p.M * ocols);
     hipLaunchKernelGGL((gemm_bf16_nt_kernel<EPI, WM, WN, MT>), dim3(tiles), dim3(WM * WN * 64), LDS, stream, p);
   }
   CCX_CHECK_LAUNCH(ctx);
@@ -630,6 +691,11 @@
   return launch_epi_geo<EPI, 2, 2, 4>(ctx, p, stream);
 }
 
+int ccx_gemm_prepare_logits(ccx_ctx* ctx) {
+  CCX_HIP(ctx, (optin_epi_geo<EPI_F32_LOGITS, 2, 2, 4>(ctx)));
+  return CCX_OK;
+}
+
 int ccx_launch_gemm(ccx_ctx* ctx, int epi, const GemmParams& p, hipStream_t stream) {
   CCX_REQUIRE(ctx, p.M > 0 && p.N > 0 && p.K > 0, "gemm: empty problem M=%d N=%d K=%d", p.M, p.N, p.K);
   CCX_REQUIRE(ctx, p.K % BK == 0, "gemm: K=%d must be a multiple of %d", p.K, BK);
@@ -681,6 +747,12 @@
     case EPI_F32_GELU_POS: return launch_epi<EPI_F32_GELU_POS>(ctx, p, stream);
     case EPI_BF16_LRELU_AFFINE: return launch_epi<EPI_BF16_LRELU_AFFINE>(ctx, p, stream);
     case EPI_BF16_ADD_RELU: return launch_epi<EPI_BF16_ADD_RELU>(ctx, p, stream);
+    case EPI_F32_LOGITS:
+      CCX_REQUIRE(ctx, p.rec_c0 >= 0 && p.rec_c0 % 128 == 0 && p.rec_c0 <= p.N, "gemm logits: rec_c0=%d must be a multiple of 128 in [0, N]", p.rec_c0);
+      CCX_REQUIRE(ctx, p.rec_c0 == 0 || (p.rec && ((uintptr_t)p.rec & 15) == 0 && p.ld_rec >= p.rec_c0 / 128), "gemm logits: rec null, not 16-byte aligned or ld_rec=%ld below rec_c0 / 128", p.ld_rec);
+      CCX_REQUIRE(ctx, p.rec_c0 == 0 || (p.col_mask && ((uintptr_t)p.col_mask & 3) == 0), "gemm logits: col_mask null or not 4-byte aligned");
+      CCX_REQUIRE(ctx, p.rpb_in <= 0 && p.ntaps <= 1, "gemm logits: no row remap, no taps");
+      return launch_epi_geo<EPI_F32_LOGITS, 2, 2, 4>(ctx, p, stream);
   }
   return ccx_fail(ctx, CCX_ERR_ARG, "gemm: unknown epilogue %d", epi);
 }
diff --git a/clearconverse_amd/csrc/whisper.hip b/clearconverse_amd/csrc/whisper.hip
--- a/clearconverse_amd/csrc/whisper.hip
+++ b/clearconverse_amd/csrc/whisper.hip
@@ -95,6 +95,9 @@
   float *dshift = nullptr, *pf_shift = nullptr;
   bool lnfree = true;
   float *xs_po = nullptr, *xs_pml = nullptr, *pf_xs_po = nullptr, *pf_xs_pml = nullptr;
+  bool head_rec_on = true, head_rec = false;
+  float4* drec = nullptr;
+  long rec_ld = 0;
   static constexpr int kLanePool = 8;
   hipStream_t lane_pool[kLanePool] = {};
   std::map<hipStream_t, std::vector<hipStream_t>> lane_sets;
@@ -462,6 +465,8 @@
   CCX_TRY(w->store.alloc(&w->dattn, (size_t)B * D, true));
   CCX_TRY(w->store.alloc(&w->dffn, (size_t)B * F, true));
   CCX_TRY(w->store.alloc(&w->dlogits, (size_t)B * w->Vpad, true));
+  w->rec_ld = w->Vpad / 128;
+  CCX_TRY(w->store.alloc(&w->drec, (size_t)B * w->rec_ld, true));
   CCX_TRY(w->store.alloc(&w->part_o, (size_t)B * H * ccx_whisper::kCrossSplitMax * 64, true));
   CCX_TRY(w->store.alloc(&w->part_ml, (size_t)B * H * ccx_whisper::kCrossSplitMax * 2, true));
   CCX_TRY(w->store.alloc(&w->cur_tok, (size_t)B, true));
@@ -593,6 +598,8 @@
   return CCX_OK;
 }
 static void read_chain_switches(ccx_whisper* w) {
+  { const char* e = getenv("CCX_DEC_HEAD_FUSED"); w->head_rec_on = !(e && strcmp(e, "0") == 0); }
+  w->head_rec = false;
   { const char* e = getenv("CCX_FUSE_CROSS_Q"); w->fuse_cross_q = e ? (atoi(e) != 0) : 1; }
   { const char* e = getenv("CCX_DEC_LNFREE"); w->lnfree = !(e && strcmp(e, "0") == 0); }
   { const char* e = getenv("CCX_XS_FUSE_Q"); w->xs_fuse_q = !e || atoi(e) != 0; }
@@ -725,11 +732,18 @@
   const long ro = b0;
   bf16_t* dxn = w->dxn + ro * D;
   int* pos = w->pos + b0;
+  const bool rec = w->head_rec && select;
+  const int rec_c0 = w->rules.eot / 128 * 128;
   {
     GemmParams gp;
     memset(&gp, 0, sizeof(gp));
     gp.A = dxn; gp.lda = D; gp.W = w->tok_emb_rm; gp.ldw = D; gp.M = B; gp.N = d.n_vocab; gp.K = D; gp.out = logits; gp.ldo = ld;
-    CCX_TRY(ccx_launch_gemm(ctx, EPI_F32, gp, stream));
+    if (rec) {
+      gp.rec = w->drec + ro * w->rec_ld; gp.ld_rec = w->rec_ld; gp.col_mask = w->suppress_mask; gp.rec_c0 = rec_c0;
+      CCX_TRY(ccx_launch_gemm(ctx, EPI_F32_LOGITS, gp, stream));
+    } else {
+      CCX_TRY(ccx_launch_gemm(ctx, EPI_F32, gp, stream));
+    }
   }
   if (select) {
     DecSelectParams sp;
@@ -741,6 +755,7 @@
     sp.max_initial_ts = w->rules.max_initial_timestamp_index;
     sp.tok_emb = w->tok_emb_f32; sp.pos_emb = w->dec_pos; sp.x = w->dx + ro * D; sp.D = D;
     sp.sample_cfg = w->sample_cfg; sp.row0 = b0; sp.sample = w->sampling ? 1 : 0;
+    if (rec) { sp.rec = w->drec + ro * w->rec_ld; sp.ld_rec = w->rec_ld; sp.rec_c0 = rec_c0; }
     CCX_TRY(ccx_launch_dec_select(ctx, sp, B, stream));
   }
   return CCX_OK;
@@ -1170,7 +1185,7 @@
     w->cross_stream = 1;
     w->cross_lds_pad = nl > 1 ? 98304 : 0;
   }
-  struct Lane { int b0, B; hipStream_t s; hipGraphExec_t exec; };
+  struct Lane { int b0, B; hipStream_t s; hipGraphExec_t exec[2]; };
   Lane lanes[ccx_whisper::kMaxLanes];
   {
     const int per = ccx_cdiv(ccx_cdiv(B, nl), 16) * 16;
@@ -1178,7 +1193,7 @@
     for (; n < nl && b0 < B; n++) {
       lanes[n].b0 = b0; lanes[n].B = (b0 + per <= B) ? per : B - b0;
       lanes[n].s = n == 0 ? stream : (*extra)[n - 1];
-      lanes[n].exec = nullptr;
+      lanes[n].exec[0] = lanes[n].exec[1] = nullptr;
       b0 += lanes[n].B;
     }
     nl = n;
@@ -1189,6 +1204,11 @@
     for (int i = 0; i < nl; i++)
       CCX_TRY(dec_head(w, lanes[i].b0, lanes[i].B, w->dlogits + (long)lanes[i].b0 * ld, ld, true, sample_len, max_prompt, w->n_done + i, stream));
   }
+  const bool head_rec_ok = w->head_rec_on && !w->sampling && w->xs_active && w->d.n_vocab - w->rules.eot / 128 * 128 <= kSelTailMax;
+  std::vector<char> rec_step(total_steps, head_rec_ok ? 1 : 0);
+  if (!prefill)
+    for (int b = 0; b < B; b++) rec_step[prompt_lens[b] - 1] = 0;
+  if (head_rec_ok) CCX_TRY(ccx_gemm_prepare_logits(ctx));
   CCX_HIP(ctx, hipEventRecord(w->own_event, stream));
   for (int i = 1; i < nl; i++) CCX_HIP(ctx, hipStreamWaitEvent(lanes[i].s, w->own_event, 0));
   auto step_lane = [&](int i, hipEvent_t stagger) -> int {
@@ -1197,6 +1217,7 @@
   };
   int step = prefill ? 1 : 0;
   if (step < total_steps) {
+    w->head_rec = rec_step[step] != 0;
     for (int i = 0; i < nl; i++) {
       if (i > 0) CCX_HIP(ctx, hipStreamWaitEvent(lanes[i].s, w->lane_start[i - 1], 0));
       CCX_TRY(step_lane(i, (i + 1 < nl) ? w->lane_start[i] : nullptr));
@@ -1204,13 +1225,17 @@
     }
     step += 1;
   }
-  if (use_graph && step < total_steps) {
+  for (int rec = 0; rec < 2; rec++) {
+    bool needed = false;
+    for (int t = step; t < total_steps; t++) needed = needed || rec_step[t] == rec;
+    if (!use_graph || !needed) continue;
+    w->head_rec = rec != 0;
     for (int i = 0; i < nl; i++) {
       const int ns_key = cross_split(lanes[i].B, w->d.n_text_head, w->cross_stream != 0);
-      const int form = (w->fuse_cross_q ? 1 : 0) | ((w->xs_active ? 1 : 0) << 1) | ((w->xs_fuse_q ? 1 : 0) << 2) | ((w->lnfree ? 1 : 0) << 3);
+      const int form = (w->fuse_cross_q ? 1 : 0) | ((w->xs_active ? 1 : 0) << 1) | ((w->xs_fuse_q ? 1 : 0) << 2) | ((w->lnfree ? 1 : 0) << 3) | ((w->head_rec ? 1 : 0) << 4);
       const std::array<int, 9> key = {lanes[i].b0, lanes[i].B, sample_len, max_prompt, w->sampling ? 1 : 0, ns_key, w->cross_lds_pad, form, i};
       auto it = w->graphs.find(key);
-      if (it != w->graphs.end()) { lanes[i].exec = it->second; continue; }
+      if (it != w->graphs.end()) { lanes[i].exec[rec] = it->second; continue; }
       hipGraph_t graph = nullptr;
       hipGraphExec_t exec = nullptr;
       CCX_HIP(ctx, hipStreamBeginCapture(lanes[i].s, hipStreamCaptureModeThreadLocal));
@@ -1222,14 +1247,16 @@
       hipGraphDestroy(graph);
       if (e != hipSuccess) return ccx_fail(ctx, CCX_ERR_HIP, "hipGraphInstantiate: %s", hipGetErrorString(e));
       w->graphs[key] = exec;
-      lanes[i].exec = exec;
+      lanes[i].exec[rec] = exec;
     }
   }
   const int kChunk = 8;
-  auto queue_chunk = [&](int c, int n) -> int {
+  auto queue_chunk = [&](int c, int step0, int n) -> int {
     for (int k = 0; k < n; k++)
       for (int i = 0; i < nl; i++) {
-        if (lanes[i].exec) CCX_HIP(ctx, hipGraphLaunch(lanes[i].exec, lanes[i].s));
+        const int rec = rec_step[step0 + k];
+        w->head_rec = rec != 0;
+        if (lanes[i].exec[rec]) CCX_HIP(ctx, hipGraphLaunch(lanes[i].exec[rec], lanes[i].s));
         else {
           CCX_TRY(step_lane(i, nullptr));
           if (ctx->prof_on && !use_graph && nl > 1) CCX_HIP(ctx, hipStreamSynchronize(lanes[i].s));
@@ -1253,7 +1280,7 @@
   bool pending = false;
   while (step < total_steps) {
     const int n = (total_steps - step < kChunk) ? total_steps - step : kChunk;
-    CCX_TRY(queue_chunk(c, n));
+    CCX_TRY(queue_chunk(c, step, n));
     step += n;
     if (pending) {
       bool all;
diff --git a/include/ccx.h b/include/ccx.h
--- a/include/ccx.h
+++ b/include/ccx.h
@@ -160,6 +160,16 @@
 
 int ccx_dec_select_step(ccx_ctx* ctx, const ccx_dec_select_desc* desc, void* stream);
 
+typedef struct ccx_dec_head_desc {
+  const void* a; const void* w; const void* bias;
+  int K;
+  int fused, run_select;
+  void* rec; int64_t ld_rec;
+  int64_t a_elems, w_elems, bias_elems, rec_elems;
+  ccx_dec_select_desc sel;
+} ccx_dec_head_desc;
+int ccx_dec_head_step(ccx_ctx* ctx, const ccx_dec_head_desc* desc, void* stream);
+
 #define CCX_ALIGN_SCORES 0
 #define CCX_ALIGN_MATRIX 1
 #define CCX_ALIGN_DTW 2
```

New measurement: 1654 (median of 6 runs). No clear change (+0.4%).
